# haowenz/FEM

Measured on AMD Instinct MI355X. Metric: mapped Mreads/s (100 bp, e=3) at 1/2/4/8 MI355X + achieved HBM GB/s vs roofline, higher is better.
Workload: dtype u32/u64 integer + 32-bit Myers bit-vectors

## Files before the change

fem_amd/csrc/fem_hip.hip:

```cpp
#include "../../include/fem_hip.h"

#include <hip/hip_runtime.h>
#include <rccl/rccl.h>
#include <sched.h>
#if defined(__x86_64__)
#include <immintrin.h>
#endif

#include <algorithm>
#include <cctype>
#include <cstdio>
#include <cstdlib>
#include <cstring>
#include <condition_variable>
#include <functional>
#include <atomic>
#include <chrono>
#include <mutex>
#include <string>
#include <thread>
#include <vector>

#include "fem_index_build.hip.h"
#include "fem_pack.h"
#include "fem_kernels.hip.h"
#include "fem_seed_fast.hip.h"
#include "fem_seed_join.hip.h"
#include "fem_tail.hip.h"
#include "fem_bgzf.hip.h"

namespace {

#ifndef FEM_SLOTS
#define FEM_SLOTS 4
#endif
constexpr int kSlots = FEM_SLOTS;
constexpr uint32_t kMaxReadLen = 1024;
constexpr size_t kFrontPad = 16;
constexpr uint32_t kXcapSmall = 512, kFcap = 128, kCcap = 128;

constexpr int kTimedKernels = 15;
struct TimedLaunch {
  int kernel;
  hipEvent_t start, stop;
  bool counts = true;
};
constexpr int kMaxParts = 4;

struct Slot {
  hipStream_t stream = nullptr;
  uint8_t *d_bases_alloc = nullptr;
  uint8_t *bases() const { return d_bases_alloc + 16; }
  size_t bases_cap = 0;
  uint64_t *d_off = nullptr;
  size_t off_cap = 0;
  uint64_t n_reads = 0;
  uint64_t n_bases = 0;
  uint32_t max_len = 0;
  bool staged = false;
  char *h_bases = nullptr;
  size_t h_bases_cap = 0;
  uint64_t *h_off = nullptr;
  size_t h_off_cap = 0;
  uint64_t acq_reads = 0, acq_bases = 0;
  char *h_quals = nullptr, *h_names = nullptr;
  uint64_t *h_name_off = nullptr;
  size_t h_quals_cap = 0, h_names_cap = 0, h_name_off_cap = 0;
  uint8_t *d_quals = nullptr, *d_names = nullptr;
  uint64_t *d_name_off = nullptr;
  size_t d_quals_cap = 0, d_names_cap = 0, d_name_off_cap = 0;
  bool text_staged = false;
  bool host_quals = false;
  const uint64_t *qual_at = nullptr;
  hipStream_t text_stream = nullptr;
  hipStream_t out_stream = nullptr;
  hipEvent_t ev_text_staged = nullptr;
  hipEvent_t ev_text_order = nullptr;
  bool have_text_order = false;
  uint8_t *d_packed = nullptr;
  size_t packed_cap = 0;
  uint32_t *d_exc_bits = nullptr;
  size_t exc_bits_cap = 0;
  uint32_t packed_bpr = 0;
  bool prefetch_results = false, staged_by_copy = false;
  uint64_t prefetched_reads2 = 0, prefetched_cand = 0, last_n_cand = 0;
  uint64_t h2d_bytes = 0;
  bool sent_packed = false;
  int parts = 1;
  uint32_t part_begin[kMaxParts + 1] = {0, 0, 0, 0, 0};
  hipEvent_t ev_part[kMaxParts] = {nullptr, nullptr, nullptr, nullptr}, ev_sel[kMaxParts] = {nullptr, nullptr, nullptr, nullptr};
  hipEvent_t ev_zeroed = nullptr;
  hipEvent_t ev_results = nullptr, ev_home = nullptr;
  uint64_t *d_cand = nullptr;
  uint32_t *d_meta = nullptr;
  uint8_t *d_ed = nullptr;
  int16_t *d_end = nullptr;
  uint32_t cand_cap = 0;
  uint32_t *d_begin = nullptr, *d_count = nullptr, *d_nmap = nullptr;
  size_t per_read_cap = 0;
  uint8_t *d_ctl = nullptr;
  uint8_t *h_ctl = nullptr;
  uint64_t *d_arena = nullptr;
  uint64_t arena_cap = 0;
  uint32_t *d_slow = nullptr;
  uint32_t slow_cap = 0;
  uint2 *d_sel = nullptr, *d_sel_hdr = nullptr;
  size_t sel_cap = 0, sel_hdr_cap = 0;
  uint32_t *h_begin = nullptr, *h_count = nullptr;
  size_t h_per_read_cap = 0;
  uint64_t *h_cand = nullptr;
  uint8_t *h_ed = nullptr;
  int16_t *h_end = nullptr;
  size_t h_cand_cap = 0;
  uint8_t *d_count8 = nullptr, *d_ped = nullptr;
  uint32_t *d_seg = nullptr;
  uint64_t *d_pcand = nullptr;
  int16_t *d_pend = nullptr;
  uint2 *d_big = nullptr;
  size_t count8_cap = 0, seg_cap = 0, pcand_cap = 0;
  uint8_t *h_count8 = nullptr, *h_ped = nullptr;
  uint32_t *h_seg = nullptr;
  uint64_t *h_pcand = nullptr;
  int16_t *h_pend = nullptr;
  uint2 *h_big = nullptr;
  size_t h_count8_cap = 0, h_seg_cap = 0, h_pcand_cap = 0;
  bool want_packed = false;
  bool packed_enqueued = false;
  uint64_t packed_home = 0, last_n_packed = 0;
  bool packed_per_read_home = false;
  uint32_t n_packed = 0, n_big = 0;
  fem_params params{};
  bool mapped = false, synced = false;
  uint64_t stats[5] = {0, 0, 0, 0, 0};
  uint32_t n_cand = 0;
  std::vector<TimedLaunch> pending;
  femt::Tail *tail = nullptr;
  bool paired = false;
  int32_t min_insert = 0, max_insert = 0;
  uint64_t n_proper = 0;
  bool rescue = false;
  int32_t rescue_edits = 0;
  uint64_t n_rescued = 0;
  bool mapq = false;
  bool unmapped = false;
  uint64_t n_unmapped = 0;
  std::vector<uint16_t> pr_flag;
  std::vector<uint32_t> pr_tid, pr_pos0, pr_cigar_off, pr_cigar, pr_md_off;
  std::vector<uint8_t> pr_nm;
  std::vector<char> pr_md;
};

constexpr size_t kCtlPackCursor = 4 * sizeof(uint32_t) + 2 * sizeof(uint64_t) + 4 * sizeof(uint64_t);
constexpr size_t kCtlBytes = kCtlPackCursor + 2 * sizeof(uint32_t);
constexpr uint32_t kBigCap = 4096;
constexpr size_t kCtlWorkCursor = 128, kCtlWorkCursor2 = 192, kCtlPartStride = 128, kCtlAlloc = 1024;
static_assert(kCtlWorkCursor2 + (kMaxParts - 1) * kCtlPartStride + 64 <= kCtlAlloc, "control block layout");
static_assert(kCtlBytes <= kCtlWorkCursor, "control block layout");

}

namespace {
class StagePool {
 public:
  ~StagePool() {
    {
      std::lock_guard<std::mutex> l(m_);
      stop_ = true;
    }
    cv_.notify_all();
    for (auto &t : threads_) t.join();
  }
  void run(unsigned n, const std::function<void(unsigned)> &work) {
    if (n <= 1) return work(0u);
    {
      std::lock_guard<std::mutex> l(m_);
      while (threads_.size() + 1 < n) {
        const unsigned id = (unsigned)threads_.size() + 1;
        threads_.emplace_back([this, id] { loop(id); });
      }
      work_ = &work, n_ = n, pending_ = n - 1, ++epoch_;
    }
    cv_.notify_all();
    work(0u);
    std::unique_lock<std::mutex> l(m_);
    done_.wait(l, [&] { return pending_ == 0; });
    work_ = nullptr;
  }

 private:
  void loop(unsigned id) {
    uint64_t seen = 0;
    for (;;) {
      const std::function<void(unsigned)> *w = nullptr;
      {
        std::unique_lock<std::mutex> l(m_);
        cv_.wait(l, [&] { return stop_ || (epoch_ != seen && id < n_); });
        if (stop_) return;
        seen = epoch_, w = work_;
      }
      (*w)(id);
      std::lock_guard<std::mutex> l(m_);
      if (--pending_ == 0) done_.notify_one();
    }
  }
  std::mutex m_;
  std::condition_variable cv_, done_;
  std::vector<std::thread> threads_;
  const std::function<void(unsigned)> *work_ = nullptr;
  unsigned n_ = 0, pending_ = 0;
  uint64_t epoch_ = 0;
  bool stop_ = false;
};
}

struct fem_dev {
  femt::TextGate text_gate;
  femz::Bgzf *bgzf = nullptr;
  uint8_t *d_zin = nullptr;
  size_t d_zin_cap = 0;
  hipStream_t z_stream = nullptr;
  std::recursive_mutex mu;
  int device = 0;
  StagePool *stage_pool = nullptr;
  uint8_t *d_ref_names = nullptr;
  uint32_t *d_ref_name_off = nullptr;
  int n_cu = 256;
  std::string err;
  uint32_t *d_lookup = nullptr;
  uint64_t n_lookup = 0;
  uint64_t *d_occ = nullptr;
  uint64_t n_occ = 0;
  int32_t k = 0, step = 0;
  uint64_t fast_occ_key = ~0ull;
  int fast_occ_blocks = 0;
  uint32_t *d_summary = nullptr;
  uint32_t *d_occ32 = nullptr, *d_goff = nullptr, *d_blkseq = nullptr;
  uint32_t list_shift = 0;
  bool no_strided = false;
  uint32_t *d_freq11 = nullptr;
  uint32_t n_banks = 1, bank_first[5] = {0, 0, 0, 0, 0};
  uint32_t *d_bank_lo = nullptr;
  uint64_t bank_limit = 0;
  uint32_t bank_seqs = 0;
  int select_occ_blocks = 0, join_occ_blocks = 0;
  uint64_t select_occ_key = ~0ull, join_occ_key = ~0ull;
  uint8_t *d_planes = nullptr;
  uint8_t *d_ref_raw = nullptr;
  uint64_t ref_bytes = 0;
  uint64_t *d_seq_off = nullptr;
  uint32_t *d_seq_len = nullptr;
  uint32_t n_seq = 0;
  std::vector<uint64_t> seq_off;
  std::vector<uint32_t> seq_len;
  Slot slot[kSlots];
  bool timing = false;
  int verify_blocks_per_cu = 0;
  double t_ms[kTimedKernels] = {};
  uint64_t t_n[kTimedKernels] = {};
  bool force_generic = false;
  bool force_hash = false;
  bool force_dense = false;
  bool no_dense = false;
  bool tiny_buffers = false;
  std::vector<hipEvent_t> event_pool;
  hipEvent_t ev_kernels_done = nullptr;
  bool have_kernels_done = false;
  hipEvent_t ev_select_done = nullptr;
  bool have_select_done = false;
  bool no_overlap = false;
  hipEvent_t ev_h2d_done = nullptr;
  bool have_h2d_done = false;
  hipStream_t side_stream = nullptr;
  bool no_parts = false;
  int max_parts = 2;
  bool timeline = false, have_epoch = false;
  hipEvent_t ev_epoch = nullptr;
};

namespace {

bool testing_switch(const char *name) {
  const char *t = getenv("FEM_TESTING");
  if (!(t && t[0] == '1')) return false;
  const char *v = getenv(name);
  return v && v[0] == '1';
}

int fail(fem_dev *h, int rc, const std::string &msg) {
  if (h) {
    std::lock_guard<std::recursive_mutex> lock(h->mu);
    h->err = msg;
  }
  return rc;
}
#define FEM_LOCK(h) std::lock_guard<std::recursive_mutex> fem_lock_(h->mu)

#define HIP_TRY(h, expr)                                                                          \
  do {                                                                                            \
    hipError_t e_ = (expr);                                                                       \
    if (e_ != hipSuccess)                                                                         \
      return fail(h, e_ == hipErrorOutOfMemory ? FEM_ERR_NOMEM : FEM_ERR_HIP,                     \
                  std::string(#expr) + ": " + hipGetErrorString(e_));                             \
  } while (0)

template <typename T>
int dev_realloc(fem_dev *h, T **p, size_t *cap, size_t want, bool keep = false) {
  if (want <= *cap && *p) return FEM_OK;
  size_t n = std::max(want, *cap + *cap / 2);
  T *q = nullptr;
  HIP_TRY(h, hipMalloc((void **)&q, std::max<size_t>(n, 1) * sizeof(T)));
  if (keep && *p && *cap) HIP_TRY(h, hipMemcpy(q, *p, *cap * sizeof(T), hipMemcpyDeviceToDevice));
  if (*p) (void)hipFree(*p);
  *p = q;
  *cap = n;
  return FEM_OK;
}

template <typename T>
int pinned_realloc(fem_dev *h, T **p, size_t *cap, size_t want) {
  if (want <= *cap && *p) return FEM_OK;
  size_t n = std::max(want, *cap + *cap / 2);
  if (*p) (void)hipHostFree(*p);
  *p = nullptr;
  HIP_TRY(h, hipHostMalloc((void **)p, std::max<size_t>(n, 1) * sizeof(T), hipHostMallocDefault));
  *cap = n;
  return FEM_OK;
}

bool params_ok(const fem_params *p) {
  return p && p->k >= 1 && p->k <= 16 && p->step >= 1 && p->step <= 16 && p->e >= 0 && p->e <= 7 && p->a >= 0 &&
         p->a <= 2;
}

femk::SeedLayout make_layout(const fem_params &p, uint32_t max_len) {
  femk::SeedLayout l{};
  const uint32_t R = (uint32_t)(p.e + 1 + p.a);
  const uint32_t lg = (uint32_t)(p.k / p.step + (p.k % p.step ? 1 : 0));
  const uint32_t n_groups = 2u * (uint32_t)p.step;
  uint32_t smax = max_len >= (uint32_t)p.k ? max_len - (uint32_t)p.k + 1u : 1u;
  int c = (int)(smax / (uint32_t)p.step) - (int)(R * lg) + 2;
  uint32_t cmax = (uint32_t)std::max(c, 2);
  l.smax = smax;
  l.cmax = cmax;
  l.cw = (cmax + 31u) / 32u;
  l.n_words = (max_len + 15u) / 16u + 2u;
  l.xcap = kXcapSmall, l.fcap = kFcap, l.ccap = kCcap;
  uint32_t o = 0;
  auto take = [&](uint32_t bytes) {
    uint32_t at = o;
    o += (bytes + 15u) & ~15u;
    return at;
  };
  l.pkw = take(l.n_words * 4u);
  l.nkw = take(l.n_words * 4u);
  l.sf = take(2u * smax * 8u);
  l.dp_rows = take(n_groups * 2u * cmax * 4u);
  l.dp_bits = take(std::max(n_groups * R * l.cw * 4u, n_groups * R * 8u));
  l.picked = take(n_groups * R * 16u);
  l.rb = take(2u * (R + 1u) * 4u);
  l.X = take(l.xcap * 8u);
  l.F = take(l.fcap * 8u);
  l.A = take(l.ccap * 8u);
  l.B = take(l.ccap * 8u);
  l.wave_bytes = o;
  return l;
}

femk::SeedLayout make_layout_fast(const fem_params &p, uint32_t max_len, bool hash) {
  femk::SeedLayout l{};
  const uint32_t R = (uint32_t)(p.e + 1 + p.a);
  const uint32_t n_groups = 2u * (uint32_t)p.step;
  l.smax = max_len >= (uint32_t)p.k ? max_len - (uint32_t)p.k + 1u : 1u;
  l.n_words = (max_len + 15u) / 16u + 2u;
  l.xcap = 64;
  uint32_t o = 0;
  auto take = [&](uint32_t bytes) {
    uint32_t at = o;
    o += (bytes + 15u) & ~15u;
    return at;
  };
  if (hash) {
    l.pkw = take(l.n_words * 4u);
    l.nkw = take(l.n_words * 4u);
  }
  if (hash) l.sf = take(std::max(2u * l.smax * 8u, 2u * 64u * 8u));
  l.dp_bits = take(std::max(n_groups, femk::kGroupQueue) * R * 8u);
  if (hash) {
    l.X = take(64u * 8u);
    l.A = take(femk::kListScratchBytes);
  }
  l.B = take(2u * femk::kReadBlock * 8u);
  if (!hash) {
    const uint32_t blk_chars = femk::kReadBlock * std::min(max_len, 256u);
    l.strm_words = blk_chars / 16u + 3u;
    l.strm = take(3u * l.strm_words * 4u);
    const uint32_t q_at = o;
    l.F = take(femk::kQueueBytes);
    const uint32_t g0 = l.smax / (uint32_t)femk::kStep;
    const uint32_t n_used = g0 > (uint32_t)femk::kLg ? g0 - (uint32_t)femk::kLg + 1u : 1u;
    l.gq_cap = std::max(384u, n_groups * n_used);
    l.gq = take(std::max(l.gq_cap * 4u + femk::kGroupQueue * 16u + 2u * 32u * 4u, femk::kFlushScratchBytes));
    l.blk_bytes = blk_chars + 32u;
    l.blk = q_at;
    if (o < q_at + l.blk_bytes) take(q_at + l.blk_bytes - o);
  }
  if (hash) {
    l.xcap = (uint32_t)femk::bloom_chunks((int)R) * 64u;
    l.F = take(femk::bloom_slots((int)R) / 16u * 4u);
  }
  l.wave_bytes = o;
  return l;
}

femk::SeedLayout make_layout_select(const fem_params &p, uint32_t max_len) {
  femk::SeedLayout l{};
// ... 48 lines not shown
}
template <int R>
int select_blocks_per_cu_r(bool banked, int block, uint32_t lds) {
  int nb = 0;
  const hipError_t e = banked ? hipOccupancyMaxActiveBlocksPerMultiprocessor(&nb, femk::seed_select_kernel<R, true>, block, lds)
                              : hipOccupancyMaxActiveBlocksPerMultiprocessor(&nb, femk::seed_select_kernel<R>, block, lds);
  return e == hipSuccess ? nb : 0;
}
typedef void (*JoinKernel)(femk::SeedParams);
JoinKernel join_kernel(int R, int which) {
  static const JoinKernel k[3][femk::kMaxR] = {
      {femk::seed_join_kernel_r1, femk::seed_join_kernel_r2, femk::seed_join_kernel_r3, femk::seed_join_kernel_r4, femk::seed_join_kernel_r5,
       femk::seed_join_kernel_r6, femk::seed_join_kernel_r7, femk::seed_join_kernel_r8, femk::seed_join_kernel_r9, femk::seed_join_kernel_r10},
      {femk::seed_join_banked_kernel_r1, femk::seed_join_banked_kernel_r2, femk::seed_join_banked_kernel_r3, femk::seed_join_banked_kernel_r4,
       femk::seed_join_banked_kernel_r5, femk::seed_join_banked_kernel_r6, femk::seed_join_banked_kernel_r7, femk::seed_join_banked_kernel_r8,
       femk::seed_join_banked_kernel_r9, femk::seed_join_banked_kernel_r10},
      {femk::seed_join_kernel_padded_r1, femk::seed_join_kernel_padded_r2, femk::seed_join_kernel_padded_r3, femk::seed_join_kernel_padded_r4,
       femk::seed_join_kernel_padded_r5, femk::seed_join_kernel_padded_r6, femk::seed_join_kernel_padded_r7, femk::seed_join_kernel_padded_r8,
       femk::seed_join_kernel_padded_r9, femk::seed_join_kernel_padded_r10}};
  return k[which][std::min(std::max(R, 1), femk::kMaxR) - 1];
}

#define FEM_DENSE_SWITCH(R, CALL)      \
  switch (R) {                         \
    case 1: CALL(1); break;            \
    case 2: CALL(2); break;            \
    case 3: CALL(3); break;            \
    case 4: CALL(4); break;            \
    case 5: CALL(5); break;            \
    case 6: CALL(6); break;            \
    case 7: CALL(7); break;            \
    case 8: CALL(8); break;            \
    case 9: CALL(9); break;            \
    default: CALL(10); break;          \
  }
template <int R>
uint32_t kernel_regs_r(bool join, int which) {
  hipFuncAttributes a{};
  const bool banked = which == 1;
  const void *f = join ? (const void *)join_kernel(R, which)
                       : banked ? (const void *)femk::seed_select_kernel<R, true> : (const void *)femk::seed_select_kernel<R>;
  return hipFuncGetAttributes(&a, f) == hipSuccess && a.numRegs > 0 ? (uint32_t)a.numRegs : 128u;
}
uint32_t kernel_regs(int R, bool join, int which = 0) {
  static std::atomic<uint32_t> cache[3][2][femk::kMaxR + 1] = {};
  std::atomic<uint32_t> &slot = cache[which][join ? 1 : 0][std::min(std::max(R, 1), femk::kMaxR)];
  uint32_t c = slot.load(std::memory_order_relaxed);
  if (c) return c;
#define FEM_CALL(r) c = kernel_regs_r<r>(join, which)
  FEM_DENSE_SWITCH(R, FEM_CALL)
#undef FEM_CALL
  slot.store(c, std::memory_order_relaxed);
  return c;
}
int select_blocks_per_cu(int R, bool banked, int block, uint32_t lds) {
  int nb = 0;
#define FEM_CALL(r) nb = select_blocks_per_cu_r<r>(banked, block, lds)
  FEM_DENSE_SWITCH(R, FEM_CALL)
#undef FEM_CALL
  return nb;
}
void launch_select(int R, bool banked, dim3 grid, dim3 block, uint32_t lds, hipStream_t st, const femk::SeedParams &sp) {
#define FEM_CALL(r) launch_select_r<r>(banked, grid, block, lds, st, sp)
  FEM_DENSE_SWITCH(R, FEM_CALL)
#undef FEM_CALL
}
int join_blocks_per_cu(int R, int which, int block, uint32_t lds) {
  int nb = 0;
  return hipOccupancyMaxActiveBlocksPerMultiprocessor(&nb, join_kernel(R, which), block, lds) == hipSuccess ? nb : 0;
}
void launch_join(int R, int which, dim3 grid, dim3 block, uint32_t lds, hipStream_t st, const femk::SeedParams &sp) {
  hipLaunchKernelGGL(join_kernel(R, which), grid, block, lds, st, sp);
}

template <int R>
void launch_fast(bool hash, dim3 grid, dim3 block, uint32_t lds, hipStream_t st, const femk::SeedParams &sp) {
  if (hash)
    hipLaunchKernelGGL((femk::seed_fast_kernel<R, true>), grid, block, lds, st, sp);
  else
    hipLaunchKernelGGL((femk::seed_fast_kernel<R, false>), grid, block, lds, st, sp);
}

template <int R>
int fast_blocks_per_cu_r(bool hash, int block, uint32_t lds) {
  int nb = 0;
  hipError_t err = hash ? hipOccupancyMaxActiveBlocksPerMultiprocessor(&nb, femk::seed_fast_kernel<R, true>, block, lds)
                        : hipOccupancyMaxActiveBlocksPerMultiprocessor(&nb, femk::seed_fast_kernel<R, false>, block, lds);
  return err == hipSuccess ? nb : 0;
}
int fast_blocks_per_cu(int R, bool hash, int block, uint32_t lds) {
  switch (R) {
    case 1: return fast_blocks_per_cu_r<1>(hash, block, lds);
    case 2: return fast_blocks_per_cu_r<2>(hash, block, lds);
    case 3: return fast_blocks_per_cu_r<3>(hash, block, lds);
    case 4: return fast_blocks_per_cu_r<4>(hash, block, lds);
    case 5: return fast_blocks_per_cu_r<5>(hash, block, lds);
    case 6: return fast_blocks_per_cu_r<6>(hash, block, lds);
    case 7: return fast_blocks_per_cu_r<7>(hash, block, lds);
    case 8: return fast_blocks_per_cu_r<8>(hash, block, lds);
    case 9: return fast_blocks_per_cu_r<9>(hash, block, lds);
    default: return fast_blocks_per_cu_r<10>(hash, block, lds);
  }
}

hipEvent_t get_event(fem_dev *h) {
  if (!h->event_pool.empty()) {
    hipEvent_t e = h->event_pool.back();
    h->event_pool.pop_back();
    return e;
  }
  hipEvent_t e = nullptr;
  (void)hipEventCreate(&e);
  return e;
}

struct Span {
  fem_dev *h;
  Slot &s;
  hipStream_t st;
  TimedLaunch t;
  bool on;
  Span(fem_dev *h_, Slot &s_, int id, hipStream_t st_) : h(h_), s(s_), st(st_), t{id, nullptr, nullptr, false}, on(h_->timing && h_->timeline) {
    if (on) {
      t.start = get_event(h), t.stop = get_event(h);
      (void)hipEventRecord(t.start, st);
    }
  }
  ~Span() {
    if (on) {
      (void)hipEventRecord(t.stop, st);
      s.pending.push_back(t);
    }
  }
};

void drain_timing(fem_dev *h, Slot &s) {
  for (auto &t : s.pending) {
    float ms = 0.f;
    if (hipEventElapsedTime(&ms, t.start, t.stop) == hipSuccess && t.kernel < kTimedKernels) {
      h->t_ms[t.kernel] += ms;
      h->t_n[t.kernel] += t.counts ? 1 : 0;
    }
    if (h->timeline && h->have_epoch) {
      float a = 0.f, b = 0.f;
      if (hipEventElapsedTime(&a, h->ev_epoch, t.start) == hipSuccess && hipEventElapsedTime(&b, h->ev_epoch, t.stop) == hipSuccess)
        fprintf(stderr, "TL slot %d id %2d  %9.3f %9.3f  (%.3f)\n", (int)(&s - h->slot), t.kernel, a, b, b - a);
    }
    h->event_pool.push_back(t.start);
    h->event_pool.push_back(t.stop);
  }
  s.pending.clear();
}

int ensure_outputs(fem_dev *h, Slot &s) {
  size_t want_reads = (size_t)s.n_reads;
  if (want_reads > s.per_read_cap || !s.d_begin) {
    size_t cap = std::max<size_t>(want_reads, 1);
    if (s.d_begin) (void)hipFree(s.d_begin);
    if (s.d_count) (void)hipFree(s.d_count);
    if (s.d_nmap) (void)hipFree(s.d_nmap);
    s.d_begin = s.d_count = s.d_nmap = nullptr;
    HIP_TRY(h, hipMalloc((void **)&s.d_begin, cap * 2 * sizeof(uint32_t)));
    HIP_TRY(h, hipMalloc((void **)&s.d_count, cap * 2 * sizeof(uint32_t)));
    HIP_TRY(h, hipMalloc((void **)&s.d_nmap, cap * sizeof(uint32_t)));
    s.per_read_cap = cap;
  }
  if (!s.d_cand || !s.d_meta || !s.d_ed || !s.d_end || s.cand_cap == 0) {
    for (void *p : {(void *)s.d_cand, (void *)s.d_meta, (void *)s.d_ed, (void *)s.d_end})
      if (p) (void)hipFree(p);
    s.d_cand = nullptr, s.d_meta = nullptr, s.d_ed = nullptr, s.d_end = nullptr;
    uint64_t want = 2 * s.n_reads + (5u << 20);
    if (h->tiny_buffers) want = 512;
    want = std::min<uint64_t>(want, 0xFFFFFFF0ull);
    s.cand_cap = 0;
    size_t c0 = 0, c1 = 0, c2 = 0, c3 = 0;
    int rc;
    if ((rc = dev_realloc(h, &s.d_cand, &c0, want))) return rc;
    if ((rc = dev_realloc(h, &s.d_meta, &c1, want))) return rc;
    if ((rc = dev_realloc(h, &s.d_ed, &c2, want))) return rc;
    if ((rc = dev_realloc(h, &s.d_end, &c3, want))) return rc;
    s.cand_cap = (uint32_t)want;
  }
  if (!s.d_ctl) {
    HIP_TRY(h, hipMalloc((void **)&s.d_ctl, kCtlAlloc));
    HIP_TRY(h, hipHostMalloc((void **)&s.h_ctl, kCtlBytes, hipHostMallocDefault));
  }
  if (!s.d_arena) {
    s.arena_cap = h->tiny_buffers ? 256u : (4u << 20);
    HIP_TRY(h, hipMalloc((void **)&s.d_arena, s.arena_cap * sizeof(uint64_t)));
  }
  {
    const double avg_bucket = (double)h->n_occ / (double)(h->n_lookup ? h->n_lookup : 1);
    uint64_t want = avg_bucket > 1.0 ? s.n_reads + (1u << 20) : (1u << 18);
    if (h->tiny_buffers) want = s.d_slow ? s.slow_cap : 32;
    if (want > s.slow_cap || !s.d_slow) {
      if (s.d_slow) (void)hipFree(s.d_slow);
      s.d_slow = nullptr;
      HIP_TRY(h, hipMalloc((void **)&s.d_slow, want * sizeof(uint32_t)));
      s.slow_cap = (uint32_t)want;
    }
  }
  return FEM_OK;
}

int grow_candidates(fem_dev *h, Slot &s, uint64_t want) {
  if (want > 0xFFFFFFF0ull) return fail(h, FEM_ERR_UNSUPPORTED, "more than 2^32 candidates in one batch; split the batch");
  s.cand_cap = 0;
  for (void *p : {(void *)s.d_cand, (void *)s.d_meta, (void *)s.d_ed, (void *)s.d_end})
    if (p) (void)hipFree(p);
  s.d_cand = nullptr, s.d_meta = nullptr, s.d_ed = nullptr, s.d_end = nullptr;
  HIP_TRY(h, hipMalloc((void **)&s.d_cand, want * sizeof(uint64_t)));
  HIP_TRY(h, hipMalloc((void **)&s.d_meta, want * sizeof(uint32_t)));
  HIP_TRY(h, hipMalloc((void **)&s.d_ed, want * sizeof(uint8_t)));
  HIP_TRY(h, hipMalloc((void **)&s.d_end, want * sizeof(int16_t)));
  s.cand_cap = (uint32_t)want;
  return FEM_OK;
}

int h2d_begin(fem_dev *h, Slot &s) {
  if (h->have_h2d_done) HIP_TRY(h, hipStreamWaitEvent(s.stream, h->ev_h2d_done, 0));
  return FEM_OK;
}
int h2d_end(fem_dev *h, Slot &s) {
  HIP_TRY(h, hipEventRecord(h->ev_h2d_done, s.stream));
  h->have_h2d_done = true;
  return FEM_OK;
}
bool device_idle(fem_dev *h) {
  return (!h->have_kernels_done || hipEventQuery(h->ev_kernels_done) == hipSuccess) &&
         (!h->have_select_done || hipEventQuery(h->ev_select_done) == hipSuccess);
}
constexpr uint64_t kPartMinReads = 1u << 16;

hipStream_t d2h_begin(fem_dev *h, Slot &s) {
  (void)h;
  return s.stream;
}
int d2h_end(fem_dev *h, Slot &s, hipStream_t st) {
  if (st == s.stream) return FEM_OK;
  HIP_TRY(h, hipEventRecord(s.ev_home, st));
  HIP_TRY(h, hipStreamWaitEvent(s.stream, s.ev_home, 0));
  return FEM_OK;
}

int enqueue_pack(fem_dev *h, Slot &s, bool kernel, bool send_home) {
  const size_t n2 = (size_t)s.n_reads * 2, n_seg = (n2 + 255) / 256;
  int rc;
  if ((rc = dev_realloc(h, &s.d_count8, &s.count8_cap, n2 + 16))) return rc;
  if ((rc = dev_realloc(h, &s.d_seg, &s.seg_cap, n_seg + 4))) return rc;
  if (s.pcand_cap < s.cand_cap || !s.d_pcand) {
    for (void *q : {(void *)s.d_pcand, (void *)s.d_ped, (void *)s.d_pend})
      if (q) (void)hipFree(q);
    s.d_pcand = nullptr, s.d_ped = nullptr, s.d_pend = nullptr, s.pcand_cap = 0;
    HIP_TRY(h, hipMalloc((void **)&s.d_pcand, (size_t)s.cand_cap * sizeof(uint64_t)));
    HIP_TRY(h, hipMalloc((void **)&s.d_ped, (size_t)s.cand_cap * sizeof(uint8_t)));
    HIP_TRY(h, hipMalloc((void **)&s.d_pend, (size_t)s.cand_cap * sizeof(int16_t)));
    s.pcand_cap = s.cand_cap;
  }
  if (!s.d_big) HIP_TRY(h, hipMalloc((void **)&s.d_big, kBigCap * sizeof(uint2)));
  if (n2 + 16 > s.h_count8_cap || !s.h_count8) {
    if (s.h_count8) (void)hipHostFree(s.h_count8);
    s.h_count8 = nullptr, s.h_count8_cap = 0;
    if ((rc = pinned_realloc(h, &s.h_count8, &s.h_count8_cap, n2 + 16))) return rc;
  }
  if (n_seg + 4 > s.h_seg_cap || !s.h_seg) {
    if (s.h_seg) (void)hipHostFree(s.h_seg);
    s.h_seg = nullptr, s.h_seg_cap = 0;
    if ((rc = pinned_realloc(h, &s.h_seg, &s.h_seg_cap, n_seg + 4))) return rc;
  }
  if (!s.h_big) {
    size_t c = 0;
    if ((rc = pinned_realloc(h, &s.h_big, &c, (size_t)kBigCap))) return rc;
  }
  if (kernel) {
  femk::PackParams pp{};
  pp.cand_begin = s.d_begin, pp.cand_count = s.d_count, pp.cand = s.d_cand, pp.ed = s.d_ed, pp.end = s.d_end;
  pp.ctr = (const uint32_t *)s.d_ctl, pp.n_strands = (uint32_t)n2;
  pp.count8 = s.d_count8, pp.seg_begin = s.d_seg, pp.pcand = s.d_pcand, pp.ped = s.d_ped, pp.pend = s.d_pend, pp.pcap = (uint32_t)s.pcand_cap;
  pp.cursor = (uint32_t *)(s.d_ctl + kCtlPackCursor), pp.big = s.d_big, pp.big_cap = kBigCap;
  const uint32_t grid = (uint32_t)std::max<size_t>(1, (n_seg + femk::kPackSegs - 1) / femk::kPackSegs);
  {
    TimedLaunch t{6, nullptr, nullptr, true};
    if (h->timing) {
      t.start = get_event(h), t.stop = get_event(h);
      HIP_TRY(h, hipEventRecord(t.start, s.stream));
    }
    hipLaunchKernelGGL(femk::pack_results_kernel, dim3(grid), dim3(256), 0, s.stream, pp);
    HIP_TRY(h, hipGetLastError());
    if (h->timing) {
      HIP_TRY(h, hipEventRecord(t.stop, s.stream));
      s.pending.push_back(t);
    }
  }
  s.packed_enqueued = true;
  }
  if (send_home) {
    hipStream_t st = d2h_begin(h, s);
    {
      Span span(h, s, 21, st);
      HIP_TRY(h, hipMemcpyAsync(s.h_count8, s.d_count8, n2, hipMemcpyDeviceToHost, st));
      HIP_TRY(h, hipMemcpyAsync(s.h_seg, s.d_seg, n_seg * sizeof(uint32_t), hipMemcpyDeviceToHost, st));
      s.packed_per_read_home = true;
      const size_t guess = std::min<size_t>({(size_t)(s.last_n_packed + s.last_n_packed / 32 + 1024), s.h_pcand_cap, s.pcand_cap});
      if (s.last_n_packed && s.h_pcand && guess) {
        HIP_TRY(h, hipMemcpyAsync(s.h_pcand, s.d_pcand, guess * sizeof(uint64_t), hipMemcpyDeviceToHost, st));
        HIP_TRY(h, hipMemcpyAsync(s.h_ped, s.d_ped, guess * sizeof(uint8_t), hipMemcpyDeviceToHost, st));
        HIP_TRY(h, hipMemcpyAsync(s.h_pend, s.d_pend, guess * sizeof(int16_t), hipMemcpyDeviceToHost, st));
        s.packed_home = guess;
      }
    }
    if ((rc = d2h_end(h, s, st))) return rc;
  }
  return FEM_OK;
}

int launch_batch(fem_dev *h, Slot &s) {
  const fem_params &p = s.params;
  uint32_t *d_ctr = (uint32_t *)s.d_ctl;
  unsigned long long *d_arena_ctr = (unsigned long long *)(s.d_ctl + 4 * sizeof(uint32_t));
  unsigned long long *d_stats = (unsigned long long *)(s.d_ctl + 4 * sizeof(uint32_t) + 2 * sizeof(uint64_t));
  int parts = 1;
  uint32_t part_begin[kMaxParts + 1] = {0, 0, 0, 0, 0};
  const bool copied_in_parts = s.parts > 1;
  {
    const int R_ = p.e + 1 + p.a;
    const bool dense_overlap = !h->force_generic && p.k == femk::kK && p.step == femk::kStep && R_ >= 1 && R_ <= femk::kMaxR && h->d_occ32 &&
                               h->d_freq11 && !h->no_overlap;
    if (dense_overlap && !h->no_parts && s.n_reads >= 2 * kPartMinReads && (copied_in_parts || device_idle(h))) {
      parts = copied_in_parts ? s.parts : (int)std::min<uint64_t>((uint64_t)h->max_parts, s.n_reads / kPartMinReads);
      for (int q = 0; q <= parts; ++q)
        part_begin[q] = copied_in_parts ? s.part_begin[q] : q == parts ? (uint32_t)s.n_reads : (uint32_t)((s.n_reads * q / parts) & ~63ull);
    }
    s.parts = 1;
  }
  if (parts > 1) {
    if (h->have_select_done) HIP_TRY(h, hipStreamWaitEvent(h->side_stream, h->ev_select_done, 0));
    HIP_TRY(h, hipMemsetAsync(s.d_ctl, 0, kCtlAlloc, h->side_stream));
  } else {
    HIP_TRY(h, hipMemsetAsync(s.d_ctl, 0, kCtlAlloc, s.stream));
  }

  femk::SeedParams sp{};
  sp.bases = s.bases();
  sp.read_off = s.d_off;
  sp.n_reads = (uint32_t)s.n_reads;
  sp.read_begin = 0;
  sp.lookup = h->d_lookup;
  sp.occ = h->d_occ;
  sp.inf32 = (uint32_t)h->n_occ;
  sp.seq_len = h->d_seq_len;
  sp.e = p.e, sp.a = p.a, sp.R = p.e + 1 + p.a, sp.k = p.k, sp.step = p.step;
  sp.lg = p.k / p.step + (p.k % p.step ? 1 : 0);
  sp.cand = s.d_cand, sp.cand_meta = s.d_meta, sp.cand_cap = s.cand_cap;
  sp.cand_begin = s.d_begin, sp.cand_count = s.d_count;
  sp.ctr = d_ctr;
  sp.work_cursor = (uint32_t *)(s.d_ctl + kCtlWorkCursor);
  sp.stats = d_stats;
  sp.arena = s.d_arena, sp.arena_cap = s.arena_cap, sp.arena_ctr = d_arena_ctr;
  sp.lay = make_layout(p, std::max<uint32_t>(s.max_len, (uint32_t)p.k));

  sp.n_seq = h->n_seq;
  sp.summary = h->d_summary;
  sp.slow_queue = s.d_slow, sp.slow_cap = s.slow_cap;
  sp.work_queue = nullptr;
  const int R = p.e + 1 + p.a;
  const bool use_fast = !h->force_generic && p.k == femk::kK && p.step == femk::kStep && R >= 1 && R <= femk::kMaxR;

  auto shape = [&](const femk::SeedLayout &lay, uint32_t *wpb_out, uint32_t *lds_out, uint32_t *grid_out) {
    uint32_t wpb = std::min<uint32_t>(4u, std::max<uint32_t>(1u, (64u * 1024u) / lay.wave_bytes));
    uint32_t lds_bytes = wpb * lay.wave_bytes;
    uint32_t waves_per_cu = std::min<uint32_t>(32u, (160u * 1024u / lds_bytes) * wpb);
    uint64_t blocks_wanted = (s.n_reads + wpb - 1) / wpb;
    uint64_t blocks_resident = (uint64_t)h->n_cu * std::max<uint32_t>(1u, waves_per_cu / wpb);
    *wpb_out = wpb, *lds_out = lds_bytes;
    *grid_out = (uint32_t)std::max<uint64_t>(1, std::min<uint64_t>(blocks_wanted, blocks_resident * 4));
  };
  if (sp.lay.wave_bytes > 64u * 1024u) return fail(h, FEM_ERR_UNSUPPORTED, "read too long for the device path");

  auto timed = [&](int id, hipStream_t st, auto &&launch, bool counts = true) -> int {
    TimedLaunch t{id, nullptr, nullptr, counts};
    if (h->timing) {
      t.start = get_event(h), t.stop = get_event(h);
      HIP_TRY(h, hipEventRecord(t.start, st));
    }
    launch();
    HIP_TRY(h, hipGetLastError());
    if (h->timing) {
      HIP_TRY(h, hipEventRecord(t.stop, st));
      s.pending.push_back(t);
    }
    return FEM_OK;
  };

  if (s.n_reads) {
    int rc;
    const bool split_dense = use_fast && h->d_occ32 && h->d_freq11;
    const bool overlap = split_dense && !h->no_overlap;
    if (!overlap && h->have_kernels_done) HIP_TRY(h, hipStreamWaitEvent(s.stream, h->ev_kernels_done, 0));
    femk::VerifyParams vp{};
    vp.bases = s.bases(), vp.read_off = s.d_off;
    vp.planes = h->d_planes, vp.seq_off = h->d_seq_off;
    vp.cand = s.d_cand, vp.cand_meta = s.d_meta;
    vp.ctr = d_ctr, vp.cand_cap = s.cand_cap, vp.e = p.e;
    vp.ed = s.d_ed, vp.end = s.d_end;
    vp.n_map = s.d_nmap, vp.stats = d_stats;
    HIP_TRY(h, hipMemsetAsync(s.d_nmap, 0, (size_t)s.n_reads * sizeof(uint32_t), s.stream));
    if (h->verify_blocks_per_cu == 0) {
      int nb = 0;
      if (hipOccupancyMaxActiveBlocksPerMultiprocessor(&nb, femk::verify_kernel, 256, 0) != hipSuccess || nb <= 0) nb = 4;
      h->verify_blocks_per_cu = nb;
    }
    const uint32_t vgrid = (uint32_t)h->n_cu * (uint32_t)h->verify_blocks_per_cu;
    if (split_dense) {
      const uint32_t max_len = std::max<uint32_t>(s.max_len, (uint32_t)p.k);
      const bool banked = h->n_banks > 1;
      const size_t want_sel = (size_t)s.n_reads * 6u * (size_t)R * h->n_banks;
      if ((rc = dev_realloc(h, &s.d_sel, &s.sel_cap, want_sel))) return rc;
      if ((rc = dev_realloc(h, &s.d_sel_hdr, &s.sel_hdr_cap, (size_t)s.n_reads))) return rc;
      femk::SeedParams fp = sp;
      fp.occ32 = h->d_occ32, fp.list_shift = h->list_shift, fp.goff = h->d_goff, fp.blkseq = h->d_blkseq;
      fp.freq11 = h->d_freq11, fp.sel = s.d_sel, fp.sel_hdr = s.d_sel_hdr;
      fp.n_banks = h->n_banks, fp.bank_lo = h->d_bank_lo, fp.n_buckets = (uint32_t)(h->n_lookup - 1);
      fp.blk_stride = (femk::kDenseRemap >> femk::kDenseBlkShift) + 1u;
      for (uint32_t b = 0; b <= femk::kDenseMaxBanks; ++b) fp.bank_first[b] = h->bank_first[b];
      uint32_t select_lds = 0, select_threads = 256;
      fp.lay = make_layout_select(p, max_len);
      if (fp.lay.wave_bytes > 64u * 1024u) return fail(h, FEM_ERR_UNSUPPORTED, "read too long for the device path");
      const femk::SeedLayout lay_select = fp.lay;
      femk::SeedLayout lay_join = make_layout_join(p, banked, !banked && h->list_shift != 0);
      const uint32_t wpb_s = std::min<uint32_t>(4u, std::max<uint32_t>(1u, (64u * 1024u) / lay_select.wave_bytes));
      const uint32_t wpb_j = std::min<uint32_t>(4u, std::max<uint32_t>(1u, (60u * 1024u) / lay_join.wave_bytes));
      lay_join.picked = wpb_j * lay_join.wave_bytes;
      const uint32_t lds_j = wpb_j * lay_join.wave_bytes + 64u * 8u;
      const int which = banked ? 1 : h->list_shift ? 2 : 0;
      uint64_t per_cu_s, per_cu_j;
      {
        const uint32_t lds_bytes = wpb_s * lay_select.wave_bytes;
        const uint64_t key = ((uint64_t)banked << 48) | ((uint64_t)R << 40) | lds_bytes;
        if (h->select_occ_key != key) h->select_occ_key = key, h->select_occ_blocks = select_blocks_per_cu(R, banked, (int)(64u * wpb_s), lds_bytes);
        per_cu_s = h->select_occ_blocks > 0 ? (uint64_t)h->select_occ_blocks : std::max<uint64_t>(1, 160u * 1024u / lds_bytes);
        if (overlap) per_cu_s = 1;
        select_lds = lds_bytes, select_threads = 64u * wpb_s;
      }
      {
        const uint64_t key = ((uint64_t)which << 48) | ((uint64_t)R << 40) | lds_j;
        if (h->join_occ_key != key) h->join_occ_key = key, h->join_occ_blocks = join_blocks_per_cu(R, which, (int)(64u * wpb_j), lds_j);
        per_cu_j = h->join_occ_blocks > 0 ? (uint64_t)h->join_occ_blocks : std::max<uint64_t>(1, 160u * 1024u / lds_j);
        if (overlap) {
          const uint32_t vj = (kernel_regs(R, true, which) + 7u) & ~7u, vs = (kernel_regs(R, false, banked ? 1 : 0) + 7u) & ~7u;
          const uint32_t wj = 64u * wpb_j / 256u ? 64u * wpb_j / 256u : 1u, ws = select_threads / 256u ? select_threads / 256u : 1u;
          const uint32_t lj = (lds_j + 511u) & ~511u, ls = (select_lds + 511u) & ~511u;
          while (per_cu_j > 1 && (per_cu_j * wj * vj + ws * vs > 512u || per_cu_j * lj + ls > 160u * 1024u || per_cu_j * wj + ws > 8u)) --per_cu_j;
        }
      }
      if (parts > 1 && !copied_in_parts) {
        HIP_TRY(h, hipEventRecord(s.ev_zeroed, s.stream));
        HIP_TRY(h, hipStreamWaitEvent(h->side_stream, s.ev_zeroed, 0));
      }
      for (int q = 0; q < parts; ++q) {
        const uint32_t r_lo = parts > 1 ? part_begin[q] : 0u, r_hi = parts > 1 ? part_begin[q + 1] : (uint32_t)s.n_reads;
        const uint64_t blocks_of_reads = ((uint64_t)(r_hi - r_lo) + femk::kReadBlock - 1) / femk::kReadBlock;
        fp.read_begin = r_lo, fp.n_reads = r_hi;
        hipStream_t st_sel = parts > 1 ? h->side_stream : s.stream;
        {
          fp.lay = lay_select;
          if (parts > 1) {
            if (copied_in_parts) HIP_TRY(h, hipStreamWaitEvent(st_sel, s.ev_part[q], 0));
          } else if (overlap && h->have_select_done) {
            HIP_TRY(h, hipStreamWaitEvent(s.stream, h->ev_select_done, 0));
          }
          const uint32_t grid = (uint32_t)std::max<uint64_t>(1, std::min<uint64_t>((blocks_of_reads + wpb_s - 1) / wpb_s, (uint64_t)h->n_cu * per_cu_s));
          fp.work_cursor = (uint32_t *)(s.d_ctl + kCtlWorkCursor + (size_t)q * kCtlPartStride);
          rc = timed(8, st_sel, [&] { launch_select(R, banked, dim3(grid), dim3(64u * wpb_s), select_lds, st_sel, fp); }, q == 0);
          if (rc) return rc;
          if (parts > 1) {
            HIP_TRY(h, hipEventRecord(s.ev_sel[q], st_sel));
            HIP_TRY(h, hipStreamWaitEvent(s.stream, s.ev_sel[q], 0));
          }
          if (overlap && q + 1 == parts) {
            HIP_TRY(h, hipEventRecord(h->ev_select_done, st_sel));
            h->have_select_done = true;
          }
          if (overlap && q == 0 && h->have_kernels_done) HIP_TRY(h, hipStreamWaitEvent(s.stream, h->ev_kernels_done, 0));
        }
        {
          fp.lay = lay_join;
          const uint32_t grid = (uint32_t)std::max<uint64_t>(1, std::min<uint64_t>((blocks_of_reads + wpb_j - 1) / wpb_j, (uint64_t)h->n_cu * per_cu_j));
          fp.work_cursor = (uint32_t *)(s.d_ctl + kCtlWorkCursor2 + (size_t)q * kCtlPartStride);
          rc = timed(0, s.stream, [&] { launch_join(R, which, dim3(grid), dim3(64u * wpb_j), lds_j, s.stream, fp); }, q == 0);
          if (rc) return rc;
        }
      }
      sp.work_queue = s.d_slow;
    } else if (use_fast) {
      femk::SeedParams fp = sp;
      const bool hash = h->force_hash || (double)h->n_occ > (double)h->n_lookup;
      fp.lay = make_layout_fast(p, std::max<uint32_t>(s.max_len, (uint32_t)p.k), hash);
      uint32_t wpb, lds_bytes, grid;
      shape(fp.lay, &wpb, &lds_bytes, &grid);
      {
        const uint64_t key = ((uint64_t)R << 40) | ((uint64_t)hash << 32) | lds_bytes;
        if (h->fast_occ_key != key) h->fast_occ_key = key, h->fast_occ_blocks = fast_blocks_per_cu((int)R, hash, (int)(64u * wpb), lds_bytes);
        static const uint64_t mult = testing_switch("FEM_TESTING") && getenv("FEM_GRID_MULT") ? (uint64_t)std::max(1, atoi(getenv("FEM_GRID_MULT"))) : 1;
        const uint64_t per_cu = h->fast_occ_blocks > 0 ? (uint64_t)h->fast_occ_blocks : std::max<uint64_t>(1, 160u * 1024u / lds_bytes);
        const uint64_t wanted = (s.n_reads + (uint64_t)femk::kReadBlock * wpb - 1) / ((uint64_t)femk::kReadBlock * wpb);
        grid = (uint32_t)std::max<uint64_t>(1, std::min<uint64_t>(wanted, (uint64_t)h->n_cu * per_cu * mult));
      }
      auto launch_range = [&](uint32_t lo, uint32_t hi) {
        femk::SeedParams q = fp;
        q.read_begin = lo, q.n_reads = hi;
        dim3 g(grid), b(64u * wpb);
        switch (R) {
          case 1: launch_fast<1>(hash, g, b, lds_bytes, s.stream, q); break;
          case 2: launch_fast<2>(hash, g, b, lds_bytes, s.stream, q); break;
          case 3: launch_fast<3>(hash, g, b, lds_bytes, s.stream, q); break;
          case 4: launch_fast<4>(hash, g, b, lds_bytes, s.stream, q); break;
          case 5: launch_fast<5>(hash, g, b, lds_bytes, s.stream, q); break;
          case 6: launch_fast<6>(hash, g, b, lds_bytes, s.stream, q); break;
          case 7: launch_fast<7>(hash, g, b, lds_bytes, s.stream, q); break;
          case 8: launch_fast<8>(hash, g, b, lds_bytes, s.stream, q); break;
          case 9: launch_fast<9>(hash, g, b, lds_bytes, s.stream, q); break;
          default: launch_fast<10>(hash, g, b, lds_bytes, s.stream, q); break;
        }
      };
      rc = timed(0, s.stream, [&] { launch_range(0, (uint32_t)s.n_reads); });
      if (rc) return rc;
      sp.work_queue = s.d_slow;
    }
    {
      uint32_t wpb, lds_bytes, grid;
      shape(sp.lay, &wpb, &lds_bytes, &grid);
      rc = timed(2, s.stream, [&] { hipLaunchKernelGGL(femk::seed_filter_kernel, dim3(grid), dim3(64u * wpb), lds_bytes, s.stream, sp); });
      if (rc) return rc;
    }
    rc = timed(1, s.stream, [&] { hipLaunchKernelGGL(femk::verify_kernel, dim3(vgrid), dim3(256), 0, s.stream, vp); });
    if (rc) return rc;
    s.packed_enqueued = false, s.packed_home = 0, s.packed_per_read_home = false;
    if (s.want_packed && split_dense && (rc = enqueue_pack(h, s, true, false))) return rc;
    HIP_TRY(h, hipEventRecord(h->ev_kernels_done, s.stream));
    h->have_kernels_done = true;
    if (s.want_packed && (rc = enqueue_pack(h, s, !split_dense, true))) return rc;
  } else {
    s.packed_enqueued = false, s.packed_home = 0, s.packed_per_read_home = false;
  }
  HIP_TRY(h, hipMemcpyAsync(s.h_ctl, s.d_ctl, kCtlBytes, hipMemcpyDeviceToHost, s.stream));
  s.prefetched_reads2 = 0, s.prefetched_cand = 0;
  static const bool no_prefetch = testing_switch("FEM_NO_PREFETCH");
  if (s.prefetch_results && !s.want_packed && s.staged_by_copy && !no_prefetch) {
    hipStream_t st = d2h_begin(h, s);
    {
      Span span(h, s, 21, st);
      const size_t n2 = (size_t)s.n_reads * 2;
      if (n2 && s.h_begin && n2 <= s.h_per_read_cap) {
        HIP_TRY(h, hipMemcpyAsync(s.h_begin, s.d_begin, n2 * sizeof(uint32_t), hipMemcpyDeviceToHost, st));
        HIP_TRY(h, hipMemcpyAsync(s.h_count, s.d_count, n2 * sizeof(uint32_t), hipMemcpyDeviceToHost, st));
        s.prefetched_reads2 = n2;
      }
      const size_t guess = std::min<size_t>({(size_t)(s.last_n_cand + s.last_n_cand / 32 + 1024), s.h_cand_cap, (size_t)s.cand_cap});
      if (s.last_n_cand && s.h_cand && guess) {
        HIP_TRY(h, hipMemcpyAsync(s.h_cand, s.d_cand, guess * sizeof(uint64_t), hipMemcpyDeviceToHost, st));
        HIP_TRY(h, hipMemcpyAsync(s.h_ed, s.d_ed, guess * sizeof(uint8_t), hipMemcpyDeviceToHost, st));
        HIP_TRY(h, hipMemcpyAsync(s.h_end, s.d_end, guess * sizeof(int16_t), hipMemcpyDeviceToHost, st));
        s.prefetched_cand = guess;
      }
    }
    int rc2 = d2h_end(h, s, st);
    if (rc2) return rc2;
  }
  s.mapped = true;
  s.synced = false;
  return FEM_OK;
}

int refresh_summary(fem_dev *h) {
  if (h->d_summary) (void)hipFree(h->d_summary);
  h->d_summary = nullptr;
  const uint64_t n_buckets = h->n_lookup - 1;
// ... 121 lines not shown
  std::vector<uint64_t *> bufs;
};
std::mutex g_comm_mu;
CommSet *g_comm = nullptr;
void destroy_comm_set() {
  if (!g_comm) return;
  for (size_t i = 0; i < g_comm->devs.size(); ++i) {
    (void)hipSetDevice(g_comm->devs[i]);
    if (g_comm->bufs[i]) (void)hipFree(g_comm->bufs[i]);
    if (g_comm->comms[i]) ncclCommDestroy(g_comm->comms[i]);
  }
  delete g_comm;
  g_comm = nullptr;
}

int check_slot(fem_dev *h, int slot) {
  if (!h) return FEM_ERR_INVALID;
  if (slot < 0 || slot >= kSlots) return fail(h, FEM_ERR_INVALID, "slot out of range");
  return FEM_OK;
}


using fempack::pack_bases;

int enqueue_packed(fem_dev *h, Slot &s, uint64_t n, uint32_t len, uint64_t n_exc) {
  const uint32_t bpr = fempack::bytes_per_read(len);
  const uint64_t code_bytes = fempack::code_bytes(n, len), n_bases = n * (uint64_t)len;
  const uint64_t total = code_bytes + n_exc * 5u;
  int rc;
  if ((rc = dev_realloc(h, &s.d_packed, &s.packed_cap, (size_t)total + 64))) return rc;
  if ((rc = dev_realloc(h, &s.d_bases_alloc, &s.bases_cap, kFrontPad + (size_t)n_bases + 64))) return rc;
  if ((rc = dev_realloc(h, &s.d_off, &s.off_cap, (size_t)n + 1))) return rc;
  if ((rc = dev_realloc(h, &s.d_exc_bits, &s.exc_bits_cap, (size_t)n / 32 + 2))) return rc;
  s.parts = 1;
  if (!h->no_parts && !h->no_overlap && n_exc == 0 && n >= 2 * kPartMinReads && device_idle(h))
    s.parts = (int)std::min<uint64_t>((uint64_t)h->max_parts, n / kPartMinReads);
  for (int q = 0; q <= s.parts; ++q) s.part_begin[q] = q == s.parts ? (uint32_t)n : (uint32_t)((n * q / s.parts) & ~63ull);
  HIP_TRY(h, hipMemsetAsync(s.d_exc_bits, 0, ((size_t)n / 32 + 1) * sizeof(uint32_t), s.stream));
  hipLaunchKernelGGL(femk::uniform_offsets_kernel, dim3((uint32_t)std::min<uint64_t>((n + 256) / 256, (uint64_t)h->n_cu * 8u)), dim3(256), 0,
                     s.stream, s.d_off, n, len);
  if ((rc = h2d_begin(h, s))) return rc;
  for (int q = 0; q < s.parts; ++q) {
    const uint64_t r0 = s.part_begin[q], r1 = s.part_begin[q + 1];
    const uint64_t b0 = r0 * bpr, b1 = q + 1 == s.parts ? total : r1 * bpr;
    Span span(h, s, 20, s.stream);
    if (b1 > b0) HIP_TRY(h, hipMemcpyAsync(s.d_packed + b0, s.h_bases + b0, b1 - b0, hipMemcpyHostToDevice, s.stream));
    if (q + 1 == s.parts && (rc = h2d_end(h, s))) return rc;
    if (r1 > r0) {
      const uint32_t grid = (uint32_t)std::min<uint64_t>(((r1 - r0) * bpr + 255) / 256, (uint64_t)h->n_cu * 16u);
      hipLaunchKernelGGL(femk::unpack_reads_kernel, dim3(grid), dim3(256), 0, s.stream, (const uint8_t *)s.d_packed + b0, r1 - r0, len, bpr,
                         s.bases() + r0 * len);
    }
    if (s.parts > 1) HIP_TRY(h, hipEventRecord(s.ev_part[q], s.stream));
  }
  if (n_exc) {
    const dim3 g((uint32_t)std::min<uint64_t>((n_exc + 255) / 256, (uint64_t)h->n_cu * 4u));
    hipLaunchKernelGGL(femk::scatter_chars_kernel, g, dim3(256), 0, s.stream, (const uint32_t *)(s.d_packed + code_bytes),
                       (const uint8_t *)(s.d_packed + code_bytes + 4u * n_exc), n_exc, s.bases());
    hipLaunchKernelGGL(femk::mark_exception_reads_kernel, g, dim3(256), 0, s.stream, (const uint32_t *)(s.d_packed + code_bytes), n_exc, len,
                       s.d_exc_bits);
  }
  s.packed_bpr = bpr;
  HIP_TRY(h, hipGetLastError());
  s.n_reads = n, s.n_bases = n_bases, s.max_len = len;
  s.staged = true, s.mapped = false, s.synced = false;
  s.h2d_bytes = total, s.sent_packed = true;
  return FEM_OK;
}

unsigned stage_threads(uint64_t n_reads) {
  unsigned want = 12;
  if (const char *e = getenv("FEM_STAGE_THREADS")) want = (unsigned)std::max(1, atoi(e));
  const unsigned hw = std::thread::hardware_concurrency();
  return (unsigned)std::max<uint64_t>(1, std::min<uint64_t>({(uint64_t)(hw ? hw : 1), (uint64_t)want, n_reads / 65536 + 1}));
}

}

extern "C" {

const char *fem_strerror(int rc) {
  switch (rc) {
    case FEM_OK: return "ok";
    case FEM_ERR_INVALID: return "invalid argument";
    case FEM_ERR_HIP: return "HIP runtime error";
    case FEM_ERR_NOMEM: return "out of memory";
    case FEM_ERR_STATE: return "call order violated";
    case FEM_ERR_UNSUPPORTED: return "input not supported by the device path";
    case FEM_ERR_RCCL: return "RCCL error";
    default: return "unknown error";
  }
}

const char *fem_dev_last_error(const fem_dev *h) { return h ? h->err.c_str() : "null handle"; }

static std::atomic<int> g_blocking_waits{0};
int fem_set_blocking_waits(int on) {
  g_blocking_waits.store(on ? 1 : 0);
  return FEM_OK;
}

int fem_dev_open(int device, fem_dev **out) {
  if (!out) return FEM_ERR_INVALID;
  *out = nullptr;
  int n = 0;
  if (hipGetDeviceCount(&n) != hipSuccess || n <= 0) return FEM_ERR_HIP;
  if (device < 0 || device >= n) return FEM_ERR_INVALID;
  fem_dev *h = new (std::nothrow) fem_dev();
  if (!h) return FEM_ERR_NOMEM;
  h->device = device;
  if (hipSetDevice(device) != hipSuccess) {
    delete h;
    return FEM_ERR_HIP;
  }
  if (g_blocking_waits.load() || testing_switch("FEM_BLOCKING_SYNC")) (void)hipSetDeviceFlags(hipDeviceScheduleBlockingSync);
  hipDeviceProp_t prop;
  if (hipGetDeviceProperties(&prop, device) == hipSuccess) h->n_cu = prop.multiProcessorCount;
  for (int i = 0; i < kSlots; ++i) {
    if (hipStreamCreateWithFlags(&h->slot[i].stream, hipStreamNonBlocking) != hipSuccess) {
      delete h;
      return FEM_ERR_HIP;
    }
  }
  bool ok_ev = hipEventCreateWithFlags(&h->ev_kernels_done, hipEventDisableTiming) == hipSuccess &&
               hipEventCreateWithFlags(&h->ev_select_done, hipEventDisableTiming) == hipSuccess &&
               hipEventCreateWithFlags(&h->ev_h2d_done, hipEventDisableTiming) == hipSuccess &&
               hipStreamCreateWithFlags(&h->side_stream, hipStreamNonBlocking) == hipSuccess;
  for (int i = 0; ok_ev && i < kSlots; ++i) {
    Slot &sl = h->slot[i];
    ok_ev = hipEventCreateWithFlags(&sl.ev_zeroed, hipEventDisableTiming) == hipSuccess &&
            hipEventCreateWithFlags(&sl.ev_results, hipEventDisableTiming) == hipSuccess &&
            hipEventCreateWithFlags(&sl.ev_home, hipEventDisableTiming) == hipSuccess;
    for (int q = 0; ok_ev && q < kMaxParts; ++q)
      ok_ev = hipEventCreateWithFlags(&sl.ev_part[q], hipEventDisableTiming) == hipSuccess &&
              hipEventCreateWithFlags(&sl.ev_sel[q], hipEventDisableTiming) == hipSuccess;
  }
  if (!ok_ev) {
    (void)fem_dev_close(h);
    return FEM_ERR_HIP;
  }
  if (testing_switch("FEM_TESTING")) {
    h->no_overlap = testing_switch("FEM_NO_OVERLAP");
    h->no_parts = testing_switch("FEM_NO_PARTS");
    if (const char *mp = getenv("FEM_PARTS")) h->max_parts = std::min(kMaxParts, std::max(1, atoi(mp)));
    h->timeline = testing_switch("FEM_TIMELINE");
    if (h->timeline && hipEventCreate(&h->ev_epoch) == hipSuccess && hipEventRecord(h->ev_epoch, h->side_stream) == hipSuccess)
      h->timing = true, h->have_epoch = true;
    h->force_generic = testing_switch("FEM_FORCE_GENERIC");
    h->force_hash = testing_switch("FEM_FORCE_HASH");
    h->force_dense = testing_switch("FEM_FORCE_DENSE");
    h->no_dense = testing_switch("FEM_NO_DENSE");
    h->no_strided = testing_switch("FEM_NO_STRIDED");
    h->tiny_buffers = testing_switch("FEM_TEST_TINY_BUFFERS");
    if (const char *bl = getenv("FEM_TEST_BANK_BASES")) h->bank_limit = strtoull(bl, nullptr, 10);
    if (const char *bs = getenv("FEM_TEST_BANK_SEQS")) h->bank_seqs = (uint32_t)strtoul(bs, nullptr, 10);
  }
  *out = h;
  return FEM_OK;
}

int fem_dev_close(fem_dev *h) {
  if (!h) return FEM_ERR_INVALID;
  {
    std::lock_guard<std::mutex> lock(g_comm_mu);
    if (g_comm && std::find(g_comm->devs.begin(), g_comm->devs.end(), h->device) != g_comm->devs.end()) destroy_comm_set();
  }
  (void)hipSetDevice(h->device);
  (void)hipDeviceSynchronize();
  delete h->stage_pool;
  h->stage_pool = nullptr;
  for (auto &s : h->slot) {
    drain_timing(h, s);
    for (void *p : {(void *)s.d_bases_alloc, (void *)s.d_off, (void *)s.d_cand, (void *)s.d_meta, (void *)s.d_ed,
                    (void *)s.d_end, (void *)s.d_begin, (void *)s.d_count, (void *)s.d_nmap, (void *)s.d_ctl,
                    (void *)s.d_arena, (void *)s.d_slow, (void *)s.d_sel, (void *)s.d_sel_hdr, (void *)s.d_packed, (void *)s.d_exc_bits, (void *)s.d_quals, (void *)s.d_names,
                    (void *)s.d_name_off, (void *)s.d_count8, (void *)s.d_seg, (void *)s.d_pcand, (void *)s.d_ped, (void *)s.d_pend, (void *)s.d_big})
      if (p) (void)hipFree(p);
    for (void *p : {(void *)s.h_ctl, (void *)s.h_begin, (void *)s.h_count, (void *)s.h_cand, (void *)s.h_ed,
                    (void *)s.h_end, (void *)s.h_bases, (void *)s.h_off, (void *)s.h_quals, (void *)s.h_names, (void *)s.h_name_off,
                    (void *)s.h_count8, (void *)s.h_seg, (void *)s.h_pcand, (void *)s.h_ped, (void *)s.h_pend, (void *)s.h_big})
      if (p) (void)hipHostFree(p);
    if (s.stream) (void)hipStreamDestroy(s.stream);
    if (s.text_stream) (void)hipStreamDestroy(s.text_stream);
    if (s.out_stream) (void)hipStreamDestroy(s.out_stream);
    if (s.ev_text_staged) (void)hipEventDestroy(s.ev_text_staged);
    if (s.ev_text_order) (void)hipEventDestroy(s.ev_text_order);
    delete s.tail;
    s.tail = nullptr;
  }
  delete h->bgzf;
  h->bgzf = nullptr;
  if (h->d_zin) (void)hipFree(h->d_zin);
  if (h->z_stream) (void)hipStreamDestroy(h->z_stream);
  if (h->d_ref_names) (void)hipFree(h->d_ref_names);
  if (h->d_ref_name_off) (void)hipFree(h->d_ref_name_off);
  for (hipEvent_t e : h->event_pool) (void)hipEventDestroy(e);
  if (h->ev_kernels_done) (void)hipEventDestroy(h->ev_kernels_done);
  if (h->ev_select_done) (void)hipEventDestroy(h->ev_select_done);
  if (h->ev_h2d_done) (void)hipEventDestroy(h->ev_h2d_done);
  if (h->ev_epoch) (void)hipEventDestroy(h->ev_epoch);
  if (h->side_stream) (void)hipStreamDestroy(h->side_stream);
  for (int i = 0; i < kSlots; ++i) {
    Slot &sl = h->slot[i];
    if (sl.ev_zeroed) (void)hipEventDestroy(sl.ev_zeroed);
    if (sl.ev_results) (void)hipEventDestroy(sl.ev_results);
    if (sl.ev_home) (void)hipEventDestroy(sl.ev_home);
    for (int q = 0; q < kMaxParts; ++q) {
      if (sl.ev_part[q]) (void)hipEventDestroy(sl.ev_part[q]);
      if (sl.ev_sel[q]) (void)hipEventDestroy(sl.ev_sel[q]);
    }
  }
  for (void *p : {(void *)h->d_lookup, (void *)h->d_occ, (void *)h->d_ref_raw, (void *)h->d_seq_off,
                  (void *)h->d_seq_len, (void *)h->d_summary, (void *)h->d_planes, (void *)h->d_occ32, (void *)h->d_goff, (void *)h->d_blkseq,
                  (void *)h->d_freq11, (void *)h->d_bank_lo})
    if (p) (void)hipFree(p);
  delete h;
  return FEM_OK;
}

int fem_dev_limits(const fem_dev *h, uint32_t *max_read_len, int32_t *n_slots) {
  if (!h) return FEM_ERR_INVALID;
  if (max_read_len) *max_read_len = kMaxReadLen;
  if (n_slots) *n_slots = kSlots;
  return FEM_OK;
}

int fem_dev_upload_index(fem_dev *h, int32_t k, int32_t step, const uint32_t *lookup, uint64_t n_lookup,
                         const uint64_t *occ, uint64_t n_occ) {
  if (!h || !lookup || (!occ && n_occ)) return FEM_ERR_INVALID;
  if (k < 1 || k > 16 || step < 1) return fail(h, FEM_ERR_INVALID, "k must be 1..16 and step >= 1");
  if (n_lookup != (1ull << (2 * k)) + 1) return fail(h, FEM_ERR_INVALID, "lookup table must have 4^k + 1 entries");
  if (n_occ > 0xFFFFFFFFull) return fail(h, FEM_ERR_INVALID, "occurrence table larger than its uint32 prefix sums");
  HIP_TRY(h, hipSetDevice(h->device));
  if (h->d_lookup) (void)hipFree(h->d_lookup);
  if (h->d_occ) (void)hipFree(h->d_occ);
  h->d_lookup = nullptr, h->d_occ = nullptr;
  HIP_TRY(h, hipMalloc((void **)&h->d_lookup, n_lookup * sizeof(uint32_t)));
  HIP_TRY(h, hipMalloc((void **)&h->d_occ, std::max<uint64_t>(n_occ, 1) * sizeof(uint64_t)));
  HIP_TRY(h, hipMemcpy(h->d_lookup, lookup, n_lookup * sizeof(uint32_t), hipMemcpyHostToDevice));
  if (n_occ) HIP_TRY(h, hipMemcpy(h->d_occ, occ, n_occ * sizeof(uint64_t), hipMemcpyHostToDevice));
  h->n_lookup = n_lookup, h->n_occ = n_occ, h->k = k, h->step = step;
  int rc = refresh_summary(h);
  return rc ? rc : refresh_dense(h);
}

namespace {
int make_codes(fem_dev *h, uint8_t **out) {
  *out = nullptr;
  uint8_t *codes = nullptr;
  const uint64_t total = h->ref_bytes;
  HIP_TRY(h, hipMalloc((void **)&codes, total + 128));
  hipError_t e = hipMemcpy(codes, h->d_ref_raw, total, hipMemcpyDeviceToDevice);
  if (e == hipSuccess) e = hipMemset(codes + total, 4, 128);
  if (e == hipSuccess && total) {
    hipLaunchKernelGGL(femk::ref_encode_kernel, dim3((uint32_t)h->n_cu * 8u), dim3(256), 0, 0, codes, total);
    e = hipGetLastError();
    if (e == hipSuccess) e = hipDeviceSynchronize();
  }
  if (e != hipSuccess) {
    (void)hipFree(codes);
    HIP_TRY(h, e);
  }
  *out = codes;
  return FEM_OK;
}
}

int fem_dev_upload_reference(fem_dev *h, uint32_t n_seq, const char *const *seq, const uint32_t *seq_len) {
  if (!h || !seq || !seq_len || n_seq == 0) return FEM_ERR_INVALID;
  HIP_TRY(h, hipSetDevice(h->device));
  h->seq_off.assign(n_seq, 0);
  h->seq_len.assign(seq_len, seq_len + n_seq);
  uint64_t total = 0;
  for (uint32_t i = 0; i < n_seq; ++i) {
    h->seq_off[i] = total;
    total += seq_len[i];
  }
  for (void *p : {(void *)h->d_ref_raw, (void *)h->d_seq_off, (void *)h->d_seq_len, (void *)h->d_planes})
    if (p) (void)hipFree(p);
  h->d_ref_raw = nullptr, h->d_seq_off = nullptr, h->d_seq_len = nullptr;
  h->d_planes = nullptr;
  h->ref_bytes = 0, h->n_seq = 0;
  HIP_TRY(h, hipMalloc((void **)&h->d_ref_raw, total + 128));
  HIP_TRY(h, hipMalloc((void **)&h->d_seq_off, n_seq * sizeof(uint64_t)));
  HIP_TRY(h, hipMalloc((void **)&h->d_seq_len, n_seq * sizeof(uint32_t)));
  for (uint32_t i = 0; i < n_seq; ++i)
    if (seq_len[i]) HIP_TRY(h, hipMemcpy(h->d_ref_raw + h->seq_off[i], seq[i], seq_len[i], hipMemcpyHostToDevice));
  HIP_TRY(h, hipMemset(h->d_ref_raw + total, 0, 128));
  HIP_TRY(h, hipMemcpy(h->d_seq_off, h->seq_off.data(), n_seq * sizeof(uint64_t), hipMemcpyHostToDevice));
  HIP_TRY(h, hipMemcpy(h->d_seq_len, h->seq_len.data(), n_seq * sizeof(uint32_t), hipMemcpyHostToDevice));
  HIP_TRY(h, hipMemset(h->d_ref_raw + total, 'N', 128));
  h->ref_bytes = total, h->n_seq = n_seq;
  {
    auto drop_reference = [&]() {
      for (void *q : {(void *)h->d_ref_raw, (void *)h->d_seq_off, (void *)h->d_seq_len, (void *)h->d_planes})
        if (q) (void)hipFree(q);
      h->d_ref_raw = nullptr, h->d_seq_off = nullptr, h->d_seq_len = nullptr, h->d_planes = nullptr;
      h->ref_bytes = 0, h->n_seq = 0;
    };
    uint8_t *codes = nullptr;
    int rc = make_codes(h, &codes);
    if (rc) {
      drop_reference();
      return rc;
    }
    const uint64_t n_pb = (total + 64 + 7) / 8;
    hipError_t e = hipMalloc((void **)&h->d_planes, femk::plane_bytes(n_pb));
    if (e == hipSuccess) e = hipMemset(h->d_planes, 0, femk::plane_bytes(n_pb));
    if (e == hipSuccess) {
      hipLaunchKernelGGL(femk::ref_planes_kernel, dim3((uint32_t)h->n_cu * 8u), dim3(256), 0, 0, codes, h->d_ref_raw, n_pb, h->d_planes);
      e = hipGetLastError();
      if (e == hipSuccess) e = hipDeviceSynchronize();
    }
    (void)hipFree(codes);
    if (e != hipSuccess) drop_reference();
    HIP_TRY(h, e);
  }
  return refresh_dense(h);
}

int fem_dev_build_index(fem_dev *h, int32_t k, int32_t step, uint32_t *lookup_out, uint64_t *occ_out, uint64_t occ_cap,
                        uint64_t *n_occ_out) {
  if (!h) return FEM_ERR_INVALID;
  if (!h->d_ref_raw) return fail(h, FEM_ERR_STATE, "upload the reference before building the index");
  if (k < 1 || k > 16 || step < 1) return fail(h, FEM_ERR_INVALID, "k must be 1..16 and step >= 1");
  HIP_TRY(h, hipSetDevice(h->device));
  if (h->d_lookup) (void)hipFree(h->d_lookup);
  if (h->d_occ) (void)hipFree(h->d_occ);
  h->d_lookup = nullptr, h->d_occ = nullptr;
// ... 116 lines not shown
  Slot &s = h->slot[slot];
  if (!s.h_bases) return fail(h, FEM_ERR_STATE, "acquire the slot's staging buffers first");
  if (read_len == 0 && n_reads) return fail(h, FEM_ERR_INVALID, "packed batches hold reads of one non-zero length");
  if (read_len > kMaxReadLen)
    return fail(h, FEM_ERR_UNSUPPORTED, "read longer than the device path supports (" + std::to_string(kMaxReadLen) + ")");
  const uint64_t n_bases = n_reads * (uint64_t)read_len;
  if (n_reads > s.acq_reads || n_bases > s.acq_bases) return fail(h, FEM_ERR_INVALID, "more reads than the staging buffers were acquired for");
  if (n_bases >= 0xFFFFFFF0ull) return fail(h, FEM_ERR_UNSUPPORTED, "a packed batch holds fewer than 2^32 bases; split the batch");
  const uint64_t code_bytes = fempack::code_bytes(n_reads, read_len);
  if (code_bytes + n_exceptions * 5u > s.acq_bases + 64 || n_exceptions > n_bases / 16u)
    return fail(h, FEM_ERR_INVALID, "more exceptions than a packed batch may carry (fem_dev_packed_layout): commit the characters instead");
  const uint32_t *pos = (const uint32_t *)(s.h_bases + code_bytes);
  for (uint64_t i = 0; i < n_exceptions; ++i)
    if (pos[i] >= n_bases) return fail(h, FEM_ERR_INVALID, "exception position outside the batch");
  HIP_TRY(h, hipSetDevice(h->device));
  if ((rc = enqueue_packed(h, s, n_reads, read_len, n_exceptions))) return rc;
  s.staged_by_copy = true;
  return FEM_OK;
}

int fem_dev_stage_reads(fem_dev *h, int slot, const fem_read_batch *reads) {
  int rc = check_slot(h, slot);
  if (rc) return rc;
  if (!reads || (reads->n_reads && (!reads->bases || !reads->offsets))) return fail(h, FEM_ERR_INVALID, "null read batch");
  if (reads->n_reads > 0x3FFFFFF0ull) return fail(h, FEM_ERR_UNSUPPORTED, "more than 2^30 reads in one batch");
  const uint64_t n = reads->n_reads;
  const uint64_t base0 = n ? reads->offsets[0] : 0;
  if (n && reads->offsets[n] < base0) return fail(h, FEM_ERR_INVALID, "read offsets must be ascending");
  const uint64_t n_bases = n ? reads->offsets[n] - base0 : 0;
  char *hb = nullptr;
  uint64_t *ho = nullptr;
  if ((rc = fem_dev_acquire_stage(h, slot, n, n_bases, &hb, &ho))) return rc;
  Slot &s = h->slot[slot];
  const unsigned n_thr = stage_threads(n);
  if (!h->stage_pool) h->stage_pool = new (std::nothrow) StagePool();
  if (!h->stage_pool) return fail(h, FEM_ERR_NOMEM, "out of host memory");
  auto run_threads = [&](unsigned nt, const std::function<void(unsigned)> &work) { h->stage_pool->run(nt, work); };
  std::vector<uint32_t> t_max(n_thr, 0), t_min(n_thr, 0xFFFFFFFFu);
  std::atomic<int> bad{0};
  run_threads(n_thr, [&](unsigned t) {
    const uint64_t r_lo = n * t / n_thr, r_hi = n * (t + 1) / n_thr;
    uint32_t mx = 0, mn = 0xFFFFFFFFu;
    for (uint64_t i = r_lo; i < r_hi; ++i) {
      const uint64_t o0 = reads->offsets[i], o1 = reads->offsets[i + 1];
      if (o1 < o0) {
        bad.store(1);
        return;
      }
      const uint64_t len = o1 - o0;
      if (len > kMaxReadLen) {
        bad.store(2);
        return;
      }
      mx = std::max<uint32_t>(mx, (uint32_t)len), mn = std::min<uint32_t>(mn, (uint32_t)len);
    }
    t_max[t] = mx, t_min[t] = mn;
  });
  if (bad.load() == 1) return fail(h, FEM_ERR_INVALID, "read offsets must be ascending");
  if (bad.load() == 2)
    return fail(h, FEM_ERR_UNSUPPORTED, "read longer than the device path supports (" + std::to_string(kMaxReadLen) + ")");
  uint32_t max_len = 0, min_len = 0xFFFFFFFFu;
  for (unsigned t = 0; t < n_thr; ++t) max_len = std::max(max_len, t_max[t]), min_len = std::min(min_len, t_min[t]);
  const bool no_pack = testing_switch("FEM_NO_PACK");
  if (n && min_len == max_len && max_len > 0 && n_bases < 0xFFFFFFF0ull && !no_pack) {
    const uint32_t len = max_len, bpr = (len + 3u) / 4u;
    const uint64_t code_bytes = (n * bpr + 7u) & ~7ull;
    const uint64_t exc_cap = (n_bases + 64 - std::min<uint64_t>(code_bytes, n_bases + 64)) / 5u;
    std::vector<std::vector<uint64_t>> exc(n_thr);
    const uint8_t *src = (const uint8_t *)reads->bases + base0;
    constexpr uint64_t kPiece = 32768;
    std::atomic<uint64_t> next_piece{0};
    run_threads(n_thr, [&](unsigned t) {
      for (;;) {
        const uint64_t r_lo = next_piece.fetch_add(1, std::memory_order_relaxed) * kPiece;
        if (r_lo >= n) break;
        const uint64_t r_hi = std::min(n, r_lo + kPiece);
        if ((len & 3u) == 0u) {
          pack_bases(src + r_lo * len, (r_hi - r_lo) * len, (uint8_t *)hb + r_lo * bpr, r_lo * len, exc[t]);
        } else {
          for (uint64_t i = r_lo; i < r_hi; ++i) pack_bases(src + i * len, len, (uint8_t *)hb + i * bpr, i * len, exc[t]);
        }
      }
    });
    uint64_t n_exc = 0;
    for (const auto &v : exc) n_exc += v.size();
    if (n_exc <= exc_cap && n_exc <= n_bases / 16u) {
      uint32_t *he = (uint32_t *)(hb + code_bytes);
      uint8_t *hc = (uint8_t *)(he + n_exc);
      for (const auto &v : exc)
        for (uint64_t x : v) *he++ = (uint32_t)(x >> 8), *hc++ = (uint8_t)x;
      {
        FEM_LOCK(h);
        if ((rc = enqueue_packed(h, s, n, len, n_exc))) return rc;
      }
      s.staged_by_copy = true;
      return FEM_OK;
    }
  }
  run_threads(n_thr, [&](unsigned t) {
    const uint64_t r_lo = n * t / n_thr, r_hi = n * (t + 1) / n_thr;
    for (uint64_t i = r_lo; i < r_hi; ++i) ho[i] = reads->offsets[i] - base0;
    if (r_hi == n) ho[n] = reads->offsets[n] - base0;
    if (r_hi > r_lo) memcpy(hb + (reads->offsets[r_lo] - base0), reads->bases + reads->offsets[r_lo], reads->offsets[r_hi] - reads->offsets[r_lo]);
  });
  if (n == 0) ho[0] = 0;
  rc = fem_dev_commit_stage(h, slot, n, max_len);
  s.staged_by_copy = true;
  return rc;
}

int fem_dev_stage_info(fem_dev *h, int slot, uint64_t *h2d_bytes, int32_t *packed) {
  int rc = check_slot(h, slot);
  if (rc) return rc;
  if (h2d_bytes) *h2d_bytes = h->slot[slot].h2d_bytes;
  if (packed) *packed = h->slot[slot].sent_packed ? 1 : 0;
  return FEM_OK;
}

int fem_dev_map_staged(fem_dev *h, int slot, const fem_params *p) {
  int rc = check_slot(h, slot);
  if (rc) return rc;
  FEM_LOCK(h);
  if (!params_ok(p)) return fail(h, FEM_ERR_INVALID, "parameters out of range (k 1..16, step 1..16, e 0..7, a 0..2)");
  if (!h->d_lookup || !h->d_ref_raw || !h->d_planes) return fail(h, FEM_ERR_STATE, "index and reference must be uploaded first");
  if (p->k != h->k) return fail(h, FEM_ERR_INVALID, "k differs from the uploaded index");
  Slot &s = h->slot[slot];
  if (!s.staged) return fail(h, FEM_ERR_STATE, "no reads staged in this slot");
  HIP_TRY(h, hipSetDevice(h->device));
  s.params = *p;
  if ((rc = ensure_outputs(h, s))) return rc;
  return launch_batch(h, s);
}

int fem_dev_sync(fem_dev *h, int slot) {
  int rc = check_slot(h, slot);
  if (rc) return rc;
  Slot &s = h->slot[slot];
  if (!s.mapped) return fail(h, FEM_ERR_STATE, "nothing was mapped in this slot");
  HIP_TRY(h, hipSetDevice(h->device));
  if (s.synced) return FEM_OK;
  for (int attempt = 0; attempt < 8; ++attempt) {
    HIP_TRY(h, hipStreamSynchronize(s.stream));
    FEM_LOCK(h);
    drain_timing(h, s);
    const uint32_t *ctr = (const uint32_t *)s.h_ctl;
    const uint64_t *arena_ctr = (const uint64_t *)(s.h_ctl + 4 * sizeof(uint32_t));
    const uint64_t *st = (const uint64_t *)(s.h_ctl + 4 * sizeof(uint32_t) + 2 * sizeof(uint64_t));
    uint32_t flags = ctr[1];
    if (flags & femk::kFlagTooLarge)
      return fail(h, FEM_ERR_UNSUPPORTED, "a read selects more than 2^31 occurrence entries in one seed group");
    if (flags == 0) {
      s.n_cand = ctr[0];
      s.n_packed = ((const uint32_t *)(s.h_ctl + kCtlPackCursor))[0], s.n_big = ((const uint32_t *)(s.h_ctl + kCtlPackCursor))[1];
      s.stats[0] = s.n_reads;
      s.stats[1] = st[3];
      s.stats[2] = st[0];
      s.stats[3] = st[1];
      s.stats[4] = st[2];
      s.synced = true;
      return FEM_OK;
    }
    if (flags & femk::kFlagCandOverflow) {
      uint64_t want = (uint64_t)ctr[0] + ctr[0] / 8 + 1024;
      if ((rc = grow_candidates(h, s, std::min<uint64_t>(want, 0xFFFFFFF0ull)))) return rc;
    }
    if (flags & femk::kFlagQueueOverflow) {
      uint64_t want = (uint64_t)ctr[2] + ctr[2] / 8 + 4096;
      (void)hipFree(s.d_slow);
      s.d_slow = nullptr;
      s.slow_cap = 0;
      hipError_t e = hipMalloc((void **)&s.d_slow, want * sizeof(uint32_t));
      if (e != hipSuccess) return fail(h, FEM_ERR_NOMEM, "slow-read queue does not fit in device memory");
      s.slow_cap = (uint32_t)std::min<uint64_t>(want, 0xFFFFFFF0ull);
    }
    if (flags & femk::kFlagArenaOverflow) {
      uint64_t want = arena_ctr[1] + arena_ctr[1] / 8 + 1024;
      (void)hipFree(s.d_arena);
      s.d_arena = nullptr;
      hipError_t e = hipMalloc((void **)&s.d_arena, want * sizeof(uint64_t));
      if (e != hipSuccess) {
        s.arena_cap = 0;
        return fail(h, FEM_ERR_NOMEM, "scratch arena for oversized seed lists does not fit in device memory; use smaller batches");
      }
      s.arena_cap = want;
    }
    if ((rc = launch_batch(h, s))) return rc;
  }
  return fail(h, FEM_ERR_HIP, "batch kept overflowing its scratch buffers");
}

int fem_dev_fetch_stats(fem_dev *h, int slot, uint64_t stats[5]) {
  int rc = fem_dev_sync(h, slot);
  if (rc) return rc;
  if (stats) memcpy(stats, h->slot[slot].stats, sizeof(uint64_t) * 5);
  h->slot[slot].prefetch_results = false;
  return FEM_OK;
}

int fem_dev_fetch(fem_dev *h, int slot, fem_batch_result *out) {
  int rc = fem_dev_sync(h, slot);
  if (rc) return rc;
  if (!out) return fail(h, FEM_ERR_INVALID, "null result");
  Slot &s = h->slot[slot];
  const size_t n2 = (size_t)s.n_reads * 2, nc = s.n_cand;
  bool regrown = false;
  if (n2 > s.h_per_read_cap || !s.h_begin) {
    regrown = true;
    size_t c0 = 0, c1 = 0;
    if (s.h_begin) (void)hipHostFree(s.h_begin);
    if (s.h_count) (void)hipHostFree(s.h_count);
    s.h_begin = s.h_count = nullptr;
    if ((rc = pinned_realloc(h, &s.h_begin, &c0, std::max<size_t>(n2, 2)))) return rc;
    if ((rc = pinned_realloc(h, &s.h_count, &c1, std::max<size_t>(n2, 2)))) return rc;
    s.h_per_read_cap = c0;
  }
  if (nc > s.h_cand_cap || !s.h_cand) {
    regrown = true;
    size_t c0 = 0, c1 = 0, c2 = 0;
    for (void *p : {(void *)s.h_cand, (void *)s.h_ed, (void *)s.h_end})
      if (p) (void)hipHostFree(p);
    s.h_cand = nullptr, s.h_ed = nullptr, s.h_end = nullptr;
    size_t want = std::max<size_t>(nc + nc / 4, 1024);
    if ((rc = pinned_realloc(h, &s.h_cand, &c0, want))) return rc;
    if ((rc = pinned_realloc(h, &s.h_ed, &c1, want))) return rc;
    if ((rc = pinned_realloc(h, &s.h_end, &c2, want))) return rc;
    s.h_cand_cap = c0;
  }
  const bool per_read_home = !regrown && s.prefetched_reads2 == n2;
  const size_t c_from = regrown ? 0 : std::min<size_t>(s.prefetched_cand, nc);
  if (n2 && !per_read_home) {
    HIP_TRY(h, hipMemcpyAsync(s.h_begin, s.d_begin, n2 * sizeof(uint32_t), hipMemcpyDeviceToHost, s.stream));
    HIP_TRY(h, hipMemcpyAsync(s.h_count, s.d_count, n2 * sizeof(uint32_t), hipMemcpyDeviceToHost, s.stream));
  }
  if (nc > c_from) {
    HIP_TRY(h, hipMemcpyAsync(s.h_cand + c_from, s.d_cand + c_from, (nc - c_from) * sizeof(uint64_t), hipMemcpyDeviceToHost, s.stream));
    HIP_TRY(h, hipMemcpyAsync(s.h_ed + c_from, s.d_ed + c_from, (nc - c_from) * sizeof(uint8_t), hipMemcpyDeviceToHost, s.stream));
    HIP_TRY(h, hipMemcpyAsync(s.h_end + c_from, s.d_end + c_from, (nc - c_from) * sizeof(int16_t), hipMemcpyDeviceToHost, s.stream));
  }
  if ((n2 && !per_read_home) || nc > c_from) HIP_TRY(h, hipStreamSynchronize(s.stream));
  s.prefetch_results = true, s.last_n_cand = nc, s.want_packed = false;
  out->n_reads = s.n_reads;
  out->n_candidates = nc;
  out->cand_begin = s.h_begin, out->cand_count = s.h_count;
  out->cand = s.h_cand, out->ed = s.h_ed, out->end = s.h_end;
  memcpy(out->stats, s.stats, sizeof s.stats);
  return FEM_OK;
}

int fem_dev_fetch_packed(fem_dev *h, int slot, fem_batch_packed *out) {
  int rc = fem_dev_sync(h, slot);
  if (rc) return rc;
  if (!out) return fail(h, FEM_ERR_INVALID, "null result");
  Slot &s = h->slot[slot];
  const size_t n2 = (size_t)s.n_reads * 2, n_seg = (n2 + 255) / 256;
  if (!s.packed_enqueued && s.n_reads) {
    if ((rc = enqueue_pack(h, s, true, false))) return rc;
    HIP_TRY(h, hipMemcpyAsync(s.h_ctl, s.d_ctl, kCtlBytes, hipMemcpyDeviceToHost, s.stream));
    HIP_TRY(h, hipStreamSynchronize(s.stream));
    s.n_packed = ((const uint32_t *)(s.h_ctl + kCtlPackCursor))[0], s.n_big = ((const uint32_t *)(s.h_ctl + kCtlPackCursor))[1];
  }
  if (s.n_big > kBigCap) return fail(h, FEM_ERR_UNSUPPORTED, "more strands with 255 candidates and more than a packed result lists: use fem_dev_fetch");
  const size_t np = s.n_reads ? s.n_packed : 0;
  bool regrown = false;
  if (np > s.h_pcand_cap || !s.h_pcand) {
    regrown = true;
    for (void *q : {(void *)s.h_pcand, (void *)s.h_ped, (void *)s.h_pend})
      if (q) (void)hipHostFree(q);
    s.h_pcand = nullptr, s.h_ped = nullptr, s.h_pend = nullptr;
    size_t c0 = 0, c1 = 0, c2 = 0;
    const size_t want = std::max<size_t>(np + np / 4, 1024);
    if ((rc = pinned_realloc(h, &s.h_pcand, &c0, want))) return rc;
    if ((rc = pinned_realloc(h, &s.h_ped, &c1, want))) return rc;
    if ((rc = pinned_realloc(h, &s.h_pend, &c2, want))) return rc;
    s.h_pcand_cap = c0;
  }
  bool copied = false;
  if (n2 && !s.packed_per_read_home) {
    HIP_TRY(h, hipMemcpyAsync(s.h_count8, s.d_count8, n2, hipMemcpyDeviceToHost, s.stream));
    HIP_TRY(h, hipMemcpyAsync(s.h_seg, s.d_seg, n_seg * sizeof(uint32_t), hipMemcpyDeviceToHost, s.stream));
    s.packed_per_read_home = true, copied = true;
  }
  const size_t c_from = regrown ? 0 : std::min<size_t>(s.packed_home, np);
  if (np > c_from) {
    HIP_TRY(h, hipMemcpyAsync(s.h_pcand + c_from, s.d_pcand + c_from, (np - c_from) * sizeof(uint64_t), hipMemcpyDeviceToHost, s.stream));
    HIP_TRY(h, hipMemcpyAsync(s.h_ped + c_from, s.d_ped + c_from, (np - c_from) * sizeof(uint8_t), hipMemcpyDeviceToHost, s.stream));
    HIP_TRY(h, hipMemcpyAsync(s.h_pend + c_from, s.d_pend + c_from, (np - c_from) * sizeof(int16_t), hipMemcpyDeviceToHost, s.stream));
    s.packed_home = np, copied = true;
  }
  if (s.n_big) {
    HIP_TRY(h, hipMemcpyAsync(s.h_big, s.d_big, (size_t)s.n_big * sizeof(uint2), hipMemcpyDeviceToHost, s.stream));
    copied = true;
  }
  if (copied) HIP_TRY(h, hipStreamSynchronize(s.stream));
  s.want_packed = true, s.last_n_packed = np;
  out->n_reads = s.n_reads;
  out->n_candidates = np;
  out->count = s.h_count8, out->seg_begin = s.h_seg;
  out->cand = s.h_pcand, out->ed = s.h_ped, out->end = s.h_pend;
  out->big = (const uint32_t *)s.h_big, out->n_big = s.n_big;
  memcpy(out->stats, s.stats, sizeof s.stats);
  return FEM_OK;
}

int fem_dev_upload_reference_names(fem_dev *h, uint32_t n_seq, const char *names, const uint64_t *name_off) {
  if (!h || !names || !name_off || n_seq == 0) return FEM_ERR_INVALID;
  if (h->n_seq && n_seq != h->n_seq) return fail(h, FEM_ERR_INVALID, "as many names as reference sequences, please");
// ... 364 lines not shown
}

int fem_dev_set_rescue(fem_dev *h, int slot, const fem_rescue_params *rp) {
  int rc = check_slot(h, slot);
  if (rc) return rc;
  FEM_LOCK(h);
  Slot &s = h->slot[slot];
  if (!rp) {
    s.rescue = false;
    return FEM_OK;
  }
  if (rp->max_edits < 0 || rp->max_edits > 15) return fail(h, FEM_ERR_INVALID, "rescue edit bound out of range (0 <= max_edits <= 15)");
  s.rescue = true, s.rescue_edits = rp->max_edits;
  return FEM_OK;
}

int fem_dev_set_mapq(fem_dev *h, int slot, int on) {
  int rc = check_slot(h, slot);
  if (rc) return rc;
  FEM_LOCK(h);
  h->slot[slot].mapq = on != 0;
  return FEM_OK;
}

int fem_dev_set_unmapped(fem_dev *h, int slot, int on) {
  int rc = check_slot(h, slot);
  if (rc) return rc;
  FEM_LOCK(h);
  h->slot[slot].unmapped = on != 0;
  return FEM_OK;
}

int fem_dev_unmapped_count(fem_dev *h, int slot, uint64_t *n) {
  int rc = check_slot(h, slot);
  if (rc) return rc;
  if (!n) return fail(h, FEM_ERR_INVALID, "null output pointer");
  FEM_LOCK(h);
  *n = h->slot[slot].n_unmapped;
  return FEM_OK;
}

int fem_dev_rescue_count(fem_dev *h, int slot, uint64_t *n_rescued) {
  int rc = check_slot(h, slot);
  if (rc) return rc;
  if (!n_rescued) return fail(h, FEM_ERR_INVALID, "null output pointer");
  FEM_LOCK(h);
  Slot &s = h->slot[slot];
  if (!s.paired) return fail(h, FEM_ERR_STATE, "the slot is not in pair mode (fem_dev_set_pairs)");
  *n_rescued = s.n_rescued;
  return FEM_OK;
}

int fem_dev_fetch_pairs(fem_dev *h, int slot, fem_batch_pairs *out) {
  int rc = check_slot(h, slot);
  if (rc) return rc;
  if (!out) return fail(h, FEM_ERR_INVALID, "null result");
  if (!h->slot[slot].paired) return fail(h, FEM_ERR_STATE, "the slot is not in pair mode (fem_dev_set_pairs)");
  if ((rc = fem_dev_sync(h, slot))) return rc;
  Slot &s = h->slot[slot];
  if (s.n_reads & 1) return fail(h, FEM_ERR_INVALID, "a batch of read pairs holds an even number of reads");
  femt::RescueInput ri{};
  if ((rc = rescue_input(h, s, &ri))) return rc;
  fem_batch_records rec{};
  if ((rc = fem_dev_fetch_records(h, slot, &rec))) return rc;
  std::string err;
  femt::PairOutput po{};
  if ((rc = s.tail->pair(s.min_insert, s.max_insert, s.stream, &err, s.rescue ? &ri : nullptr))) return fail(h, rc, err);
  if ((rc = s.tail->pair_fetch(s.stream, &po, &err))) return fail(h, rc, err);
  const uint64_t nr = po.n_records;
  s.pr_flag.assign(po.flag, po.flag + nr);
  s.pr_tid.resize(nr), s.pr_pos0.resize(nr), s.pr_nm.resize(nr), s.pr_cigar_off.resize(nr + 1), s.pr_md_off.resize(nr + 1);
  s.pr_cigar.clear(), s.pr_md.clear();
  s.pr_cigar_off[0] = 0, s.pr_md_off[0] = 0;
  for (uint64_t k = 0; k < nr; ++k) {
    const uint32_t r = po.perm[k];
    if (r < po.first_rescued) {
      s.pr_tid[k] = rec.tid[r], s.pr_pos0[k] = rec.pos0[r], s.pr_nm[k] = rec.nm[r];
      s.pr_cigar.insert(s.pr_cigar.end(), rec.cigar + rec.cigar_off[r], rec.cigar + rec.cigar_off[r + 1]);
      s.pr_md.insert(s.pr_md.end(), rec.md + rec.md_off[r], rec.md + rec.md_off[r + 1]);
    } else {
      const uint32_t q = r - po.first_rescued, c0 = po.r_cigar_off[0], m0 = po.r_md_off[0];
      s.pr_tid[k] = po.r_tid[q], s.pr_pos0[k] = po.r_pos0[q], s.pr_nm[k] = po.r_nm[q];
      s.pr_cigar.insert(s.pr_cigar.end(), po.r_cigar + (po.r_cigar_off[q] - c0), po.r_cigar + (po.r_cigar_off[q + 1] - c0));
      s.pr_md.insert(s.pr_md.end(), po.r_md + (po.r_md_off[q] - m0), po.r_md + (po.r_md_off[q + 1] - m0));
    }
    s.pr_cigar_off[k + 1] = (uint32_t)s.pr_cigar.size(), s.pr_md_off[k + 1] = (uint32_t)s.pr_md.size();
  }
  s.n_proper = po.n_proper, s.n_rescued = po.n_rescued;
  out->n_pairs = po.n_pairs, out->n_records = nr;
  out->rec_begin = po.pair_begin, out->flag = s.pr_flag.data(), out->tid = s.pr_tid.data(), out->pos0 = s.pr_pos0.data();
  out->nm = s.pr_nm.data(), out->cigar_off = s.pr_cigar_off.data(), out->cigar = s.pr_cigar.data();
  out->md_off = s.pr_md_off.data(), out->md = s.pr_md.data();
  out->mate_tid = po.mate_tid, out->mate_pos0 = po.mate_pos0, out->tlen = po.tlen;
  out->n_proper = po.n_proper;
  memcpy(out->stats, s.stats, sizeof s.stats);
  return FEM_OK;
}

int fem_dev_map_batch_submit(fem_dev *h, int slot, const fem_params *p, const fem_read_batch *reads) {
  int rc = fem_dev_stage_reads(h, slot, reads);
  if (rc) return rc;
  return fem_dev_map_staged(h, slot, p);
}

int fem_dev_map_batch_wait(fem_dev *h, int slot, fem_batch_result *out) { return fem_dev_fetch(h, slot, out); }

int fem_dev_index_info(const fem_dev *h, char *buf, uint64_t cap) {
  if (!h || !buf || cap == 0) return FEM_ERR_INVALID;
  const uint64_t n_buckets = h->n_lookup ? h->n_lookup - 1 : 0;
  std::string s;
  if (!h->d_lookup) {
    s = "no index";
  } else if (h->d_occ32 && h->d_freq11) {
    s = "dense: 32-bit occurrence table, ";
    s += h->list_shift ? "strided with pads (" + std::to_string(((n_buckets + femk::kDensePadBuckets) << h->list_shift) * 4 >> 20) + " MiB)"
                       : "compact (" + std::to_string(h->n_occ * 4 >> 20) + " MiB)";
    s += ", " + std::to_string(h->n_banks) + (h->n_banks == 1 ? " bank" : " banks") + ", freq11 64 MiB";
  } else if (h->d_summary) {
    s = "sparse: bucket summaries";
  } else {
    s = "64-bit occurrence table only";
  }
  s += "; " + std::to_string(h->n_occ) + " entries in " + std::to_string(n_buckets) + " buckets";
  snprintf(buf, (size_t)cap, "%s", s.c_str());
  return FEM_OK;
}

const char *fem_dev_seed_kernel(const fem_dev *h, const fem_params *p) {
  if (!h || !params_ok(p)) return "";
  const int R = p->e + 1 + p->a;
  const bool use_fast = !h->force_generic && p->k == femk::kK && p->step == femk::kStep && R >= 1 && R <= femk::kMaxR;
  if (!use_fast) return "seed_filter_kernel";
  if (h->d_occ32 && h->d_freq11) return h->n_banks > 1 ? "seed_join_banked_kernel" : "seed_join_kernel";
  return (h->force_hash || (double)h->n_occ > (double)h->n_lookup) ? "seed_fast_kernel<hash>" : "seed_fast_kernel<lean>";
}

int fem_dev_set_timing(fem_dev *h, int on) {
  if (!h) return FEM_ERR_INVALID;
  h->timing = on != 0;
  if (h->timing && h->event_pool.size() < 64) {
    HIP_TRY(h, hipSetDevice(h->device));
    while (h->event_pool.size() < 64) {
      hipEvent_t e = nullptr;
      HIP_TRY(h, hipEventCreate(&e));
      h->event_pool.push_back(e);
    }
  }
  return FEM_OK;
}

int fem_dev_reset_timing(fem_dev *h) {
  if (!h) return FEM_ERR_INVALID;
  for (int i = 0; i < kTimedKernels; ++i) h->t_ms[i] = 0, h->t_n[i] = 0;
  if (h->timeline) {
    HIP_TRY(h, hipSetDevice(h->device));
    if (!h->ev_epoch) HIP_TRY(h, hipEventCreate(&h->ev_epoch));
    HIP_TRY(h, hipEventRecord(h->ev_epoch, h->side_stream));
    h->have_epoch = true;
  }
  return FEM_OK;
}

int fem_dev_kernel_time(fem_dev *h, int kernel, double *ms_total, uint64_t *launches) {
  if (!h || kernel < 0 || kernel >= kTimedKernels) return FEM_ERR_INVALID;
  if (ms_total) *ms_total = h->t_ms[kernel];
  if (launches) *launches = h->t_n[kernel];
  return FEM_OK;
}

int fem_dev_copy_bandwidth(fem_dev *h, uint64_t bytes, int iters, double *gb_per_s) {
  if (!h || !gb_per_s || bytes == 0 || iters <= 0) return FEM_ERR_INVALID;
  HIP_TRY(h, hipSetDevice(h->device));
  void *a = nullptr, *b = nullptr;
  HIP_TRY(h, hipMalloc(&a, bytes));
  if (hipMalloc(&b, bytes) != hipSuccess) {
    (void)hipFree(a);
    return fail(h, FEM_ERR_NOMEM, "copy bandwidth probe: out of memory");
  }
  hipStream_t st = h->slot[0].stream;
  hipEvent_t e0 = get_event(h), e1 = get_event(h);
  (void)hipMemsetAsync(a, 1, bytes, st);
  (void)hipMemcpyAsync(b, a, bytes, hipMemcpyDeviceToDevice, st);
  (void)hipEventRecord(e0, st);
  for (int i = 0; i < iters; ++i) (void)hipMemcpyAsync(b, a, bytes, hipMemcpyDeviceToDevice, st);
  (void)hipEventRecord(e1, st);
  hipError_t e = hipStreamSynchronize(st);
  float ms = 0.f;
  (void)hipEventElapsedTime(&ms, e0, e1);
  h->event_pool.push_back(e0);
  h->event_pool.push_back(e1);
  (void)hipFree(a);
  (void)hipFree(b);
  if (e != hipSuccess) return fail(h, FEM_ERR_HIP, hipGetErrorString(e));
  *gb_per_s = ms > 0 ? (2.0 * (double)bytes * iters) / (ms * 1e6) : 0.0;
  return FEM_OK;
}

int fem_dev_h2d_bandwidth(fem_dev *h, uint64_t bytes, int iters, double *gb_per_s) {
  if (!h || !gb_per_s || bytes == 0 || iters <= 0) return FEM_ERR_INVALID;
  HIP_TRY(h, hipSetDevice(h->device));
  void *a = nullptr, *b = nullptr;
  HIP_TRY(h, hipHostMalloc(&a, bytes, hipHostMallocDefault));
  if (hipMalloc(&b, bytes) != hipSuccess) {
    (void)hipHostFree(a);
    return fail(h, FEM_ERR_NOMEM, "h2d bandwidth probe: out of memory");
  }
  memset(a, 1, bytes);
  hipStream_t st = h->slot[0].stream;
  hipEvent_t e0 = get_event(h), e1 = get_event(h);
  (void)hipMemcpyAsync(b, a, bytes, hipMemcpyHostToDevice, st);
  (void)hipEventRecord(e0, st);
  for (int i = 0; i < iters; ++i) (void)hipMemcpyAsync(b, a, bytes, hipMemcpyHostToDevice, st);
  (void)hipEventRecord(e1, st);
  hipError_t e = hipStreamSynchronize(st);
  float ms = 0.f;
  (void)hipEventElapsedTime(&ms, e0, e1);
  h->event_pool.push_back(e0);
  h->event_pool.push_back(e1);
  (void)hipHostFree(a);
  (void)hipFree(b);
  if (e != hipSuccess) return fail(h, FEM_ERR_HIP, hipGetErrorString(e));
  *gb_per_s = ms > 0 ? ((double)bytes * iters) / (ms * 1e6) : 0.0;
  return FEM_OK;
}

#ifdef FEM_STAMPS
int fem_dbg_stamps(uint64_t *out, int n) {
  unsigned long long tmp[femk::kNumStamps];
  if (hipMemcpyFromSymbol(tmp, HIP_SYMBOL(femk::g_stamp_cycles), sizeof tmp) != hipSuccess) return -1;
  for (int i = 0; i < n && i < femk::kNumStamps; ++i) out[i] = tmp[i];
  memset(tmp, 0, sizeof tmp);
  (void)hipMemcpyToSymbol(HIP_SYMBOL(femk::g_stamp_cycles), tmp, sizeof tmp);
  return 0;
}
#endif

int fem_device_numa(int device, int32_t *node, char *cpulist, uint64_t cap) {
  if (node) *node = -1;
  if (cpulist && cap) cpulist[0] = 0;
  char bdf[64] = {0};
  if (hipDeviceGetPCIBusId(bdf, (int)sizeof bdf, device) != hipSuccess) return FEM_ERR_HIP;
  for (char *c = bdf; *c; ++c) *c = (char)tolower((unsigned char)*c);
  char path[160];
  snprintf(path, sizeof path, "/sys/bus/pci/devices/%s/numa_node", bdf);
  FILE *f = fopen(path, "r");
  if (!f) return FEM_OK;
  int n = -1;
  if (fscanf(f, "%d", &n) != 1) n = -1;
  fclose(f);
  if (node) *node = n;
  if (n >= 0 && cpulist && cap) {
    snprintf(path, sizeof path, "/sys/devices/system/node/node%d/cpulist", n);
    if ((f = fopen(path, "r"))) {
      if (!fgets(cpulist, (int)std::min<uint64_t>(cap, 1u << 20), f)) cpulist[0] = 0;
      fclose(f);
      for (char *c = cpulist; *c; ++c)
        if (*c == '\n') *c = 0;
    }
  }
  return FEM_OK;
}

int fem_bind_thread_near_device(int device) {
  const char *env = getenv("FEM_NUMA_BIND");
  if (env && env[0] == '0') return 1;
  int32_t node = -1;
  std::vector<char> list(4096, 0);
  if (fem_device_numa(device, &node, list.data(), list.size()) != FEM_OK || node < 0 || !list[0]) return 1;
  cpu_set_t now, want;
  CPU_ZERO(&now);
  CPU_ZERO(&want);
  if (sched_getaffinity(0, sizeof now, &now) != 0) return 1;
  int n_set = 0;
  for (const char *c = list.data(); *c;) {
    char *end = nullptr;
    const long lo = strtol(c, &end, 10);
    if (end == c) break;
    long hi = lo;
    if (*end == '-') hi = strtol(end + 1, &end, 10);
    for (long i = lo; i <= hi && i < CPU_SETSIZE; ++i)
      if (i >= 0 && CPU_ISSET((int)i, &now)) {
        CPU_SET((int)i, &want);
        ++n_set;
      }
    if (*end != ',') break;
    c = end + 1;
  }
  if (n_set == 0) return 1;
  return sched_setaffinity(0, sizeof want, &want) == 0 ? 0 : 1;
}

int fem_dev_allreduce_stats(fem_dev *const *hs, int n, uint64_t *stats) {
  if (!hs || n <= 0 || !stats) return FEM_ERR_INVALID;
  std::vector<int> devs(n);
  for (int i = 0; i < n; ++i) {
    if (!hs[i]) return FEM_ERR_INVALID;
    devs[i] = hs[i]->device;
  }
  fem_dev *h0 = hs[0];
  std::lock_guard<std::mutex> lock(g_comm_mu);
  if (!g_comm || g_comm->devs != devs) {
    destroy_comm_set();
    CommSet *cs = new (std::nothrow) CommSet();
    if (!cs) return fail(h0, FEM_ERR_NOMEM, "out of host memory");
    cs->devs = devs;
    cs->comms.assign(n, nullptr);
    cs->bufs.assign(n, nullptr);
    if (ncclCommInitAll(cs->comms.data(), n, devs.data()) != ncclSuccess) {
      delete cs;
      return fail(h0, FEM_ERR_RCCL, "ncclCommInitAll failed");
    }
    g_comm = cs;
    for (int i = 0; i < n; ++i)
      if (hipSetDevice(devs[i]) != hipSuccess || hipMalloc((void **)&cs->bufs[i], 5 * sizeof(uint64_t)) != hipSuccess) {
        destroy_comm_set();
        return fail(h0, FEM_ERR_HIP, "allreduce: allocating the counter buffers failed");
// ... 29 lines not shown
```

fem_amd/csrc/fem_kernels.hip.h:

```cpp
#pragma once
#include <hip/hip_runtime.h>
#include <stdint.h>
#include "fem_planes.hip.h"

namespace femk {

constexpr int kWave = 64;
constexpr uint32_t kFlagCandOverflow = 1u;
constexpr uint32_t kFlagArenaOverflow = 2u;
constexpr uint32_t kFlagTooLarge = 4u;
constexpr uint32_t kInvalidMeta = 0xFFFFFFFFu;
constexpr int kMaxR = 10;
constexpr uint32_t kMeta16 = 0x80000000u;
constexpr uint32_t kSlotChunk = 256u;
constexpr uint32_t kFlagQueueOverflow = 8u;
constexpr uint32_t kQueueChunk = 32u;
constexpr uint32_t kInvalidRead = 0xFFFFFFFFu;

struct SeedLayout {
  uint32_t pkw, nkw;
  uint32_t sf;
  uint32_t dp_rows;
  uint32_t dp_bits;
  uint32_t picked;
  uint32_t rb;
  uint32_t X, F, A, B;
  uint32_t xcap, fcap, ccap;
  uint32_t smax, cmax, cw;
  uint32_t n_words;
  uint32_t blk, blk_bytes;
  uint32_t gq, gq_cap;
  uint32_t strm, strm_words;
  uint32_t fq, gstride, nb;
  uint32_t rinfo;
  uint32_t wave_bytes;
};

struct SeedParams {
  const uint8_t *bases;
  const uint64_t *read_off;
  uint32_t n_reads;
  uint32_t read_begin;
  uint32_t *work_cursor;
  const uint32_t *lookup;
  const uint64_t *occ;
  uint32_t inf32;
  const uint32_t *seq_len;
  int32_t e, a, R, k, step, lg;
  uint64_t *cand;
  uint32_t *cand_meta;
  uint32_t cand_cap;
  uint32_t *cand_begin;
  uint32_t *cand_count;
  uint32_t *ctr;
  uint32_t n_seq;
  uint32_t *slow_queue;
  uint32_t slow_cap;
  const uint32_t *work_queue;
  const uint32_t *summary;
  const uint32_t *occ32;
  uint32_t list_shift;
  const uint32_t *goff;
  const uint32_t *blkseq;
  const uint32_t *freq11;
  uint2 *sel;
  uint2 *sel_hdr;
  uint32_t n_banks;
  uint32_t bank_first[5];
  const uint32_t *bank_lo;
  uint32_t n_buckets;
  uint32_t blk_stride;
  unsigned long long *stats;
  uint64_t *arena;
  unsigned long long arena_cap;
  unsigned long long *arena_ctr;
  SeedLayout lay;
};

__global__ void uniform_offsets_kernel(uint64_t *off, uint64_t n, uint32_t len) {
  const uint64_t stride = (uint64_t)gridDim.x * blockDim.x;
  for (uint64_t i = (uint64_t)blockIdx.x * blockDim.x + threadIdx.x; i <= n; i += stride) off[i] = i * (uint64_t)len;
}

__global__ void unpack_reads_kernel(const uint8_t *packed, uint64_t n_reads, uint32_t len, uint32_t bytes_per_read, uint8_t *bases) {
  const uint64_t stride = (uint64_t)gridDim.x * blockDim.x, total = n_reads * bytes_per_read;
  const bool aligned = (len & 3u) == 0u && (((uintptr_t)bases) & 3u) == 0u;
  for (uint64_t i = (uint64_t)blockIdx.x * blockDim.x + threadIdx.x; i < total; i += stride) {
    const uint32_t b = packed[i];
    const uint32_t c0 = (0x54474341u >> (8u * (b & 3u))) & 0xFFu, c1 = (0x54474341u >> (8u * ((b >> 2) & 3u))) & 0xFFu;
    const uint32_t c2 = (0x54474341u >> (8u * ((b >> 4) & 3u))) & 0xFFu, c3 = (0x54474341u >> (8u * (b >> 6))) & 0xFFu;
    if (aligned) {
      ((uint32_t *)bases)[i] = c0 | (c1 << 8) | (c2 << 16) | (c3 << 24);
    } else {
      const uint64_t r = i / bytes_per_read;
      const uint32_t k = (uint32_t)(i - r * bytes_per_read) * 4u;
      uint8_t *o = bases + r * len + k;
      o[0] = (uint8_t)c0;
      if (k + 1u < len) o[1] = (uint8_t)c1;
      if (k + 2u < len) o[2] = (uint8_t)c2;
      if (k + 3u < len) o[3] = (uint8_t)c3;
    }
  }
}
__global__ void scatter_chars_kernel(const uint32_t *at, const uint8_t *ch, uint64_t n, uint8_t *bases) {
  const uint64_t stride = (uint64_t)gridDim.x * blockDim.x;
  for (uint64_t i = (uint64_t)blockIdx.x * blockDim.x + threadIdx.x; i < n; i += stride) bases[at[i]] = ch[i];
}

__global__ void mark_exception_reads_kernel(const uint32_t *at, uint64_t n, uint32_t len, uint32_t *bits) {
  const uint64_t stride = (uint64_t)gridDim.x * blockDim.x;
  for (uint64_t i = (uint64_t)blockIdx.x * blockDim.x + threadIdx.x; i < n; i += stride) {
    const uint32_t r = at[i] / len;
    atomicOr(&bits[r >> 5], 1u << (r & 31u));
  }
}

struct Picked {
  uint32_t start, lo, freq, pad;
};

struct Bufs {
  uint64_t *X;
  uint64_t *F;
  uint64_t *A;
  uint64_t *B;
  uint32_t xcap, fcap, ccap;
};

__device__ __forceinline__ uint32_t lane_id() { return threadIdx.x & 63u; }

#ifdef FEM_STAMPS
constexpr int kNumStamps = 12;
__device__ unsigned long long g_stamp_cycles[kNumStamps];
struct Prof {
  unsigned long long acc[kNumStamps] = {};
  unsigned long long last = 0;
  __device__ void start() { last = __builtin_amdgcn_s_memtime(); }
  __device__ void mark(int id) {
    unsigned long long t = __builtin_amdgcn_s_memtime();
    acc[id] += t - last;
    last = t;
  }
  __device__ void flush() {
    if (lane_id() == 0)
      for (int i = 0; i < kNumStamps; ++i) atomicAdd(&g_stamp_cycles[i], acc[i]);
  }
};
#define STAMP_START(p) (p).start()
#define STAMP(p, id) (p).mark(id)
#else
struct Prof {};
#define STAMP_START(p) ((void)0)
#define STAMP(p, id) ((void)0)
#endif

__device__ __forceinline__ void wave_sync_lds() {
  __builtin_amdgcn_fence(__ATOMIC_RELEASE, "wavefront");
  __builtin_amdgcn_wave_barrier();
  __builtin_amdgcn_fence(__ATOMIC_ACQUIRE, "wavefront");
}
__device__ __forceinline__ void wave_sync_global() {
  __builtin_amdgcn_fence(__ATOMIC_RELEASE, "workgroup");
  __builtin_amdgcn_wave_barrier();
  __builtin_amdgcn_fence(__ATOMIC_ACQUIRE, "workgroup");
}
template <bool GLOBAL>
__device__ __forceinline__ void wave_sync() {
  if (GLOBAL)
    wave_sync_global();
  else
    wave_sync_lds();
}

__device__ __forceinline__ uint32_t bcast0(uint32_t v) { return __builtin_amdgcn_readfirstlane(v); }

__device__ __forceinline__ uint32_t base_code(uint32_t c) {
  uint32_t x = (c >> 1) & 3u;
  uint32_t code = x ^ (x >> 1);
  uint32_t u = c & 0xDFu;
  bool acgt = (u == 'A') | (u == 'C') | (u == 'G') | (u == 'T');
  return acgt ? code : 4u;
}

__device__ __forceinline__ uint32_t reverse_pairs(uint32_t x, int k) {
  uint32_t r = __brev(x) >> (32 - 2 * k);
  return ((r & 0x55555555u) << 1) | ((r >> 1) & 0x55555555u);
}

template <typename T>
__device__ __forceinline__ uint32_t lower_bound_u64(const T *x, uint32_t lo, uint32_t hi, uint64_t key) {
  while (lo < hi) {
    uint32_t mid = (lo + hi) >> 1;
    if (x[mid] < key)
      lo = mid + 1;
    else
      hi = mid;
  }
  return lo;
}
template <typename T>
__device__ __forceinline__ uint32_t upper_bound_u64(const T *x, uint32_t lo, uint32_t hi, uint64_t key) {
  while (lo < hi) {
    uint32_t mid = (lo + hi) >> 1;
    if (x[mid] <= key)
      lo = mid + 1;
    else
      hi = mid;
  }
  return lo;
}

template <bool GLOBAL>
__device__ uint32_t strand_lists(const SeedParams &p, const Picked *picked ,
                                 uint32_t *rb, const Bufs &b, uint64_t **result, Prof &prof) {
  const uint32_t ln = lane_id();
  const uint64_t lt_mask = (1ull << ln) - 1ull;
  const int R = p.R;
  const uint64_t e64 = (uint64_t)p.e;
  uint32_t *fb = rb + (R + 1);
  uint64_t *A = b.A, *B = b.B;
  uint32_t nA = 0;

  for (int si = 0; si < p.step; ++si) {
    const Picked *pk = picked + si * R;
    uint32_t n = 0;
// ... 781 lines not shown
    wave_sync_lds();
    STAMP(prof, 1);

    uint32_t pre_g = 0;
    uint32_t dp_w = 0;
    if (2u * (uint32_t)step * (uint32_t)R <= (uint32_t)kWave && R <= kMaxR) {
      uint32_t widest = (uint32_t)(S / step - R * lg + 1);
      dp_w = widest <= 16u ? 16u : widest <= 32u ? 32u : widest <= 64u ? 64u : 0u;
    }
    if (dp_w) {
      pre_g = select_seeds_dpp<0, 0, 0>(p, S, strand_ok, sf, smax, dp_w, (unsigned long long *)dp_bits, picked);
    } else if (ln < 2u * (uint32_t)step && strand_ok[ln / (uint32_t)step]) {
      const uint32_t strand = ln / (uint32_t)step, si = ln % (uint32_t)step;
      const int G = (S - (int)si) / step;
      const int C = G - R * lg + 2;
      uint32_t *rows = dp_rows + (size_t)ln * 2u * cmax;
      uint32_t *bits = dp_bits + (size_t)ln * (uint32_t)R * cw;
      const uint2 *sfs = sf + strand * smax;
      for (int c = 1; c < C; ++c) rows[c] = 0;
      uint32_t left = p.inf32;
      for (int row = 1; row <= R; ++row) {
        const uint32_t *prev = rows + (size_t)((row - 1) & 1) * cmax;
        uint32_t *cur = rows + (size_t)(row & 1) * cmax;
        left = p.inf32;
        uint32_t acc = 0;
        for (int col = 1; col < C; ++col) {
          uint32_t pos = (uint32_t)(col + (row - 1) * lg - 1);
          uint32_t with_new = prev[col] + sfs[si + (uint32_t)step * pos].y;
          bool take = with_new < left;
          left = take ? with_new : left;
          cur[col] = left;
          acc |= (uint32_t)take << (col & 31);
          if ((col & 31) == 31 || col == C - 1) {
            bits[(uint32_t)(row - 1) * cw + ((uint32_t)col >> 5)] = acc;
            acc = 0;
          }
        }
      }
      pre_g = left;
      Picked *out = picked + (size_t)ln * (uint32_t)R;
      for (int t = 0; t < R; ++t) out[t] = Picked{0, 0, 0, 0};
      int r = R, c = C - 1, n_out = 0;
      while (r > 0 && c > 0) {
        uint32_t bit = (bits[(uint32_t)(r - 1) * cw + ((uint32_t)c >> 5)] >> (c & 31)) & 1u;
        if (bit) {
          uint32_t sidx = si + (uint32_t)step * (uint32_t)(c + (r - 1) * lg - 1);
          uint2 s = sfs[sidx];
          out[n_out++] = Picked{sidx, s.x, s.y, 0};
          --r;
        } else {
          --c;
        }
      }
      for (int i = 1; i < R; ++i) {
        Picked t = out[i];
        int j = i;
        while (j > 0 && t.freq < out[j - 1].freq) {
          out[j] = out[j - 1];
          --j;
        }
        out[j] = t;
      }
    }
    wave_sync_lds();
    STAMP(prof, 2);

    for (uint32_t strand = 0; strand < 2; ++strand) {
      if (!strand_ok[strand]) {
        if (ln == 0) {
          p.cand_begin[read * 2u + strand] = 0;
          p.cand_count[read * 2u + strand] = 0;
        }
        continue;
      }
      uint32_t pre = 0, pre_max = 0;
      unsigned long long pre_wide = 0;
      for (int si = 0; si < step; ++si) {
        uint32_t v = __shfl(pre_g, (int)(strand * (uint32_t)step) + si);
        pre += v;
        pre_wide += v;
        pre_max = v > pre_max ? v : pre_max;
      }
      pre_sum += pre;
      const Picked *pk = picked + (size_t)strand * (uint32_t)step * (uint32_t)R;
      uint64_t *list = nullptr;
      STAMP(prof, 3);
      if (strand_small(p, pk, lds.X, read, strand, L, cand_sum, chunk)) {
        STAMP(prof, 8);
        continue;
      }
      uint32_t n = strand_lists<false>(p, pk, rb, lds, &list, prof);
      if (n < 0xFFFFFFFEu) {
        clip_and_emit<false>(p, read, strand, L, list, n, list == lds.A ? lds.B : lds.A, cand_sum, chunk);
      } else if (n == 0xFFFFFFFEu) {
        if (ln == 0) atomicOr(&p.ctr[1], kFlagTooLarge);
      } else {
        unsigned long long want = 2ull * pre_max + 2ull * pre_wide + 8ull;
        unsigned long long base = 0;
        if (ln == 0) {
          base = atomicAdd(&p.arena_ctr[0], want);
          atomicAdd(&p.arena_ctr[1], want);
        }
        base = ((unsigned long long)bcast0((uint32_t)(base >> 32)) << 32) | bcast0((uint32_t)base);
        if (base + want > p.arena_cap) {
          if (ln == 0) atomicOr(&p.ctr[1], kFlagArenaOverflow);
          if (ln == 0) {
            p.cand_begin[read * 2u + strand] = 0;
            p.cand_count[read * 2u + strand] = 0;
          }
        } else {
          Bufs g;
          g.X = p.arena + base;
          g.F = g.X + pre_max + 2;
          g.A = g.F + pre_max + 2;
          g.B = g.A + pre_wide + 2;
          g.xcap = pre_max + 1u, g.fcap = pre_max + 1u;
          g.ccap = pre_wide > 0x7ffffff0ull ? 0x7ffffff0u : (uint32_t)pre_wide + 1u;
          uint32_t n2 = strand_lists_big(p, pk, rb, g, lds.X, p.lay.xcap + p.lay.fcap + 2u * p.lay.ccap, &list, prof);
          if (n2 < 0xFFFFFFFEu) {
            clip_and_emit<true>(p, read, strand, L, list, n2, list == g.A ? g.B : g.A, cand_sum, chunk);
          } else {
            if (ln == 0) atomicOr(&p.ctr[1], kFlagTooLarge);
          }
        }
      }
      wave_sync_lds();
      STAMP(prof, 7);
    }
  }
  pad_chunk(p, chunk);
#ifdef FEM_STAMPS
  prof.flush();
#endif
  if (ln == 0) {
    if (pre_sum) atomicAdd(&p.stats[0], pre_sum);
    if (cand_sum) atomicAdd(&p.stats[1], cand_sum);
  }
}

struct VerifyParams {
  const uint8_t *bases;
  const uint64_t *read_off;
  const uint8_t *planes;
  const uint64_t *seq_off;
  const uint64_t *cand;
  const uint32_t *cand_meta;
  const uint32_t *ctr;
  uint32_t cand_cap;
  int32_t e;
  uint8_t *ed;
  int16_t *end;
  uint32_t *n_map;
  unsigned long long *stats;
};

__device__ __forceinline__ uint4 load_u128_unaligned(const uint8_t *p) {
  uint4 w;
  __builtin_memcpy(&w, p, 16);
  return w;
}

__device__ __forceinline__ uint4 plane_window(const uint8_t *planes, int q, uint64_t at) {
  return load_u128_unaligned(plane_addr(planes, q, at));
}
__device__ __forceinline__ uint32_t load_u32_unaligned(const uint8_t *p) {
  uint32_t w;
  __builtin_memcpy(&w, p, 4);
  return w;
}

struct MyersState {
  uint32_t VP, VN;
  int score;
};

__device__ __forceinline__ void decode4(uint32_t chars, uint32_t complement, uint32_t &code, uint32_t &nflag) {
  const uint32_t t = (chars >> 1) & 0x03030303u;
  const uint32_t c = t ^ ((t >> 1) & 0x01010101u);
  const uint32_t upper = chars & 0xDFDFDFDFu;
  const uint32_t expect = __builtin_amdgcn_perm(0u, 0x54474341u , c);
  const uint32_t z = upper ^ expect;
  nflag = ((((z & 0x7F7F7F7Fu) + 0x7F7F7F7Fu) | z) >> 7) & 0x01010101u;
  code = (c ^ complement) & ~(nflag * 3u);
}

__device__ __forceinline__ uint32_t window_head(const uint4 &w, uint32_t off) { return __builtin_amdgcn_alignbit(w.y, w.x, off); }
__device__ __forceinline__ void window_advance16(uint4 &w) {
  w.x = __builtin_amdgcn_alignbit(w.y, w.x, 16u), w.y = __builtin_amdgcn_alignbit(w.z, w.y, 16u);
  w.z = __builtin_amdgcn_alignbit(w.w, w.z, 16u), w.w >>= 16;
}

__device__ __forceinline__ void myers_column(MyersState &m, uint32_t B0, uint32_t B1, uint32_t B2, uint32_t m0, uint32_t m1,
                                             uint32_t m2, uint32_t j, uint32_t width, uint32_t wm) {
  const uint32_t eq = __builtin_amdgcn_ubfe(~((B0 ^ m0) | (B1 ^ m1) | (B2 ^ m2)), j, width);
  uint32_t X = eq | m.VN;
  const uint32_t D0 = ((((X & m.VP) + m.VP) ^ m.VP) | X) & wm;
  const uint32_t HN = m.VP & D0;
  const uint32_t HP = (m.VN | ~(m.VP | D0)) & wm;
  X = D0 >> 1;
  m.VN = X & HP;
  m.VP = (HN | ~(X | HP)) & wm;
  m.score += 1 - (int)(D0 & 1u);
}

constexpr int kStepsPerPlaneLoad = 6;

__global__ void __launch_bounds__(256) verify_kernel(VerifyParams p) {
  if (p.ctr[1] != 0) return;
  const uint32_t total = min(p.ctr[0], p.cand_cap);
  const uint32_t stride = gridDim.x * blockDim.x;
  const int e = p.e;
  const uint32_t width = 2u * (uint32_t)e + 1u;
  constexpr int kStageChunks = 4;
  __shared__ uint4 stage[kStageChunks][256];
  uint32_t(*part)[4] = (uint32_t(*)[4]) & stage[0][0];
  uint32_t mappings = 0, mapped = 0;
  for (uint32_t i = blockIdx.x * blockDim.x + threadIdx.x; i < total; i += stride) {
    const uint32_t meta = p.cand_meta[i];
    if (meta == kInvalidMeta) {
      p.ed[i] = 0xFF, p.end[i] = 0;
      continue;
    }
    const uint32_t read = (meta & ~kMeta16) >> 1, strand = meta & 1u;
    const uint32_t wm = (meta & kMeta16) ? 0xFFFFu : 0xFFFFFFFFu;
    const uint64_t c = p.cand[i];
    const uint64_t pat = p.seq_off[(uint32_t)(c >> 32)] + (uint32_t)c;
    const uint64_t off = p.read_off[read];
    const int L = (int)(p.read_off[read + 1] - off);
    const uint8_t *rd = p.bases + off;
    const uint32_t complement = strand ? 0x03030303u : 0u;
    MyersState m{0, 0, 0};
    bool rejected = false;
    const int n_steps = (L + 15) >> 4;
    auto text_chunk = [&](int col) { return load_u128_unaligned(strand == 0 ? rd + col : rd + (L - 16 - col)); };
    auto plane_chunk = [&](int q, int col) { return plane_window(p.planes, q, (pat + (uint32_t)col) >> 3); };
    uint4 P0 = make_uint4(0, 0, 0, 0), P1 = P0, P2 = P0, P0n = P0, P1n = P0, P2n = P0;
    if (n_steps > 0) {
      P0n = plane_chunk(0, 0), P1n = plane_chunk(1, 0), P2n = plane_chunk(2, 0);
    }
    const uint32_t pat_bit = (uint32_t)pat & 7u;
    for (int step = 0; step < n_steps && !rejected; ++step) {
      const int col = step << 4, sub = step % kStepsPerPlaneLoad;
      if (step % kStageChunks == 0) {
        uint4 t4[kStageChunks];
#pragma unroll
        for (int c = 0; c < kStageChunks; ++c) t4[c] = step + c < n_steps ? text_chunk(col + 16 * c) : make_uint4(0, 0, 0, 0);
#pragma unroll
        for (int c = 0; c < kStageChunks; ++c) stage[c][threadIdx.x] = t4[c];
      }
      const uint4 r = stage[step % kStageChunks][threadIdx.x];
      if (sub == 0) {
        P0 = P0n, P1 = P1n, P2 = P2n;
        if (step + kStepsPerPlaneLoad < n_steps) {
          const int nc = col + 16 * kStepsPerPlaneLoad;
          P0n = plane_chunk(0, nc), P1n = plane_chunk(1, nc), P2n = plane_chunk(2, nc);
        }
      } else {
        window_advance16(P0), window_advance16(P1), window_advance16(P2);
      }
      const uint32_t b0 = window_head(P0, pat_bit), b1 = window_head(P1, pat_bit), b2 = window_head(P2, pat_bit);
      uint32_t cw[4], nw[4];
      {
        const uint32_t w0 = strand ? __builtin_bswap32(r.w) : r.x, w1 = strand ? __builtin_bswap32(r.z) : r.y;
        const uint32_t w2 = strand ? __builtin_bswap32(r.y) : r.z, w3 = strand ? __builtin_bswap32(r.x) : r.w;
        decode4(w0, complement, cw[0], nw[0]);
        decode4(w1, complement, cw[1], nw[1]);
        decode4(w2, complement, cw[2], nw[2]);
        decode4(w3, complement, cw[3], nw[3]);
      }
      if (col + 16 <= L) {
#pragma unroll
        for (int q = 0; q < 16; ++q) {
          const uint32_t m0 = (uint32_t)__builtin_amdgcn_sbfe((int)cw[q >> 2], 8 * (q & 3), 1);
          const uint32_t m1 = (uint32_t)__builtin_amdgcn_sbfe((int)cw[q >> 2], 8 * (q & 3) + 1, 1);
          const uint32_t m2 = (uint32_t)__builtin_amdgcn_sbfe((int)nw[q >> 2], 8 * (q & 3), 1);
          myers_column(m, b0, b1, b2, m0, m1, m2, (uint32_t)q, width, wm);
        }
      } else {
        const uint64_t clo = ((uint64_t)cw[1] << 32) | cw[0], chi = ((uint64_t)cw[3] << 32) | cw[2];
        const uint64_t nlo = ((uint64_t)nw[1] << 32) | nw[0], nhi = ((uint64_t)nw[3] << 32) | nw[2];
        for (int q = 0; q < L - col; ++q) {
          const uint32_t cb = (uint32_t)((q < 8 ? clo : chi) >> (8 * (q & 7)));
          const uint32_t nb = (uint32_t)((q < 8 ? nlo : nhi) >> (8 * (q & 7)));
          myers_column(m, b0, b1, b2, 0u - (cb & 1u), 0u - ((cb >> 1) & 1u), 0u - (nb & 1u), (uint32_t)q, width, wm);
        }
      }
      rejected = m.score > 3 * e;
    }
    int score = m.score;
    int best = score, endp = L - 1;
    if (!rejected) {
      for (int j = 0; j < 2 * e; ++j) {
        score += (int)((m.VP >> j) & 1u) - (int)((m.VN >> j) & 1u);
        if (score < best) {
          best = score;
          endp = L + j;
        }
      }
    }
    const bool accepted = !rejected && best <= e;
    p.ed[i] = accepted ? (uint8_t)best : (uint8_t)0xFF;
    p.end[i] = accepted ? (int16_t)endp : (int16_t)0;
    {
      const uint32_t ln = lane_id();
      const uint64_t acc = __ballot(accepted);
      const uint32_t prev_read = __shfl_up(read, 1);
      const bool joins_prev = accepted && ln > 0u && ((acc >> (ln - 1u)) & 1ull) && prev_read == read;
      const uint64_t heads = __ballot(accepted && !joins_prev);
      if (accepted && !joins_prev) {
        const uint64_t stop = (heads | ~acc) >> ln >> 1;
        const uint32_t run = stop ? (uint32_t)__builtin_ctzll(stop) + 1u : 64u - ln;
        mapped += (uint32_t)(atomicAdd(&p.n_map[read], run) == 0u);
      }
      if (accepted) ++mappings;
    }
  }
  for (int d = 32; d >= 1; d >>= 1) mappings += __shfl_xor(mappings, d), mapped += __shfl_xor(mapped, d);
  __syncthreads();
  if (lane_id() == 0) part[0][threadIdx.x >> 6] = mappings, part[1][threadIdx.x >> 6] = mapped;
  __syncthreads();
  if (threadIdx.x == 0) {
    const uint32_t a = part[0][0] + part[0][1] + part[0][2] + part[0][3], b = part[1][0] + part[1][1] + part[1][2] + part[1][3];
    if (a) atomicAdd(&p.stats[2], (unsigned long long)a);
    if (b) atomicAdd(&p.stats[3], (unsigned long long)b);
  }
}

struct PackParams {
  const uint32_t *cand_begin, *cand_count;
  const uint64_t *cand;
  const uint8_t *ed;
  const int16_t *end;
  const uint32_t *ctr;
  uint32_t n_strands;
  uint8_t *count8;
  uint32_t *seg_begin;
  uint64_t *pcand;
  uint8_t *ped;
  int16_t *pend;
  uint32_t pcap;
  uint32_t *cursor;
  uint2 *big;
  uint32_t big_cap;
};
constexpr uint32_t kPackSegs = 16;
__global__ void __launch_bounds__(256) pack_results_kernel(PackParams p) {
  if (p.ctr[1] != 0) return;
  __shared__ uint32_t part[kPackSegs * 4u];
  __shared__ uint32_t block_base;
  const uint32_t seg0 = blockIdx.x * kPackSegs;
  const uint32_t wave = threadIdx.x >> 6;
  uint32_t cnt[kPackSegs], beg[kPackSegs], incl[kPackSegs];
#pragma unroll
  for (uint32_t i = 0; i < kPackSegs; ++i) {
    const uint32_t s = (seg0 + i) * 256u + threadIdx.x;
    const bool in = s < p.n_strands;
    cnt[i] = in ? p.cand_count[s] : 0u;
    beg[i] = in ? p.cand_begin[s] : 0u;
  }
#pragma unroll
  for (uint32_t i = 0; i < kPackSegs; ++i) {
    uint32_t x = cnt[i];
    for (int d = 1; d < 64; d <<= 1) {
      const uint32_t o = __shfl_up(x, d);
      if ((int)lane_id() >= d) x += o;
    }
    incl[i] = x;
    if (lane_id() == 63) part[i * 4u + wave] = x;
  }
  __syncthreads();
  if (threadIdx.x < 64u) {
    const uint32_t v = part[threadIdx.x];
    uint32_t x = v;
    for (int d = 1; d < 64; d <<= 1) {
      const uint32_t o = __shfl_up(x, d);
      if ((int)threadIdx.x >= d) x += o;
    }
    part[threadIdx.x] = x - v;
    if (threadIdx.x == 63u) block_base = x ? atomicAdd(&p.cursor[0], x) : 0u;
  }
  __syncthreads();
  const uint32_t n_seg = (p.n_strands + 255u) / 256u;
#pragma unroll
  for (uint32_t i = 0; i < kPackSegs; ++i) {
    const uint32_t seg = seg0 + i, s = seg * 256u + threadIdx.x;
    if (threadIdx.x == 0 && seg < n_seg) p.seg_begin[seg] = block_base + part[i * 4u];
    if (s >= p.n_strands) continue;
    const uint32_t c = cnt[i], at = block_base + part[i * 4u + wave] + incl[i] - c;
    p.count8[s] = (uint8_t)(c < 255u ? c : 255u);
    if (c >= 255u) {
      const uint32_t j = atomicAdd(&p.cursor[1], 1u);
      if (j < p.big_cap) p.big[j] = make_uint2(s, c);
    }
    for (uint32_t k = 0; k < c; ++k) {
      if (at + k >= p.pcap) break;
      p.pcand[at + k] = p.cand[beg[i] + k];
      p.ped[at + k] = p.ed[beg[i] + k];
      p.pend[at + k] = p.end[beg[i] + k];
    }
  }
}

__global__ void ref_planes_kernel(const uint8_t *codes, const uint8_t *raw, uint64_t n_bytes, uint8_t *planes) {
  const uint64_t stride = (uint64_t)gridDim.x * blockDim.x;
  for (uint64_t b = (uint64_t)blockIdx.x * blockDim.x + threadIdx.x; b < n_bytes; b += stride) {
    uint64_t w, r;
    __builtin_memcpy(&w, codes + 8 * b, 8);
    __builtin_memcpy(&r, raw + 8 * b, 8);
    uint32_t o[4] = {0, 0, 0, 0};
    for (int k = 0; k < 8; ++k) {
      const uint32_t c = (uint32_t)(w >> (8 * k)) & 0xFFu, ch = (uint32_t)(r >> (8 * k)) & 0xFFu;
      o[0] |= (c & 1u) << k, o[1] |= ((c >> 1) & 1u) << k, o[2] |= ((c >> 2) & 1u) << k;
      o[3] |= (uint32_t)(ch != ((0x4E54474341ull >> (8u * c)) & 0xFFu)) << k;
    }
    const uint64_t g = b >> 4, r16 = b & 15u;
    for (int q = 0; q < 4; ++q) {
      planes[g * kPlaneGroup + (uint32_t)q * 32u + r16] = (uint8_t)o[q];
      if (g) planes[(g - 1) * kPlaneGroup + (uint32_t)q * 32u + 16u + r16] = (uint8_t)o[q];
    }
  }
}

constexpr uint32_t kSummaryBuckets = 24;

__device__ __forceinline__ void summary_slot(uint32_t h, uint32_t &q, uint32_t &r) {
  q = (uint32_t)((float)(h >> 3) * 0.33333334f);
  r = h - __umul24(q, kSummaryBuckets);
}
__device__ __forceinline__ bool summary_nonempty(uint32_t w, uint32_t r) { return (w >> r) & 1u; }
__device__ __forceinline__ bool summary_multi(uint32_t w, uint32_t r) { return (w >> (kSummaryBuckets + (__umul24(r, 11u) >> 5))) & 1u; }

__global__ void bucket_summary_kernel(const uint32_t *lookup, uint64_t n_buckets, uint32_t *summary) {
  const uint64_t stride = (uint64_t)gridDim.x * blockDim.x;
  for (uint64_t h = (uint64_t)blockIdx.x * blockDim.x + threadIdx.x; h < n_buckets; h += stride) {
    const uint32_t f = lookup[h + 1] - lookup[h];
    if (f == 0u) continue;
    const uint32_t q = (uint32_t)(h / kSummaryBuckets), r = (uint32_t)(h % kSummaryBuckets);
    atomicOr(&summary[q], (1u << r) | (f >= 2u ? 1u << (kSummaryBuckets + r / 3u) : 0u));
  }
}

__global__ void ref_encode_kernel(uint8_t *text, uint64_t n) {
  uint64_t stride = (uint64_t)gridDim.x * blockDim.x;
  for (uint64_t i = (uint64_t)blockIdx.x * blockDim.x + threadIdx.x; i < n; i += stride)
    text[i] = (uint8_t)base_code(text[i]);
}

}
```

fem_amd/csrc/fem_seed_join.hip.h:

```cpp
#pragma once
#include "fem_seed_dense.hip.h"

namespace femk {

#ifndef FEM_JOIN_SLOTS_HI
#define FEM_JOIN_SLOTS_HI 32768u
#endif
#ifndef FEM_JOIN_OPT
#define FEM_JOIN_OPT 15
#endif
#ifndef FEM_JOIN_OPT_HI
#define FEM_JOIN_OPT_HI 12
#endif
#ifndef FEM_JOIN_ABL
#define FEM_JOIN_ABL 0
#endif
#ifndef FEM_JOIN_SLOTS_LO
#define FEM_JOIN_SLOTS_LO 32768u
#endif
constexpr uint32_t join_slots(int R, bool padded = false) { return R >= 7 ? FEM_JOIN_SLOTS_HI : padded ? FEM_JOIN_SLOTS_LO : 32768u; }
#ifndef FEM_JOIN_BATCH_HI
#define FEM_JOIN_BATCH_HI 3
#endif

// ... 332 lines not shown
      }
    }
    if (kSecondProbe && n_flag > kProbeMin) {
      const bool have0 = ln < n_flag, have1 = ln + (uint32_t)kWave < n_flag;
      const uint32_t v0 = have0 ? flg_g[ln] : 0u, v1 = have1 ? flg_g[ln + (uint32_t)kWave] : 0u;
      auto key2 = [&](uint32_t v) -> uint32_t {
        const uint32_t slot2 = (__builtin_amdgcn_ubfe(v, 3u, kSlotBits) + (v >> kPeriodBits) * 0x9E5u) & (kSlots - 1u);
        return (slot2 << 3) | (v & 7u);
      };
      auto edge = [&](uint32_t v) -> bool {
        const uint32_t lo = v & ((1u << kPeriodBits) - 1u);
        return lo < e || lo + e >= (1u << kPeriodBits);
      };
      auto wipe = [&](uint32_t k) {
        const uint32_t qm = (k >> 3) - 1u;
        uint32_t *w = bitmap + __builtin_amdgcn_ubfe(qm, 5u, kWordBits);
        w[0] = 0u, w[1] = 0u;
      };
      const uint32_t k0 = key2(v0), k1 = key2(v1);
      const uint32_t h0 = insert(have0 ? k0 : kDenseSent), h1 = insert(have1 ? k1 : kDenseSent);
      if (__builtin_amdgcn_ballot_w64((h0 | h1) != 0u)) mark(k0, h0), mark(k1, h1);
      wave_sync_lds();
      const bool keep0 = have0 && (edge(v0) || (window(k0) & 5u) != 0u);
      const bool keep1 = have1 && (edge(v1) || (window(k1) & 5u) != 0u);
      wave_sync_lds();
      if (have0) wipe(k0);
      if (have1) wipe(k1);
      wave_sync_lds();
      if (ln == 0) bitmap[kWords] = 0xFFFFFFFFu;
      const uint64_t m0 = __builtin_amdgcn_ballot_w64(keep0), m1 = __builtin_amdgcn_ballot_w64(keep1);
      const uint32_t c0 = (uint32_t)__popcll(m0);
      if (keep0) flg_g[__builtin_amdgcn_mbcnt_hi((uint32_t)(m0 >> 32), __builtin_amdgcn_mbcnt_lo((uint32_t)m0, 0u))] = v0;
      if (keep1) flg_g[__builtin_amdgcn_mbcnt_hi((uint32_t)(m1 >> 32), __builtin_amdgcn_mbcnt_lo((uint32_t)m1, c0))] = v1;
      n_flag = c0 + (uint32_t)__popcll(m1);
      wave_sync_lds();
      if (kOptPairs) {
        if (ln >= n_flag) flg_g[ln] = 0xFFFFFFFFu;
        if (kFlagCap > (uint32_t)kWave && ln + (uint32_t)kWave >= n_flag) flg_g[ln + (uint32_t)kWave] = 0xFFFFFFFFu;
        wave_sync_lds();
      }
    }
    if (!(FEM_JOIN_ABL & 2) && n_flag > (uint32_t)p.a) {
      const bool have = ln < n_flag;
      uint32_t fv;
      uint32_t cnt = 0;
      bool pass_hi = false;
      uint32_t fv_hi = 0;
      if (kOptPairs && n_flag <= 8u) {
        const uint32_t xj = flg_g[ln & 7u], fi = flg_g[ln >> 3];
        const uint64_t m = __builtin_amdgcn_ballot_w64(xj - fi <= e);
        cnt = (uint32_t)__popc((uint32_t)(m >> (8u * (ln & 7u))) & 0xFFu);
        fv = have ? xj : 0u;
      } else if (kOptPairs && n_flag <= 16u) {
        const uint32_t xj = flg_g[ln & 15u];
        const uint32_t *fp = flg_g + (ln >> 4);
        const uint64_t m0 = __builtin_amdgcn_ballot_w64(xj - fp[0] <= e), m1 = __builtin_amdgcn_ballot_w64(xj - fp[4] <= e);
        const uint64_t m2 = __builtin_amdgcn_ballot_w64(xj - fp[8] <= e), m3 = __builtin_amdgcn_ballot_w64(xj - fp[12] <= e);
        const uint32_t r0 = (uint32_t)(m0 >> sh16), r1 = (uint32_t)(m1 >> sh16), r2 = (uint32_t)(m2 >> sh16), r3 = (uint32_t)(m3 >> sh16);
        uint32_t row = r0;
        asm("v_cndmask_b32 %0, %0, %1, %2" : "+v"(row) : "v"(r1), "s"(q_is1));
        asm("v_cndmask_b32 %0, %0, %1, %2" : "+v"(row) : "v"(r2), "s"(q_is2));
        asm("v_cndmask_b32 %0, %0, %1, %2" : "+v"(row) : "v"(r3), "s"(q_is3));
        cnt = (uint32_t)__popc(row & 0xFFFFu);
        fv = have ? xj : 0u;
      } else {
        fv = have ? flg_g[ln] : 0u;
        const uint32_t n_lo = n_flag < (uint32_t)kWave ? n_flag : (uint32_t)kWave;
        if (kFlagCap > (uint32_t)kWave && n_flag > (uint32_t)kWave) {
          const bool have_hi = ln + (uint32_t)kWave < n_flag;
          fv_hi = have_hi ? flg_g[ln + (uint32_t)kWave] : 0u;
          uint32_t cnt_hi = 0;
          for (uint32_t j = 0; j < n_lo; ++j) {
            const uint32_t x = (uint32_t)__builtin_amdgcn_readlane((int)fv, (int)j);
            cnt += (uint32_t)(x - fv <= e), cnt_hi += (uint32_t)(x - fv_hi <= e);
          }
          for (uint32_t j = (uint32_t)kWave; j < n_flag; ++j) {
            const uint32_t x = (uint32_t)__builtin_amdgcn_readlane((int)fv_hi, (int)(j - (uint32_t)kWave));
            cnt += (uint32_t)(x - fv <= e), cnt_hi += (uint32_t)(x - fv_hi <= e);
          }
          pass_hi = have_hi && cnt_hi > (uint32_t)p.a;
        } else {
          for (uint32_t j = 0; j < n_lo; ++j) {
            const uint32_t x = (uint32_t)__builtin_amdgcn_readlane((int)fv, (int)j);
            cnt += (uint32_t)(x - fv <= e);
          }
        }
      }
      const bool pass = have && cnt > (uint32_t)p.a;
      const uint64_t pm = __builtin_amdgcn_ballot_w64(pass);
      if (__builtin_amdgcn_ballot_w64(pass_hi)) {
        any_hi = true;
        cmin = pass_hi && fv_hi < cmin ? fv_hi : cmin;
        cmax = pass_hi && fv_hi > cmax ? fv_hi : cmax;
      }
      if (pm != 0) {
        if (g == 0) pm0 = pm, nf0 = n_flag;
        else if (g == 1) pm1 = pm, nf1 = n_flag;
        else pm2 = pm, nf2 = n_flag;
        cmin = pass && fv < cmin ? fv : cmin;
        cmax = pass && fv > cmax ? fv : cmax;
      }
    }
    if (g != (uint32_t)kStep - 1u) continue;
    uint32_t kept = 0, cv = 0;
    if ((pm0 | pm1 | pm2) != 0 || any_hi) {
      const uint32_t lo_all = wave_min_u32(cmin), hi_all = wave_max_u32(cmax);
      if (hi_all - lo_all <= e) {
        cv = ln == 0 ? lo_all : 0u;
        kept = 1;
      } else if (any_hi) {
        return false;
      } else {
#pragma unroll 1
        for (uint32_t gg = 0; gg < (uint32_t)kStep; ++gg) {
          const uint64_t pm = gg == 0 ? pm0 : gg == 1 ? pm1 : pm2;
          const uint32_t nfl = gg == 0 ? nf0 : gg == 1 ? nf1 : nf2;
          if (pm == 0) continue;
          const uint32_t nF = (uint32_t)__popcll(pm);
          const bool mine = (pm >> ln) & 1ull;
          const uint32_t fv = ln < nfl ? flg[gg * kFlgStride + ln] : 0u;
          uint32_t rank = 0;
          for (uint64_t m = pm; m;) {
            const int j = __builtin_ctzll(m);
            m &= m - 1;
            const uint32_t x = (uint32_t)__builtin_amdgcn_readlane((int)fv, j);
            rank += (uint32_t)(x < fv || (x == fv && (uint32_t)j < ln));
          }
          wave_sync_lds();
          if (mine) scatter[rank] = fv;
          wave_sync_lds();
          const uint32_t fs = ln < nF ? scatter[ln] : 0u;
          kept = dense_merge_group(cv, kept, fs, nF, e);
          if (kept == 0xFFFFFFFFu) return false;
        }
      }
    }
    cand_lds[(u >= (uint32_t)kStep ? (uint32_t)kWave : 0u) + ln] = cv;
    if (u >= (uint32_t)kStep) kept1 = kept; else kept0 = kept;
    cmin = 0xFFFFFFFFu, cmax = 0u, any_hi = false;
    pm0 = pm1 = pm2 = 0, nf0 = nf1 = nf2 = 0;
  }
  return true;
}

#ifndef FEM_JOIN_WAVES_LO
#define FEM_JOIN_WAVES_LO 7
#endif
#ifndef FEM_JOIN_WAVES_HI
#define FEM_JOIN_WAVES_HI 6
#endif

constexpr int join_waves(int R) { return R <= 6 ? FEM_JOIN_WAVES_LO : FEM_JOIN_WAVES_HI; }

template <int R, bool BANKED = false, bool PADDED = false>
__device__ __forceinline__ void seed_join_body(const SeedParams &p, uint8_t *smem) {
  constexpr uint32_t kSeeds = (uint32_t)(kStep * R);
  static_assert(2 * kStep * R <= kWave, "both strands' seeds must fit the lanes of one wave");
  const uint32_t ln = lane_id();
  const uint32_t wave_in_block = (uint32_t)__builtin_amdgcn_readfirstlane((int)(threadIdx.x >> 6));
  uint8_t *wbase = smem + (size_t)wave_in_block * p.lay.wave_bytes;
  uint32_t *scatter = (uint32_t *)(wbase + p.lay.X);
  uint32_t *flg = (uint32_t *)(wbase + p.lay.A);
  uint32_t *bitmap = (uint32_t *)(wbase + p.lay.F);
  uint2 *blk_entries = (uint2 *)(wbase + p.lay.B);
  uint32_t *cand_lds = (uint32_t *)(wbase + p.lay.sf);
  uint2 *seqtab = (uint2 *)(smem + p.lay.picked);
  const bool small_ref = p.n_seq <= (uint32_t)kWave;
  if (wave_in_block == 0) seqtab[ln] = ln < p.n_seq ? make_uint2(p.goff[ln], p.seq_len[ln]) : make_uint2(0xFFFFFFFFu, 0u);
  __syncthreads();
  for (uint32_t i = ln; i < join_bitmap_words(R, PADDED); i += kWave) bitmap[i] = i < join_slots(R, PADDED) / 32u ? 0u : 0xFFFFFFFFu;
  wave_sync_lds();
  unsigned long long pre_sum = 0, cand_sum = 0;
  SlotChunk chunk, qchunk;

  auto queue_slow = [&](uint32_t read) {
    if (qchunk.left == 0) {
      uint32_t base = 0;
      if (ln == 0) base = atomicAdd(&p.ctr[2], kQueueChunk);
      qchunk.next = bcast0(base);
      qchunk.left = kQueueChunk;
    }
    if (qchunk.next < p.slow_cap) {
      if (ln == 0) p.slow_queue[qchunk.next] = read;
    } else if (ln == 0) {
      atomicOr(&p.ctr[1], kFlagQueueOverflow);
    }
    ++qchunk.next, --qchunk.left;
  };

  for (;;) {
    uint32_t pull = 0;
    if (ln == 0) pull = atomicAdd(p.work_cursor, kReadBlock);
    pull = bcast0(pull);
    if ((uint64_t)p.read_begin + pull >= p.n_reads) break;
    const uint32_t r0 = p.read_begin + pull;
    const uint32_t n_blk = p.n_reads - r0 < kReadBlock ? p.n_reads - r0 : kReadBlock;
    if (ln < 2u * kReadBlock) blk_entries[ln] = make_uint2(kBlkSkip, 0u);
    uint2 hdr = make_uint2(kSelSlow, 0u);
    if (ln < n_blk) hdr = p.sel_hdr[r0 + ln];
    uint2 sel_next = make_uint2(0u, 0u);
    if (!BANKED && ln < 2u * kSeeds) sel_next = p.sel[(size_t)r0 * (2u * kSeeds) + ln];
    for (uint32_t rb = 0; rb < n_blk; ++rb) {
      const uint32_t read = r0 + rb;
      const uint32_t h0 = (uint32_t)__builtin_amdgcn_readlane((int)hdr.x, (int)rb);
      const uint32_t status = h0 & 3u, L = h0 >> 8;
      const uint2 sel = sel_next;
      if (!BANKED && rb + 1u < n_blk && ln < 2u * kSeeds) sel_next = p.sel[(size_t)(read + 1u) * (2u * kSeeds) + ln];
      if (status == kSelSlow) continue;
      if (status == kSelNone) {
        if (ln / 2u == rb) blk_entries[ln] = make_uint2(0u, 0u);
        continue;
      }
      if constexpr (BANKED) {
        constexpr uint32_t kStash = (uint32_t)kWave;
        uint64_t *stash = (uint64_t *)(wbase + p.lay.gq);
        uint32_t acc[2] = {0u, 0u};
        bool failed = false;
        for (uint32_t b = 0; b < p.n_banks && !failed; ++b) {
          uint2 sel_b = make_uint2(0u, 0u);
          if (ln < 2u * kSeeds) sel_b = p.sel[((size_t)read * p.n_banks + b) * (2u * kSeeds) + ln];
          uint32_t kept0 = 0, kept1 = 0;
          if (!join_read<R, true>(p, sel_b.y & 0xFFFFu, sel_b.x, sel_b.y >> 16, bitmap, flg, scatter, cand_lds, kept0, kept1, p.bank_first[b])) {
            failed = true;
            break;
          }
          const uint32_t sq_lo = p.bank_first[b], sq_hi = p.bank_first[b + 1u];
#pragma unroll 1
          for (uint32_t strand = 0; strand < 2u; ++strand) {
            const uint32_t kept = strand ? kept1 : kept0;
            if (kept == 0) continue;
            const uint32_t v = cand_lds[strand * (uint32_t)kWave + ln];
            uint32_t sq = 0, pos = 0, slen = 0;
            if (small_ref) {
              const uint2 tab = seqtab[ln];
              const bool mine = ln >= sq_lo && ln < sq_hi;
              for (uint32_t i = 0; i < kept; ++i) {
                const uint32_t vi = (uint32_t)__builtin_amdgcn_readlane((int)v, (int)i);
                const uint32_t s_i = sq_lo + (uint32_t)__popcll(__builtin_amdgcn_ballot_w64(mine && tab.x <= vi)) - 1u;
                const uint32_t g_i = (uint32_t)__builtin_amdgcn_readlane((int)tab.x, (int)s_i);
                const uint32_t l_i = (uint32_t)__builtin_amdgcn_readlane((int)tab.y, (int)s_i);
                if (ln == i) sq = s_i, pos = vi - g_i, slen = l_i;
              }
            } else if (ln < kept) {
              sq = p.blkseq[(size_t)b * p.blk_stride + (v >> kDenseBlkShift)];
              while (sq + 1u < sq_hi && p.goff[sq + 1u] <= v) ++sq;
              pos = v - p.goff[sq];
              slen = p.seq_len[sq];
            }
            const bool ok = ln < kept && pos >= (uint32_t)p.e && pos + L + (uint32_t)p.e < slen;
            const uint64_t mo = __ballot(ok);
            const uint32_t n_ok = (uint32_t)__popcll(mo);
            if (acc[strand] + n_ok > kStash) {
              failed = true;
              break;
            }
            if (ok) stash[strand * kStash + acc[strand] + (uint32_t)__popcll(mo & ((1ull << ln) - 1ull))] = (((uint64_t)sq << 32) | pos) - (uint64_t)p.e;
            acc[strand] += n_ok;
          }
        }
        if (failed) {
          queue_slow(read);
          continue;
        }
        pre_sum += (uint32_t)__builtin_amdgcn_readlane((int)hdr.y, (int)rb);
        wave_sync_lds();
#pragma unroll 1
        for (uint32_t strand = 0; strand < 2u; ++strand) {
          const uint32_t n_out = acc[strand];
          uint32_t base = 0;
          if (n_out > 0) {
            if (n_out <= chunk.left) {
              base = chunk.next;
              chunk.next += n_out, chunk.left -= n_out;
            } else {
              pad_chunk(p, chunk);
              if (ln == 0) base = atomicAdd(&p.ctr[0], kSlotChunk);
              base = bcast0(base);
              chunk.next = base + n_out, chunk.left = kSlotChunk - n_out;
            }
            if ((unsigned long long)base + n_out > p.cand_cap) {
              if (ln == 0) atomicOr(&p.ctr[1], kFlagCandOverflow);
            } else {
              for (uint32_t i = ln; i < n_out; i += (uint32_t)kWave) {
                p.cand[base + i] = stash[strand * kStash + i];
                p.cand_meta[base + i] = (read * 2u + strand) | (i < (n_out & ~7u) ? kMeta16 : 0u);
              }
            }
          }
          if (ln == 0) blk_entries[2u * rb + strand] = make_uint2(base, n_out);
          cand_sum += n_out;
        }
        wave_sync_lds();
        continue;
      }
      const uint32_t s_lo = sel.x, s_start = sel.y & 0xFFFFu, s_freq = sel.y >> 16;
      uint32_t kept0 = 0, kept1 = 0;
      if (!join_read<R, false, PADDED>(p, s_start, s_lo, s_freq, bitmap, flg, scatter, cand_lds, kept0, kept1)) {
        queue_slow(read);
        continue;
      }
      if (FEM_JOIN_ABL & 16) kept0 = kept1 = 0;
      pre_sum += (uint32_t)__builtin_amdgcn_readlane((int)hdr.y, (int)rb);
#pragma unroll 1
      for (uint32_t strand = 0; strand < 2u; ++strand) {
        const uint32_t kept = strand ? kept1 : kept0;
        uint64_t out = 0;
        bool ok = false;
        if (kept == 0) {
          if (ln == 0) blk_entries[2u * rb + strand] = make_uint2(0u, 0u);
          continue;
        }
        const uint32_t v = cand_lds[strand * (uint32_t)kWave + ln];
        uint32_t sq = 0, pos = 0, slen = 0;
        if (small_ref) {
          const uint2 tab = seqtab[ln];
          for (uint32_t i = 0; i < kept; ++i) {
            const uint32_t vi = (uint32_t)__builtin_amdgcn_readlane((int)v, (int)i);
            const uint32_t s_i = (uint32_t)__popcll(__builtin_amdgcn_ballot_w64(tab.x <= vi)) - 1u;
            const uint32_t g_i = (uint32_t)__builtin_amdgcn_readlane((int)tab.x, (int)s_i);
            const uint32_t l_i = (uint32_t)__builtin_amdgcn_readlane((int)tab.y, (int)s_i);
            if (ln == i) sq = s_i, pos = vi - g_i, slen = l_i;
          }
        } else if (ln < kept) {
          sq = p.blkseq[v >> kDenseBlkShift];
          while (sq + 1u < p.n_seq && p.goff[sq + 1u] <= v) ++sq;
          pos = v - p.goff[sq];
          slen = p.seq_len[sq];
        }
        if (ln < kept) {
          ok = pos >= (uint32_t)p.e && pos + L + (uint32_t)p.e < slen;
          out = (((uint64_t)sq << 32) | pos) - (uint64_t)p.e;
        }
        const uint64_t mo = __ballot(ok);
        const uint32_t n_out = (uint32_t)__popcll(mo);
        uint32_t base = 0;
        if (n_out > 0) {
          if (n_out <= chunk.left) {
            base = chunk.next;
            chunk.next += n_out, chunk.left -= n_out;
          } else {
            pad_chunk(p, chunk);
            if (ln == 0) base = atomicAdd(&p.ctr[0], kSlotChunk);
            base = bcast0(base);
            chunk.next = base + n_out, chunk.left = kSlotChunk - n_out;
          }
          if ((unsigned long long)base + n_out > p.cand_cap) {
            if (ln == 0) atomicOr(&p.ctr[1], kFlagCandOverflow);
          } else if (ok) {
            const uint32_t rank = (uint32_t)__popcll(mo & ((1ull << ln) - 1ull)), at = base + rank;
            p.cand[at] = out;
            p.cand_meta[at] = (read * 2u + strand) | (rank < (n_out & ~7u) ? kMeta16 : 0u);
          }
        }
        if (ln == 0) blk_entries[2u * rb + strand] = make_uint2(base, n_out);
        cand_sum += n_out;
      }
    }
    wave_sync_lds();
    const uint2 entry = blk_entries[ln];
    wave_sync_lds();
    if (ln < 2u * kReadBlock && r0 + ln / 2u < p.n_reads && entry.x != kBlkSkip) {
      __builtin_nontemporal_store(entry.x, &p.cand_begin[r0 * 2u + ln]);
      __builtin_nontemporal_store(entry.y, &p.cand_count[r0 * 2u + ln]);
    }
  }
  pad_chunk(p, chunk);
  for (uint32_t i = ln; i < qchunk.left; i += kWave)
    if (qchunk.next + i < p.slow_cap) p.slow_queue[qchunk.next + i] = kInvalidRead;
  if (ln == 0) {
    if (pre_sum) atomicAdd(&p.stats[0], pre_sum);
    if (cand_sum) atomicAdd(&p.stats[1], cand_sum);
  }
}


#define FEM_JOIN_KERNEL(R, WAVES)                                                                                               \
  __global__ void __launch_bounds__(256) __attribute__((amdgpu_waves_per_eu(WAVES, 8))) seed_join_kernel_r##R(SeedParams p) {                         \
    extern __shared__ __attribute__((aligned(16))) uint8_t smem[];                                                               \
    seed_join_body<R>(p, smem);                                                                                                  \
  }                                                                                                                              \
  __global__ void __launch_bounds__(256) __attribute__((amdgpu_waves_per_eu(FEM_JOIN_WAVES_HI, 8))) seed_join_banked_kernel_r##R(SeedParams p) {  \
    extern __shared__ __attribute__((aligned(16))) uint8_t smem[];                                                               \
    seed_join_body<R, true>(p, smem);                                                                                            \
  }                                                                                                                              \
  __global__ void __launch_bounds__(256) __attribute__((amdgpu_waves_per_eu(WAVES, 8))) seed_join_kernel_padded_r##R(SeedParams p) {  \
    extern __shared__ __attribute__((aligned(16))) uint8_t smem[];                                                               \
    seed_join_body<R, false, true>(p, smem);                                                                                     \
  }
FEM_JOIN_KERNEL(1, FEM_JOIN_WAVES_LO)
FEM_JOIN_KERNEL(2, FEM_JOIN_WAVES_LO)
FEM_JOIN_KERNEL(3, FEM_JOIN_WAVES_LO)
FEM_JOIN_KERNEL(4, FEM_JOIN_WAVES_LO)
FEM_JOIN_KERNEL(5, FEM_JOIN_WAVES_LO)
FEM_JOIN_KERNEL(6, FEM_JOIN_WAVES_LO)
FEM_JOIN_KERNEL(7, FEM_JOIN_WAVES_HI)
FEM_JOIN_KERNEL(8, FEM_JOIN_WAVES_HI)
FEM_JOIN_KERNEL(9, FEM_JOIN_WAVES_HI)
FEM_JOIN_KERNEL(10, FEM_JOIN_WAVES_HI)
#undef FEM_JOIN_KERNEL

}
```

fem_amd/device.py:

```python
import ctypes as C
import os

import numpy as np

_HERE = os.path.dirname(os.path.abspath(__file__))
_HIP = None

ABI_SYMBOLS = [
    "fem_dev_open", "fem_dev_close", "fem_strerror", "fem_dev_last_error", "fem_dev_limits",
    "fem_dev_upload_index", "fem_dev_upload_reference", "fem_dev_build_index", "fem_dev_fetch_index",
    "fem_dev_map_batch_submit", "fem_dev_map_batch_wait",
    "fem_dev_stage_reads", "fem_dev_stage_info", "fem_dev_acquire_stage", "fem_dev_commit_stage", "fem_dev_commit_stage_uniform", "fem_dev_packed_layout", "fem_dev_commit_stage_packed", "fem_dev_map_staged", "fem_dev_sync", "fem_dev_fetch_stats", "fem_dev_fetch", "fem_dev_fetch_packed",
    "fem_dev_fetch_records", "fem_dev_seed_kernel", "fem_dev_index_info",
    "fem_dev_upload_reference_names", "fem_dev_acquire_text_stage", "fem_dev_commit_text_stage", "fem_dev_commit_names_stage", "fem_dev_sam_quals", "fem_dev_reserve_text", "fem_dev_reserve_batch", "fem_set_blocking_waits", "fem_dev_fetch_sam", "fem_dev_fetch_sam_nowait", "fem_dev_sam_wait",
    "fem_dev_set_timing", "fem_dev_reset_timing", "fem_dev_kernel_time", "fem_dev_copy_bandwidth",
    "fem_dev_h2d_bandwidth",
    "fem_device_numa", "fem_bind_thread_near_device",
    "fem_dev_allreduce_stats",
    "fem_dev_set_pairs", "fem_dev_fetch_pairs", "fem_dev_pair_count",
    "fem_dev_set_rescue", "fem_dev_rescue_count", "fem_dev_set_mapq",
    "fem_dev_set_unmapped", "fem_dev_unmapped_count",
    "fem_dev_fetch_bam", "fem_dev_fetch_bam_nowait", "fem_dev_bam_wait", "fem_dev_bgzf_compress",
]

# ... 388 lines not shown
        st = np.zeros(5, dtype=np.uint64)
        self._check(self._L.fem_dev_fetch_stats(self._h, slot, st.ctypes.data))
        return st

    def fetch(self, slot=0, copy=True):
        r = _BatchResult()
        self._check(self._L.fem_dev_fetch(self._h, slot, C.byref(r)))
        return BatchResult(r, copy)

    def fetch_packed(self, slot=0, copy=True):
        r = _BatchPacked()
        self._check(self._L.fem_dev_fetch_packed(self._h, slot, C.byref(r)))
        return BatchPacked(r, copy)

    def seed_kernel(self, e=3, a=1, k=12, step=3):
        p = Params(k, step, e, a)
        return self._L.fem_dev_seed_kernel(self._h, C.byref(p)).decode()

    def index_info(self):
        buf = C.create_string_buffer(512)
        self._check(self._L.fem_dev_index_info(self._h, buf, 512))
        return buf.value.decode()

    def reserve_batch(self, n_reads, n_records, max_len, e=3, a=1, k=12, step=3, slot=0):
        p = Params(k, step, e, a)
        self._check(self._L.fem_dev_reserve_batch(self._h, slot, n_reads, n_records, max_len, C.byref(p)))

    def fetch_records(self, slot=0):
        r = _BatchRecords()
        self._check(self._L.fem_dev_fetch_records(self._h, slot, C.byref(r)))
        return BatchRecords(r)

    def upload_reference_names(self, names):
        raw = [n.encode() if isinstance(n, str) else bytes(n) for n in names]
        off = np.zeros(len(raw) + 1, np.uint64)
        off[1:] = np.cumsum([len(n) for n in raw])
        self._check(self._L.fem_dev_upload_reference_names(self._h, len(raw), b"".join(raw), off.ctypes.data))

    def stage_text(self, quals, names, slot=0, quals_on_host=False):
        raw = [n.encode() if isinstance(n, str) else bytes(n) for n in names]
        q = np.frombuffer(bytes(quals), np.uint8) if not isinstance(quals, np.ndarray) else quals
        nn = sum(len(n) for n in raw)
        pq, pn, po = C.c_void_p(), C.c_void_p(), C.c_void_p()
        self._check(self._L.fem_dev_acquire_text_stage(self._h, slot, len(raw), len(q), nn, C.byref(pq), C.byref(pn), C.byref(po)))
        if len(q):
            C.memmove(pq.value, q.ctypes.data, len(q))
        if nn:
            C.memmove(pn.value, b"".join(raw), nn)
        off = np.zeros(len(raw) + 1, np.uint64)
        off[1:] = np.cumsum([len(n) for n in raw])
        C.memmove(po.value, off.ctypes.data, 8 * (len(raw) + 1))
        if quals_on_host:
            self._check(self._L.fem_dev_commit_names_stage(self._h, slot, len(raw), nn))
        else:
            self._check(self._L.fem_dev_commit_text_stage(self._h, slot, len(raw), nn))

    def fetch_sam(self, slot=0, nowait=False, quals=None, offsets=None):
        r = _BatchSam()
        if nowait:
            self._check(self._L.fem_dev_fetch_sam_nowait(self._h, slot, C.byref(r)))
            self._check(self._L.fem_dev_sam_wait(self._h, slot))
        else:
            self._check(self._L.fem_dev_fetch_sam(self._h, slot, C.byref(r)))
        if quals is not None and r.len:
            from fem_amd import host
            qa, nq = C.c_void_p(), C.c_uint64()
            self._check(self._L.fem_dev_sam_quals(self._h, slot, C.byref(qa), C.byref(nq)))
            q = np.ascontiguousarray(quals, dtype=np.uint8)
            o = np.ascontiguousarray(offsets, dtype=np.uint64)
            rc = host.lib().fem_sam_fill_quals(r.text, r.len, qa.value, nq.value, q.ctypes.data, o.ctypes.data, 0, 3)
            if rc:
                raise FemError("fem_sam_fill_quals failed (%d)" % rc)
        text = C.string_at(r.text, r.len) if r.len else b""
        return text, int(r.n_records), int(r.n_asserted), np.array(list(r.stats), dtype=np.uint64)

    def fetch_bam(self, slot=0, level=1, nowait=False):
        r = _BatchBam()
        if nowait:
            self._check(self._L.fem_dev_fetch_bam_nowait(self._h, slot, int(level), C.byref(r)))
            self._check(self._L.fem_dev_bam_wait(self._h, slot))
        else:
            self._check(self._L.fem_dev_fetch_bam(self._h, slot, int(level), C.byref(r)))
        data = C.string_at(r.data, r.len) if r.len else b""
        return (data, int(r.raw_len), int(r.n_blocks), int(r.n_records), int(r.n_asserted),
                np.array(list(r.stats), dtype=np.uint64))

    def bgzf_compress(self, data, level=1):
        raw = bytes(data)
        cap = 65536 * (len(raw) // 65280 + 1)
        out = C.create_string_buffer(cap)
        n = C.c_uint64()
        self._check(self._L.fem_dev_bgzf_compress(self._h, raw, len(raw), int(level), out, cap, C.byref(n)))
        return out.raw[:n.value]

    def set_pairs(self, min_insert=0, max_insert=500, slot=0):
        if min_insert is None:
            self._check(self._L.fem_dev_set_pairs(self._h, slot, None))
        else:
            pp = _PairParams(int(min_insert), int(max_insert))
            self._check(self._L.fem_dev_set_pairs(self._h, slot, C.byref(pp)))

    def fetch_pairs(self, slot=0):
        r = _BatchPairs()
        self._check(self._L.fem_dev_fetch_pairs(self._h, slot, C.byref(r)))
        return BatchPairs(r)

    def pair_count(self, slot=0):
        n = C.c_uint64()
        self._check(self._L.fem_dev_pair_count(self._h, slot, C.byref(n)))
        return int(n.value)

    def set_rescue(self, max_edits=None, slot=0):
        if max_edits is None:
            self._check(self._L.fem_dev_set_rescue(self._h, slot, None))
        else:
            rp = _RescueParams(int(max_edits))
            self._check(self._L.fem_dev_set_rescue(self._h, slot, C.byref(rp)))

    def set_mapq(self, on=True, slot=0):
        self._check(self._L.fem_dev_set_mapq(self._h, slot, 1 if on else 0))

    def set_unmapped(self, on=True, slot=0):
        self._check(self._L.fem_dev_set_unmapped(self._h, slot, 1 if on else 0))

    def unmapped_count(self, slot=0):
        n = C.c_uint64()
        self._check(self._L.fem_dev_unmapped_count(self._h, slot, C.byref(n)))
        return int(n.value)

    def rescue_count(self, slot=0):
        n = C.c_uint64()
        self._check(self._L.fem_dev_rescue_count(self._h, slot, C.byref(n)))
        return int(n.value)

    def map_batch(self, bases, offsets, e=3, a=1, k=12, step=3, slot=0):
        b, keep = self._batch(bases, offsets)
        p = Params(k, step, e, a)
        self._check(self._L.fem_dev_map_batch_submit(self._h, slot, C.byref(p), C.byref(b)))
        r = _BatchResult()
        self._check(self._L.fem_dev_map_batch_wait(self._h, slot, C.byref(r)))
        return BatchResult(r)

    def set_timing(self, on=True):
        self._check(self._L.fem_dev_set_timing(self._h, int(on)))

    def reset_timing(self):
        self._check(self._L.fem_dev_reset_timing(self._h))

    def kernel_time(self, kernel):
        ms, n = C.c_double(), C.c_uint64()
        self._check(self._L.fem_dev_kernel_time(self._h, kernel, C.byref(ms), C.byref(n)))
        return ms.value, int(n.value)

    def h2d_bandwidth(self, nbytes=1 << 28, iters=8):
        g = C.c_double()
        self._check(self._L.fem_dev_h2d_bandwidth(self._h, nbytes, iters, C.byref(g)))
        return g.value

    def copy_bandwidth(self, nbytes=1 << 30, iters=10):
        g = C.c_double()
        self._check(self._L.fem_dev_copy_bandwidth(self._h, nbytes, iters, C.byref(g)))
        return g.value
```

Baseline: 337.5.

## Verify finished candidate chunks inside seed-join tail to overlap verification

Seed-join waves now mark each 256-candidate slot chunk finished, writing candidates with agent-scope stores. After their own join work they claim finished chunks through a shared cursor and run Myers verification on them in-kernel, marking those chunks verified. The separate verify kernel then skips verified chunks. This fills the idle tail of the join kernel with verification work so the verify pass has less to do. In exchange it adds write-through stores, per-chunk state memsets, a noinline tail function that may raise register pressure, and cross-kernel memory-ordering risk.

```diff
diff --git a/fem_amd/csrc/fem_hip.hip b/fem_amd/csrc/fem_hip.hip
--- a/fem_amd/csrc/fem_hip.hip
+++ b/fem_amd/csrc/fem_hip.hip
@@ -40,6 +40,7 @@
 constexpr uint32_t kXcapSmall = 512, kFcap = 128, kCcap = 128;
 
 constexpr int kTimedKernels = 15;
+constexpr int kTailChunksId = 100;
 struct TimedLaunch {
   int kernel;
   hipEvent_t start, stop;
@@ -96,6 +97,8 @@
   uint8_t *d_ed = nullptr;
   int16_t *d_end = nullptr;
   uint32_t cand_cap = 0;
+  uint32_t *d_chunk_state = nullptr;
+  size_t chunk_state_words = 0;
   uint32_t *d_begin = nullptr, *d_count = nullptr, *d_nmap = nullptr;
   size_t per_read_cap = 0;
   uint8_t *d_ctl = nullptr;
@@ -151,11 +154,14 @@
 };
 
 constexpr size_t kCtlPackCursor = 4 * sizeof(uint32_t) + 2 * sizeof(uint64_t) + 4 * sizeof(uint64_t);
-constexpr size_t kCtlBytes = kCtlPackCursor + 2 * sizeof(uint32_t);
+constexpr size_t kCtlTailChunks = kCtlPackCursor + 2 * sizeof(uint32_t);
+constexpr size_t kCtlBytes = kCtlTailChunks + 2 * sizeof(uint32_t);
 constexpr uint32_t kBigCap = 4096;
 constexpr size_t kCtlWorkCursor = 128, kCtlWorkCursor2 = 192, kCtlPartStride = 128, kCtlAlloc = 1024;
 static_assert(kCtlWorkCursor2 + (kMaxParts - 1) * kCtlPartStride + 64 <= kCtlAlloc, "control block layout");
 static_assert(kCtlBytes <= kCtlWorkCursor, "control block layout");
+constexpr size_t kCtlVerifyCursor = 704;
+static_assert(kCtlWorkCursor2 + (kMaxParts - 1) * kCtlPartStride + 64 <= kCtlVerifyCursor && kCtlVerifyCursor + 64 <= kCtlAlloc, "control block layout");
 
 }
 
@@ -261,6 +267,9 @@
   bool force_hash = false;
   bool force_dense = false;
   bool no_dense = false;
+  bool no_tail_verify = false;
+  uint32_t tail_max_chunks = 0xFFFFFFFFu;
+  uint64_t tail_chunks = 0, tail_chunks_of = 0;
   bool tiny_buffers = false;
   std::vector<hipEvent_t> event_pool;
   hipEvent_t ev_kernels_done = nullptr;
@@ -615,6 +624,16 @@
   s.pending.clear();
 }
 
+int ensure_chunk_state(fem_dev *h, Slot &s, uint64_t cand_cap) {
+  const size_t words = (size_t)((cand_cap / femk::kSlotChunk + 4u) & ~3ull);
+  if (s.d_chunk_state && words <= s.chunk_state_words) return FEM_OK;
+  if (s.d_chunk_state) (void)hipFree(s.d_chunk_state);
+  s.d_chunk_state = nullptr, s.chunk_state_words = 0;
+  HIP_TRY(h, hipMalloc((void **)&s.d_chunk_state, words * sizeof(uint32_t)));
+  s.chunk_state_words = words;
+  return FEM_OK;
+}
+
 int ensure_outputs(fem_dev *h, Slot &s) {
   size_t want_reads = (size_t)s.n_reads;
   if (want_reads > s.per_read_cap || !s.d_begin) {
@@ -642,6 +661,7 @@
     if ((rc = dev_realloc(h, &s.d_meta, &c1, want))) return rc;
     if ((rc = dev_realloc(h, &s.d_ed, &c2, want))) return rc;
     if ((rc = dev_realloc(h, &s.d_end, &c3, want))) return rc;
+    if ((rc = ensure_chunk_state(h, s, want))) return rc;
     s.cand_cap = (uint32_t)want;
   }
   if (!s.d_ctl) {
@@ -676,6 +696,8 @@
   HIP_TRY(h, hipMalloc((void **)&s.d_meta, want * sizeof(uint32_t)));
   HIP_TRY(h, hipMalloc((void **)&s.d_ed, want * sizeof(uint8_t)));
   HIP_TRY(h, hipMalloc((void **)&s.d_end, want * sizeof(int16_t)));
+  int rc = ensure_chunk_state(h, s, want);
+  if (rc) return rc;
   s.cand_cap = (uint32_t)want;
   return FEM_OK;
 }
@@ -796,11 +818,16 @@
     }
     s.parts = 1;
   }
+  const bool tail_verify = !h->no_tail_verify && s.d_chunk_state && s.n_reads && !h->force_generic && p.k == femk::kK && p.step == femk::kStep &&
+                           p.e + 1 + p.a >= 1 && p.e + 1 + p.a <= femk::kMaxR && h->d_occ32 && h->d_freq11;
+  const size_t state_bytes = std::min<size_t>(s.chunk_state_words, ((size_t)s.cand_cap / femk::kSlotChunk + 4u) & ~(size_t)3u) * sizeof(uint32_t);
   if (parts > 1) {
     if (h->have_select_done) HIP_TRY(h, hipStreamWaitEvent(h->side_stream, h->ev_select_done, 0));
     HIP_TRY(h, hipMemsetAsync(s.d_ctl, 0, kCtlAlloc, h->side_stream));
+    if (tail_verify) HIP_TRY(h, hipMemsetAsync(s.d_chunk_state, 0, state_bytes, h->side_stream));
   } else {
     HIP_TRY(h, hipMemsetAsync(s.d_ctl, 0, kCtlAlloc, s.stream));
+    if (tail_verify) HIP_TRY(h, hipMemsetAsync(s.d_chunk_state, 0, state_bytes, s.stream));
   }
 
   femk::SeedParams sp{};
@@ -867,6 +894,7 @@
     vp.ctr = d_ctr, vp.cand_cap = s.cand_cap, vp.e = p.e;
     vp.ed = s.d_ed, vp.end = s.d_end;
     vp.n_map = s.d_nmap, vp.stats = d_stats;
+    vp.chunk_state = tail_verify ? s.d_chunk_state : nullptr;
     HIP_TRY(h, hipMemsetAsync(s.d_nmap, 0, (size_t)s.n_reads * sizeof(uint32_t), s.stream));
     if (h->verify_blocks_per_cu == 0) {
       int nb = 0;
@@ -886,6 +914,12 @@
       fp.n_banks = h->n_banks, fp.bank_lo = h->d_bank_lo, fp.n_buckets = (uint32_t)(h->n_lookup - 1);
       fp.blk_stride = (femk::kDenseRemap >> femk::kDenseBlkShift) + 1u;
       for (uint32_t b = 0; b <= femk::kDenseMaxBanks; ++b) fp.bank_first[b] = h->bank_first[b];
+      if (tail_verify) {
+        fp.chunk_state = s.d_chunk_state;
+        fp.verify_cursor = (uint32_t *)(s.d_ctl + kCtlVerifyCursor), fp.tail_chunks = (uint32_t *)(s.d_ctl + kCtlTailChunks);
+        fp.tail_max_chunks = h->tail_max_chunks;
+        fp.planes = h->d_planes, fp.seq_off = h->d_seq_off, fp.ed = s.d_ed, fp.end = s.d_end, fp.n_map = s.d_nmap;
+      }
       uint32_t select_lds = 0, select_threads = 256;
       fp.lay = make_layout_select(p, max_len);
       if (fp.lay.wave_bytes > 64u * 1024u) return fail(h, FEM_ERR_UNSUPPORTED, "read too long for the device path");
@@ -1313,6 +1347,8 @@
     h->no_dense = testing_switch("FEM_NO_DENSE");
     h->no_strided = testing_switch("FEM_NO_STRIDED");
     h->tiny_buffers = testing_switch("FEM_TEST_TINY_BUFFERS");
+    h->no_tail_verify = testing_switch("FEM_NO_TAIL_VERIFY");
+    if (const char *tm = getenv("FEM_TAIL_MAX_CHUNKS")) h->tail_max_chunks = (uint32_t)strtoul(tm, nullptr, 10);
     if (const char *bl = getenv("FEM_TEST_BANK_BASES")) h->bank_limit = strtoull(bl, nullptr, 10);
     if (const char *bs = getenv("FEM_TEST_BANK_SEQS")) h->bank_seqs = (uint32_t)strtoul(bs, nullptr, 10);
   }
@@ -1335,7 +1371,8 @@
     for (void *p : {(void *)s.d_bases_alloc, (void *)s.d_off, (void *)s.d_cand, (void *)s.d_meta, (void *)s.d_ed,
                     (void *)s.d_end, (void *)s.d_begin, (void *)s.d_count, (void *)s.d_nmap, (void *)s.d_ctl,
                     (void *)s.d_arena, (void *)s.d_slow, (void *)s.d_sel, (void *)s.d_sel_hdr, (void *)s.d_packed, (void *)s.d_exc_bits, (void *)s.d_quals, (void *)s.d_names,
-                    (void *)s.d_name_off, (void *)s.d_count8, (void *)s.d_seg, (void *)s.d_pcand, (void *)s.d_ped, (void *)s.d_pend, (void *)s.d_big})
+                    (void *)s.d_name_off, (void *)s.d_count8, (void *)s.d_seg, (void *)s.d_pcand, (void *)s.d_ped, (void *)s.d_pend, (void *)s.d_big,
+                    (void *)s.d_chunk_state})
       if (p) (void)hipFree(p);
     for (void *p : {(void *)s.h_ctl, (void *)s.h_begin, (void *)s.h_count, (void *)s.h_cand, (void *)s.h_ed,
                     (void *)s.h_end, (void *)s.h_bases, (void *)s.h_off, (void *)s.h_quals, (void *)s.h_names, (void *)s.h_name_off,
@@ -1758,6 +1795,7 @@
     if (flags == 0) {
       s.n_cand = ctr[0];
       s.n_packed = ((const uint32_t *)(s.h_ctl + kCtlPackCursor))[0], s.n_big = ((const uint32_t *)(s.h_ctl + kCtlPackCursor))[1];
+      h->tail_chunks += ((const uint32_t *)(s.h_ctl + kCtlTailChunks))[0], h->tail_chunks_of += (ctr[0] + femk::kSlotChunk - 1u) / femk::kSlotChunk;
       s.stats[0] = s.n_reads;
       s.stats[1] = st[3];
       s.stats[2] = st[0];
@@ -2428,6 +2466,7 @@
 int fem_dev_reset_timing(fem_dev *h) {
   if (!h) return FEM_ERR_INVALID;
   for (int i = 0; i < kTimedKernels; ++i) h->t_ms[i] = 0, h->t_n[i] = 0;
+  h->tail_chunks = 0, h->tail_chunks_of = 0;
   if (h->timeline) {
     HIP_TRY(h, hipSetDevice(h->device));
     if (!h->ev_epoch) HIP_TRY(h, hipEventCreate(&h->ev_epoch));
@@ -2438,6 +2477,11 @@
 }
 
 int fem_dev_kernel_time(fem_dev *h, int kernel, double *ms_total, uint64_t *launches) {
+  if (h && kernel == kTailChunksId) {
+    if (ms_total) *ms_total = (double)h->tail_chunks_of;
+    if (launches) *launches = h->tail_chunks;
+    return FEM_OK;
+  }
   if (!h || kernel < 0 || kernel >= kTimedKernels) return FEM_ERR_INVALID;
   if (ms_total) *ms_total = h->t_ms[kernel];
   if (launches) *launches = h->t_n[kernel];
diff --git a/fem_amd/csrc/fem_kernels.hip.h b/fem_amd/csrc/fem_kernels.hip.h
--- a/fem_amd/csrc/fem_kernels.hip.h
+++ b/fem_amd/csrc/fem_kernels.hip.h
@@ -13,6 +13,7 @@
 constexpr int kMaxR = 10;
 constexpr uint32_t kMeta16 = 0x80000000u;
 constexpr uint32_t kSlotChunk = 256u;
+constexpr uint32_t kChunkOpen = 0u, kChunkFinished = 1u, kChunkVerified = 2u;
 constexpr uint32_t kFlagQueueOverflow = 8u;
 constexpr uint32_t kQueueChunk = 32u;
 constexpr uint32_t kInvalidRead = 0xFFFFFFFFu;
@@ -71,6 +72,15 @@
   uint32_t n_buckets;
   uint32_t blk_stride;
   unsigned long long *stats;
+  uint32_t *chunk_state;
+  uint32_t *verify_cursor;
+  uint32_t *tail_chunks;
+  uint32_t tail_max_chunks;
+  const uint8_t *planes;
+  const uint64_t *seq_off;
+  uint8_t *ed;
+  int16_t *end;
+  uint32_t *n_map;
   uint64_t *arena;
   unsigned long long arena_cap;
   unsigned long long *arena_ctr;
@@ -1158,6 +1168,7 @@
   int16_t *end;
   uint32_t *n_map;
   unsigned long long *stats;
+  const uint32_t *chunk_state;
 };
 
 __device__ __forceinline__ uint4 load_u128_unaligned(const uint8_t *p) {
@@ -1211,115 +1222,123 @@
 
 constexpr int kStepsPerPlaneLoad = 6;
 
+constexpr int kStageChunks = 4;
+
+template <uint32_t STRIDE>
+__device__ __forceinline__ void verify_candidate(const VerifyParams &p, uint32_t i, uint4 *stage, int e, uint32_t width, uint32_t &mappings,
+                                                 uint32_t &mapped) {
+  const uint32_t meta = p.cand_meta[i];
+  if (meta == kInvalidMeta) {
+    p.ed[i] = 0xFF, p.end[i] = 0;
+    return;
+  }
+  const uint32_t read = (meta & ~kMeta16) >> 1, strand = meta & 1u;
+  const uint32_t wm = (meta & kMeta16) ? 0xFFFFu : 0xFFFFFFFFu;
+  const uint64_t c = p.cand[i];
+  const uint64_t pat = p.seq_off[(uint32_t)(c >> 32)] + (uint32_t)c;
+  const uint64_t off = p.read_off[read];
+  const int L = (int)(p.read_off[read + 1] - off);
+  const uint8_t *rd = p.bases + off;
+  const uint32_t complement = strand ? 0x03030303u : 0u;
+  MyersState m{0, 0, 0};
+  bool rejected = false;
+  const int n_steps = (L + 15) >> 4;
+  auto text_chunk = [&](int col) { return load_u128_unaligned(strand == 0 ? rd + col : rd + (L - 16 - col)); };
+  auto plane_chunk = [&](int q, int col) { return plane_window(p.planes, q, (pat + (uint32_t)col) >> 3); };
+  uint4 P0 = make_uint4(0, 0, 0, 0), P1 = P0, P2 = P0, P0n = P0, P1n = P0, P2n = P0;
+  if (n_steps > 0) {
+    P0n = plane_chunk(0, 0), P1n = plane_chunk(1, 0), P2n = plane_chunk(2, 0);
+  }
+  const uint32_t pat_bit = (uint32_t)pat & 7u;
+  for (int step = 0; step < n_steps && !rejected; ++step) {
+    const int col = step << 4, sub = step % kStepsPerPlaneLoad;
+    if (step % kStageChunks == 0) {
+      uint4 t4[kStageChunks];
+#pragma unroll
+      for (int c = 0; c < kStageChunks; ++c) t4[c] = step + c < n_steps ? text_chunk(col + 16 * c) : make_uint4(0, 0, 0, 0);
+#pragma unroll
+      for (int c = 0; c < kStageChunks; ++c) stage[c * STRIDE] = t4[c];
+    }
+    const uint4 r = stage[(step % kStageChunks) * STRIDE];
+    if (sub == 0) {
+      P0 = P0n, P1 = P1n, P2 = P2n;
+      if (step + kStepsPerPlaneLoad < n_steps) {
+        const int nc = col + 16 * kStepsPerPlaneLoad;
+        P0n = plane_chunk(0, nc), P1n = plane_chunk(1, nc), P2n = plane_chunk(2, nc);
+      }
+    } else {
+      window_advance16(P0), window_advance16(P1), window_advance16(P2);
+    }
+    const uint32_t b0 = window_head(P0, pat_bit), b1 = window_head(P1, pat_bit), b2 = window_head(P2, pat_bit);
+    uint32_t cw[4], nw[4];
+    {
+      const uint32_t w0 = strand ? __builtin_bswap32(r.w) : r.x, w1 = strand ? __builtin_bswap32(r.z) : r.y;
+      const uint32_t w2 = strand ? __builtin_bswap32(r.y) : r.z, w3 = strand ? __builtin_bswap32(r.x) : r.w;
+      decode4(w0, complement, cw[0], nw[0]);
+      decode4(w1, complement, cw[1], nw[1]);
+      decode4(w2, complement, cw[2], nw[2]);
+      decode4(w3, complement, cw[3], nw[3]);
+    }
+    if (col + 16 <= L) {
+#pragma unroll
+      for (int q = 0; q < 16; ++q) {
+        const uint32_t m0 = (uint32_t)__builtin_amdgcn_sbfe((int)cw[q >> 2], 8 * (q & 3), 1);
+        const uint32_t m1 = (uint32_t)__builtin_amdgcn_sbfe((int)cw[q >> 2], 8 * (q & 3) + 1, 1);
+        const uint32_t m2 = (uint32_t)__builtin_amdgcn_sbfe((int)nw[q >> 2], 8 * (q & 3), 1);
+        myers_column(m, b0, b1, b2, m0, m1, m2, (uint32_t)q, width, wm);
+      }
+    } else {
+      const uint64_t clo = ((uint64_t)cw[1] << 32) | cw[0], chi = ((uint64_t)cw[3] << 32) | cw[2];
+      const uint64_t nlo = ((uint64_t)nw[1] << 32) | nw[0], nhi = ((uint64_t)nw[3] << 32) | nw[2];
+      for (int q = 0; q < L - col; ++q) {
+        const uint32_t cb = (uint32_t)((q < 8 ? clo : chi) >> (8 * (q & 7)));
+        const uint32_t nb = (uint32_t)((q < 8 ? nlo : nhi) >> (8 * (q & 7)));
+        myers_column(m, b0, b1, b2, 0u - (cb & 1u), 0u - ((cb >> 1) & 1u), 0u - (nb & 1u), (uint32_t)q, width, wm);
+      }
+    }
+    rejected = m.score > 3 * e;
+  }
+  int score = m.score;
+  int best = score, endp = L - 1;
+  if (!rejected) {
+    for (int j = 0; j < 2 * e; ++j) {
+      score += (int)((m.VP >> j) & 1u) - (int)((m.VN >> j) & 1u);
+      if (score < best) {
+        best = score;
+        endp = L + j;
+      }
+    }
+  }
+  const bool accepted = !rejected && best <= e;
+  p.ed[i] = accepted ? (uint8_t)best : (uint8_t)0xFF;
+  p.end[i] = accepted ? (int16_t)endp : (int16_t)0;
+  {
+    const uint32_t ln = lane_id();
+    const uint64_t acc = __ballot(accepted);
+    const uint32_t prev_read = __shfl_up(read, 1);
+    const bool joins_prev = accepted && ln > 0u && ((acc >> (ln - 1u)) & 1ull) && prev_read == read;
+    const uint64_t heads = __ballot(accepted && !joins_prev);
+    if (accepted && !joins_prev) {
+      const uint64_t stop = (heads | ~acc) >> ln >> 1;
+      const uint32_t run = stop ? (uint32_t)__builtin_ctzll(stop) + 1u : 64u - ln;
+      mapped += (uint32_t)(atomicAdd(&p.n_map[read], run) == 0u);
+    }
+    if (accepted) ++mappings;
+  }
+}
+
 __global__ void __launch_bounds__(256) verify_kernel(VerifyParams p) {
   if (p.ctr[1] != 0) return;
   const uint32_t total = min(p.ctr[0], p.cand_cap);
   const uint32_t stride = gridDim.x * blockDim.x;
   const int e = p.e;
   const uint32_t width = 2u * (uint32_t)e + 1u;
-  constexpr int kStageChunks = 4;
   __shared__ uint4 stage[kStageChunks][256];
   uint32_t(*part)[4] = (uint32_t(*)[4]) & stage[0][0];
   uint32_t mappings = 0, mapped = 0;
   for (uint32_t i = blockIdx.x * blockDim.x + threadIdx.x; i < total; i += stride) {
-    const uint32_t meta = p.cand_meta[i];
-    if (meta == kInvalidMeta) {
-      p.ed[i] = 0xFF, p.end[i] = 0;
-      continue;
-    }
-    const uint32_t read = (meta & ~kMeta16) >> 1, strand = meta & 1u;
-    const uint32_t wm = (meta & kMeta16) ? 0xFFFFu : 0xFFFFFFFFu;
-    const uint64_t c = p.cand[i];
-    const uint64_t pat = p.seq_off[(uint32_t)(c >> 32)] + (uint32_t)c;
-    const uint64_t off = p.read_off[read];
-    const int L = (int)(p.read_off[read + 1] - off);
-    const uint8_t *rd = p.bases + off;
-    const uint32_t complement = strand ? 0x03030303u : 0u;
-    MyersState m{0, 0, 0};
-    bool rejected = false;
-    const int n_steps = (L + 15) >> 4;
-    auto text_chunk = [&](int col) { return load_u128_unaligned(strand == 0 ? rd + col : rd + (L - 16 - col)); };
-    auto plane_chunk = [&](int q, int col) { return plane_window(p.planes, q, (pat + (uint32_t)col) >> 3); };
-    uint4 P0 = make_uint4(0, 0, 0, 0), P1 = P0, P2 = P0, P0n = P0, P1n = P0, P2n = P0;
-    if (n_steps > 0) {
-      P0n = plane_chunk(0, 0), P1n = plane_chunk(1, 0), P2n = plane_chunk(2, 0);
-    }
-    const uint32_t pat_bit = (uint32_t)pat & 7u;
-    for (int step = 0; step < n_steps && !rejected; ++step) {
-      const int col = step << 4, sub = step % kStepsPerPlaneLoad;
-      if (step % kStageChunks == 0) {
-        uint4 t4[kStageChunks];
-#pragma unroll
-        for (int c = 0; c < kStageChunks; ++c) t4[c] = step + c < n_steps ? text_chunk(col + 16 * c) : make_uint4(0, 0, 0, 0);
-#pragma unroll
-        for (int c = 0; c < kStageChunks; ++c) stage[c][threadIdx.x] = t4[c];
-      }
-      const uint4 r = stage[step % kStageChunks][threadIdx.x];
-      if (sub == 0) {
-        P0 = P0n, P1 = P1n, P2 = P2n;
-        if (step + kStepsPerPlaneLoad < n_steps) {
-          const int nc = col + 16 * kStepsPerPlaneLoad;
-          P0n = plane_chunk(0, nc), P1n = plane_chunk(1, nc), P2n = plane_chunk(2, nc);
-        }
-      } else {
-        window_advance16(P0), window_advance16(P1), window_advance16(P2);
-      }
-      const uint32_t b0 = window_head(P0, pat_bit), b1 = window_head(P1, pat_bit), b2 = window_head(P2, pat_bit);
-      uint32_t cw[4], nw[4];
-      {
-        const uint32_t w0 = strand ? __builtin_bswap32(r.w) : r.x, w1 = strand ? __builtin_bswap32(r.z) : r.y;
-        const uint32_t w2 = strand ? __builtin_bswap32(r.y) : r.z, w3 = strand ? __builtin_bswap32(r.x) : r.w;
-        decode4(w0, complement, cw[0], nw[0]);
-        decode4(w1, complement, cw[1], nw[1]);
-        decode4(w2, complement, cw[2], nw[2]);
-        decode4(w3, complement, cw[3], nw[3]);
-      }
-      if (col + 16 <= L) {
-#pragma unroll
-        for (int q = 0; q < 16; ++q) {
-          const uint32_t m0 = (uint32_t)__builtin_amdgcn_sbfe((int)cw[q >> 2], 8 * (q & 3), 1);
-          const uint32_t m1 = (uint32_t)__builtin_amdgcn_sbfe((int)cw[q >> 2], 8 * (q & 3) + 1, 1);
-          const uint32_t m2 = (uint32_t)__builtin_amdgcn_sbfe((int)nw[q >> 2], 8 * (q & 3), 1);
-          myers_column(m, b0, b1, b2, m0, m1, m2, (uint32_t)q, width, wm);
-        }
-      } else {
-        const uint64_t clo = ((uint64_t)cw[1] << 32) | cw[0], chi = ((uint64_t)cw[3] << 32) | cw[2];
-        const uint64_t nlo = ((uint64_t)nw[1] << 32) | nw[0], nhi = ((uint64_t)nw[3] << 32) | nw[2];
-        for (int q = 0; q < L - col; ++q) {
-          const uint32_t cb = (uint32_t)((q < 8 ? clo : chi) >> (8 * (q & 7)));
-          const uint32_t nb = (uint32_t)((q < 8 ? nlo : nhi) >> (8 * (q & 7)));
-          myers_column(m, b0, b1, b2, 0u - (cb & 1u), 0u - ((cb >> 1) & 1u), 0u - (nb & 1u), (uint32_t)q, width, wm);
-        }
-      }
-      rejected = m.score > 3 * e;
-    }
-    int score = m.score;
-    int best = score, endp = L - 1;
-    if (!rejected) {
-      for (int j = 0; j < 2 * e; ++j) {
-        score += (int)((m.VP >> j) & 1u) - (int)((m.VN >> j) & 1u);
-        if (score < best) {
-          best = score;
-          endp = L + j;
-        }
-      }
-    }
-    const bool accepted = !rejected && best <= e;
-    p.ed[i] = accepted ? (uint8_t)best : (uint8_t)0xFF;
-    p.end[i] = accepted ? (int16_t)endp : (int16_t)0;
-    {
-      const uint32_t ln = lane_id();
-      const uint64_t acc = __ballot(accepted);
-      const uint32_t prev_read = __shfl_up(read, 1);
-      const bool joins_prev = accepted && ln > 0u && ((acc >> (ln - 1u)) & 1ull) && prev_read == read;
-      const uint64_t heads = __ballot(accepted && !joins_prev);
-      if (accepted && !joins_prev) {
-        const uint64_t stop = (heads | ~acc) >> ln >> 1;
-        const uint32_t run = stop ? (uint32_t)__builtin_ctzll(stop) + 1u : 64u - ln;
-        mapped += (uint32_t)(atomicAdd(&p.n_map[read], run) == 0u);
-      }
-      if (accepted) ++mappings;
-    }
+    if (p.chunk_state && p.chunk_state[i / kSlotChunk] == kChunkVerified) continue;
+    verify_candidate<256u>(p, i, &stage[0][threadIdx.x], e, width, mappings, mapped);
   }
   for (int d = 32; d >= 1; d >>= 1) mappings += __shfl_xor(mappings, d), mapped += __shfl_xor(mapped, d);
   __syncthreads();
diff --git a/fem_amd/csrc/fem_seed_join.hip.h b/fem_amd/csrc/fem_seed_join.hip.h
--- a/fem_amd/csrc/fem_seed_join.hip.h
+++ b/fem_amd/csrc/fem_seed_join.hip.h
@@ -508,6 +508,88 @@
 
 constexpr int join_waves(int R) { return R <= 6 ? FEM_JOIN_WAVES_LO : FEM_JOIN_WAVES_HI; }
 
+#ifndef FEM_JOIN_WT
+#define FEM_JOIN_WT 1
+#endif
+#ifndef FEM_JOIN_TAIL
+#define FEM_JOIN_TAIL 1
+#endif
+constexpr uint32_t kTailClaim = 2u;
+
+typedef __attribute__((address_space(1))) uint32_t *GlobalU32;
+typedef __attribute__((address_space(1))) uint64_t *GlobalU64;
+__device__ __forceinline__ void store_through(uint64_t *at, uint64_t v) {
+  if (FEM_JOIN_WT) __hip_atomic_store((GlobalU64)at, v, __ATOMIC_RELAXED, __HIP_MEMORY_SCOPE_AGENT); else *at = v;
+}
+__device__ __forceinline__ void store_through(uint32_t *at, uint32_t v) {
+  if (FEM_JOIN_WT) __hip_atomic_store((GlobalU32)at, v, __ATOMIC_RELAXED, __HIP_MEMORY_SCOPE_AGENT); else *at = v;
+}
+__device__ __forceinline__ uint32_t load_agent(const uint32_t *at) {
+  return __hip_atomic_load((GlobalU32)at, __ATOMIC_RELAXED, __HIP_MEMORY_SCOPE_AGENT);
+}
+
+__device__ __forceinline__ void finish_chunk(const SeedParams &p, SlotChunk &ch) {
+  const uint32_t chunk_end = ch.next + ch.left;
+  for (uint32_t i = lane_id(); i < ch.left; i += kWave)
+    if ((unsigned long long)ch.next + i < p.cand_cap) store_through(&p.cand_meta[ch.next + i], kInvalidMeta);
+  ch.left = 0;
+  if (p.chunk_state != nullptr && chunk_end != 0u && chunk_end <= p.cand_cap) {
+    asm volatile("s_waitcnt vmcnt(0)" ::: "memory");
+    if (lane_id() == 0)
+      __hip_atomic_store((GlobalU32)p.chunk_state + (chunk_end / kSlotChunk - 1u), kChunkFinished, __ATOMIC_RELAXED, __HIP_MEMORY_SCOPE_AGENT);
+  }
+}
+
+typedef const __attribute__((address_space(4))) SeedParams *KernelSeedParams;
+template <int WAVES>
+__device__ __noinline__ void join_tail(KernelSeedParams args, __attribute__((address_space(3))) uint4 *stage_lds) {
+  const uint64_t args_at = (uint64_t)args;
+  const __attribute__((address_space(4))) SeedParams &p =
+      *(KernelSeedParams)(((uint64_t)(uint32_t)__builtin_amdgcn_readfirstlane((int)(uint32_t)(args_at >> 32)) << 32) |
+                          (uint32_t)__builtin_amdgcn_readfirstlane((int)(uint32_t)args_at));
+  if (p.chunk_state == nullptr) return;
+  const uint32_t ln = lane_id();
+  uint4 *stage = (uint4 *)stage_lds;
+#define FEM_GLOBAL(T, x) ((T *)(__attribute__((address_space(1))) T *)(x))
+  VerifyParams vp;
+  vp.bases = FEM_GLOBAL(const uint8_t, p.bases), vp.read_off = FEM_GLOBAL(const uint64_t, p.read_off);
+  vp.planes = FEM_GLOBAL(const uint8_t, p.planes), vp.seq_off = FEM_GLOBAL(const uint64_t, p.seq_off);
+  vp.cand = FEM_GLOBAL(const uint64_t, p.cand), vp.cand_meta = FEM_GLOBAL(const uint32_t, p.cand_meta);
+  vp.ctr = FEM_GLOBAL(const uint32_t, p.ctr), vp.cand_cap = p.cand_cap, vp.e = p.e;
+  vp.ed = FEM_GLOBAL(uint8_t, p.ed), vp.end = FEM_GLOBAL(int16_t, p.end), vp.n_map = FEM_GLOBAL(uint32_t, p.n_map);
+  vp.stats = FEM_GLOBAL(unsigned long long, p.stats), vp.chunk_state = nullptr;
+#undef FEM_GLOBAL
+  const int e = p.e;
+  const uint32_t width = 2u * (uint32_t)e + 1u;
+  uint32_t mappings = 0, mapped = 0, n_done = 0;
+  for (uint32_t taken = 0; taken < p.tail_max_chunks; taken += kTailClaim) {
+    const uint32_t handed = load_agent(&p.ctr[0]), flags = load_agent(&p.ctr[1]);
+    const uint32_t limit = (handed < p.cand_cap ? handed : p.cand_cap) / kSlotChunk;
+    if (flags != 0u || load_agent(p.verify_cursor) >= limit) break;
+    uint32_t first = 0;
+    if (ln == 0) first = atomicAdd((uint32_t *)(GlobalU32)p.verify_cursor, kTailClaim);
+    first = bcast0(first);
+#pragma unroll 1
+    for (uint32_t c = first; c < first + kTailClaim && c < limit; ++c) {
+      if (load_agent(&p.chunk_state[c]) != kChunkFinished) continue;
+      __builtin_amdgcn_fence(__ATOMIC_ACQUIRE, "agent");
+      asm volatile("s_waitcnt vmcnt(0)" ::: "memory");
+#pragma unroll 1
+      for (uint32_t k = 0; k < kSlotChunk; k += (uint32_t)kWave)
+        verify_candidate<(uint32_t)kWave>(vp, c * kSlotChunk + k + ln, stage + ln, e, width, mappings, mapped);
+      if (ln == 0) __hip_atomic_store((GlobalU32)p.chunk_state + c, kChunkVerified, __ATOMIC_RELAXED, __HIP_MEMORY_SCOPE_AGENT);
+      ++n_done;
+    }
+  }
+  if (n_done == 0u) return;
+  for (int d = 32; d >= 1; d >>= 1) mappings += __shfl_xor(mappings, d), mapped += __shfl_xor(mapped, d);
+  if (ln == 0) {
+    if (mappings) atomicAdd(&vp.stats[2], (unsigned long long)mappings);
+    if (mapped) atomicAdd(&vp.stats[3], (unsigned long long)mapped);
+    atomicAdd((uint32_t *)(GlobalU32)p.tail_chunks, n_done);
+  }
+}
+
 template <int R, bool BANKED = false, bool PADDED = false>
 __device__ __forceinline__ void seed_join_body(const SeedParams &p, uint8_t *smem) {
   constexpr uint32_t kSeeds = (uint32_t)(kStep * R);
@@ -629,7 +711,7 @@
               base = chunk.next;
               chunk.next += n_out, chunk.left -= n_out;
             } else {
-              pad_chunk(p, chunk);
+              finish_chunk(p, chunk);
               if (ln == 0) base = atomicAdd(&p.ctr[0], kSlotChunk);
               base = bcast0(base);
               chunk.next = base + n_out, chunk.left = kSlotChunk - n_out;
@@ -638,8 +720,8 @@
               if (ln == 0) atomicOr(&p.ctr[1], kFlagCandOverflow);
             } else {
               for (uint32_t i = ln; i < n_out; i += (uint32_t)kWave) {
-                p.cand[base + i] = stash[strand * kStash + i];
-                p.cand_meta[base + i] = (read * 2u + strand) | (i < (n_out & ~7u) ? kMeta16 : 0u);
+                store_through(&p.cand[base + i], stash[strand * kStash + i]);
+                store_through(&p.cand_meta[base + i], (read * 2u + strand) | (i < (n_out & ~7u) ? kMeta16 : 0u));
               }
             }
           }
@@ -695,7 +777,7 @@
             base = chunk.next;
             chunk.next += n_out, chunk.left -= n_out;
           } else {
-            pad_chunk(p, chunk);
+            finish_chunk(p, chunk);
             if (ln == 0) base = atomicAdd(&p.ctr[0], kSlotChunk);
             base = bcast0(base);
             chunk.next = base + n_out, chunk.left = kSlotChunk - n_out;
@@ -704,8 +786,8 @@
             if (ln == 0) atomicOr(&p.ctr[1], kFlagCandOverflow);
           } else if (ok) {
             const uint32_t rank = (uint32_t)__popcll(mo & ((1ull << ln) - 1ull)), at = base + rank;
-            p.cand[at] = out;
-            p.cand_meta[at] = (read * 2u + strand) | (rank < (n_out & ~7u) ? kMeta16 : 0u);
+            store_through(&p.cand[at], out);
+            store_through(&p.cand_meta[at], (read * 2u + strand) | (rank < (n_out & ~7u) ? kMeta16 : 0u));
           }
         }
         if (ln == 0) blk_entries[2u * rb + strand] = make_uint2(base, n_out);
@@ -720,13 +802,16 @@
       __builtin_nontemporal_store(entry.y, &p.cand_count[r0 * 2u + ln]);
     }
   }
-  pad_chunk(p, chunk);
+  finish_chunk(p, chunk);
   for (uint32_t i = ln; i < qchunk.left; i += kWave)
     if (qchunk.next + i < p.slow_cap) p.slow_queue[qchunk.next + i] = kInvalidRead;
   if (ln == 0) {
     if (pre_sum) atomicAdd(&p.stats[0], pre_sum);
     if (cand_sum) atomicAdd(&p.stats[1], cand_sum);
   }
+  static_assert(join_bitmap_words(R, PADDED) * 4u >= (uint32_t)kWave * kStageChunks * 16u, "the tail stages its reads' characters in the bitmap");
+  if (FEM_JOIN_TAIL && p.chunk_state != nullptr)
+    join_tail<join_waves(BANKED ? 7 : R)>((KernelSeedParams)__builtin_amdgcn_kernarg_segment_ptr(), (__attribute__((address_space(3))) uint4 *)bitmap);
 }
 
 
diff --git a/fem_amd/device.py b/fem_amd/device.py
--- a/fem_amd/device.py
+++ b/fem_amd/device.py
@@ -564,6 +564,10 @@
         self._check(self._L.fem_dev_kernel_time(self._h, kernel, C.byref(ms), C.byref(n)))
         return ms.value, int(n.value)
 
+    def tail_verified(self):
+        total, n = self.kernel_time(100)
+        return n, int(total)
+
     def h2d_bandwidth(self, nbytes=1 << 28, iters=8):
         g = C.c_double()
         self._check(self._L.fem_dev_h2d_bandwidth(self._h, nbytes, iters, C.byref(g)))
```

New measurement: 299.7. 0.888x the previous value.
